# google-research/rigl

Measured on AMD Instinct MI355X. Metric: images/sec/node, ResNet-50 80% ERK RigL step, higher is better.
Workload: dtype bf16

## Files before the change

### include/rigl_hip.h

```cpp
#ifndef RIGL_HIP_H_
#define RIGL_HIP_H_

#include <stddef.h>
#include <stdint.h>

#ifdef __cplusplus
extern "C" {
#endif

#define RIGL_ABI_VERSION 2

typedef void* rigl_stream_t;
typedef uint16_t rigl_bf16;

enum {
  RIGL_OK = 0,
  RIGL_EINVAL = -1,
  RIGL_ELAUNCH = -2,
  RIGL_EWORKSPACE = -3,
  RIGL_EUNSUPPORTED = -4
};

int rigl_version(void);
uint32_t rigl_crc32c(const void* data, size_t n, uint32_t crc);
// ... 104 lines not shown

int rigl_masked_adam(int64_t n, float* w, float* m, float* v,
                     const float* dense_grad, const uint32_t* mask_bits,
                     const float* beta_powers , float lr,
                     float beta1, float beta2, float epsilon,
                     float weight_decay, float grad_scale,
                     rigl_bf16* w_shadow, rigl_stream_t stream);
int rigl_adam_advance(float* beta_powers , float beta1,
                      float beta2, rigl_stream_t stream);

int rigl_pack_weights(const float* w, const uint32_t* mask_bits ,
                      int32_t k, int32_t cout, rigl_bf16* hwio, rigl_bf16* ohwi,
                      rigl_stream_t stream);
typedef struct RiglPackLayer {
  const float* w;
  const uint32_t* mask_bits;
  rigl_bf16* hwio;
  rigl_bf16* ohwi;
  int32_t k, cout;
} RiglPackLayer;
int rigl_pack_weights_batched(const RiglPackLayer* layers, int32_t n_layers,
                              rigl_stream_t stream);

typedef struct RiglConvDesc {
  int32_t n, h, w, cin;
  int32_t ho, wo, cout;
  int32_t kh, kw;
  int32_t stride_h, stride_w;
  int32_t pad_top, pad_left;
} RiglConvDesc;

size_t rigl_conv2d_workspace_bytes(const RiglConvDesc* d, int32_t which );
int rigl_masked_conv2d_fwd(const RiglConvDesc* d, const rigl_bf16* x,
                           const rigl_bf16* w_ohwi, rigl_bf16* y,
                           void* workspace, size_t workspace_bytes,
                           rigl_stream_t stream);
int rigl_masked_conv2d_dgrad(const RiglConvDesc* d, const rigl_bf16* dy,
                             const rigl_bf16* w_hwio, rigl_bf16* dx,
                             void* workspace, size_t workspace_bytes,
                             rigl_stream_t stream);
int32_t rigl_conv2d_stats_parts(const RiglConvDesc* d);
int rigl_masked_conv2d_fwd_stats(const RiglConvDesc* d, const rigl_bf16* x,
                                 const rigl_bf16* w_ohwi, rigl_bf16* y,
                                 float* stats, size_t stats_floats,
                                 void* workspace, size_t workspace_bytes,
                                 rigl_stream_t stream);
int32_t rigl_conv2d_fwd_takes_bn_input(const RiglConvDesc* d);
int rigl_masked_conv2d_fwd_bnrelu(const RiglConvDesc* d, const rigl_bf16* x_pre,
                                  const float* scale_shift, rigl_bf16* a_out,
                                  const rigl_bf16* w_ohwi, rigl_bf16* y,
                                  float* stats , size_t stats_floats,
                                  void* workspace, size_t workspace_bytes,
                                  rigl_stream_t stream);
int rigl_masked_conv2d_dgrad_acc(const RiglConvDesc* d, const rigl_bf16* dy,
                                 const rigl_bf16* w_hwio, const rigl_bf16* addend,
                                 rigl_bf16* dx, void* workspace,
                                 size_t workspace_bytes, rigl_stream_t stream);
int rigl_masked_conv2d_wgrad(const RiglConvDesc* d, const rigl_bf16* x,
                             const rigl_bf16* dy, float* dw, void* workspace,
                             size_t workspace_bytes, rigl_stream_t stream);

int rigl_masked_conv2d_bwd(const RiglConvDesc* d, const rigl_bf16* x,
                           const rigl_bf16* dy, const rigl_bf16* w_hwio,
                           const rigl_bf16* addend , float* dw,
                           rigl_bf16* dx , void* workspace,
                           size_t workspace_bytes, rigl_stream_t stream);

int rigl_masked_conv2d_bwd_grid(const RiglConvDesc* d, const rigl_bf16* x,
                                const rigl_bf16* dy, const rigl_bf16* w_hwio,
                                float* dw, rigl_bf16* dx_grid, void* workspace,
                                size_t workspace_bytes, rigl_stream_t stream);
int rigl_masked_conv2d_bwd_sub(const RiglConvDesc* d, const rigl_bf16* x,
                               const rigl_bf16* dy, const rigl_bf16* w_hwio,
                               const rigl_bf16* addend, int32_t sub_h, int32_t sub_w,
                               float* dw, rigl_bf16* dx, void* workspace,
                               size_t workspace_bytes, rigl_stream_t stream);
int32_t rigl_conv2d_bwd_takes_masked_addend(const RiglConvDesc* d);
int rigl_masked_conv2d_bwd_masked(const RiglConvDesc* d, const rigl_bf16* x,
                                  const rigl_bf16* dy, const rigl_bf16* w_hwio,
                                  const rigl_bf16* addend, const uint8_t* addend_bits,
                                  float* dw, rigl_bf16* dx, void* workspace,
                                  size_t workspace_bytes, rigl_stream_t stream);

typedef struct RiglBnReduceFuse {
  const rigl_bf16* x;
  const uint8_t* relu_bits;
  const float* params;
  int32_t relu;
  float* partial;
  size_t partial_floats;
} RiglBnReduceFuse;
int32_t rigl_conv2d_dgrad_stats_parts(const RiglConvDesc* d);
int rigl_masked_conv2d_bwd_bn(const RiglConvDesc* d, const rigl_bf16* x,
                              const rigl_bf16* dy, const rigl_bf16* w_hwio,
                              const rigl_bf16* addend, float* dw, rigl_bf16* dx,
                              void* workspace, size_t workspace_bytes,
                              const RiglBnReduceFuse* bn ,
                              rigl_stream_t stream);

size_t rigl_depthwise_conv2d_workspace_bytes(const RiglConvDesc* d);
int rigl_depthwise_conv2d_fwd(const RiglConvDesc* d, const rigl_bf16* x,
                              const float* w, rigl_bf16* y, rigl_stream_t stream);
int32_t rigl_depthwise_conv2d_stats_parts(const RiglConvDesc* d);
int rigl_depthwise_conv2d_fwd_stats(const RiglConvDesc* d, const rigl_bf16* x,
                                    const float* w, rigl_bf16* y, float* stats,
                                    size_t stats_floats, rigl_stream_t stream);
int rigl_depthwise_conv2d_dgrad(const RiglConvDesc* d, const rigl_bf16* dy,
                                const float* w, rigl_bf16* dx,
                                rigl_stream_t stream);
int rigl_depthwise_conv2d_wgrad(const RiglConvDesc* d, const rigl_bf16* x,
                                const rigl_bf16* dy, float* dw, void* workspace,
                                size_t workspace_bytes, rigl_stream_t stream);

int rigl_conv2d_fwd_ref(const RiglConvDesc* d, const rigl_bf16* x,
                        const rigl_bf16* w_ohwi, rigl_bf16* y,
                        rigl_stream_t stream);
int rigl_conv2d_dgrad_ref(const RiglConvDesc* d, const rigl_bf16* dy,
                          const rigl_bf16* w_hwio, rigl_bf16* dx,
                          rigl_stream_t stream);
int rigl_conv2d_wgrad_ref(const RiglConvDesc* d, const rigl_bf16* x,
                          const rigl_bf16* dy, float* dw, rigl_stream_t stream);

int rigl_masked_conv2d_fwd_f32(const RiglConvDesc* d, const float* x,
                               const float* w_hwio, const uint32_t* mask_bits ,
                               float* y, rigl_stream_t stream);
int rigl_masked_conv2d_dgrad_f32(const RiglConvDesc* d, const float* dy,
                                 const float* w_hwio, const uint32_t* mask_bits ,
                                 const float* addend ,
                                 float* dx, rigl_stream_t stream);
size_t rigl_conv2d_wgrad_f32_workspace_bytes(const RiglConvDesc* d);
int rigl_masked_conv2d_wgrad_f32(const RiglConvDesc* d, const float* x,
                                 const float* dy, float* dw, void* workspace,
                                 size_t workspace_bytes, rigl_stream_t stream);

size_t rigl_bn_workspace_bytes(int64_t m, int32_t c);
int rigl_bn_fwd(int64_t m, int32_t c, const rigl_bf16* x,
                const rigl_bf16* residual , const float* gamma,
                const float* beta, float* running_mean, float* running_var,
                float momentum, float eps, int32_t relu, rigl_bf16* y,
                float* save_mean, float* save_invstd, float* save_scale,
                float* save_shift, void* workspace, size_t workspace_bytes,
                rigl_stream_t stream);
int rigl_bn_fwd_stats(int64_t m, int32_t c, const rigl_bf16* x,
                      const rigl_bf16* residual ,
                      const float* gamma, const float* beta,
                      float* running_mean, float* running_var, float momentum,
                      float eps, int32_t relu, rigl_bf16* y, float* save_mean,
                      float* save_invstd, float* save_scale, float* save_shift,
                      const float* stats, int32_t stats_parts,
                      uint8_t* relu_bits ,
                      void* workspace, size_t workspace_bytes, rigl_stream_t stream);
int rigl_bn_bwd(int64_t m, int32_t c, const rigl_bf16* x,
                const rigl_bf16* y ,
                const uint8_t* relu_bits , const rigl_bf16* dy,
                const float* gamma, const float* save_mean,
                const float* save_invstd, const float* save_scale,
                const float* save_shift, int32_t relu, rigl_bf16* dx,
                rigl_bf16* dresidual , float* dgamma,
                float* dbeta, void* workspace, size_t workspace_bytes,
                rigl_stream_t stream);
int rigl_bn_bwd_stats(int64_t m, int32_t c, const rigl_bf16* x,
                      const rigl_bf16* y ,
                      const uint8_t* relu_bits , const rigl_bf16* dy,
                      const float* gamma, const float* save_mean,
                      const float* save_invstd, const float* save_scale,
                      const float* save_shift, int32_t relu, rigl_bf16* dx,
                      rigl_bf16* dresidual , float* dgamma,
                      float* dbeta, const float* stats, int32_t stats_parts,
                      void* workspace, size_t workspace_bytes, rigl_stream_t stream);

int rigl_bn_add_bn_fwd(int64_t m, int32_t c, const rigl_bf16* x, const rigl_bf16* x2,
                       const float* scale2, const float* shift2,
                       const float* gamma, const float* beta, float* running_mean,
                       float* running_var, float momentum, float eps, int32_t relu,
                       rigl_bf16* y, float* save_mean, float* save_invstd,
                       float* save_scale, float* save_shift, const float* stats,
                       int32_t stats_parts, uint8_t* relu_bits ,
                       void* workspace, size_t workspace_bytes, rigl_stream_t stream);
size_t rigl_bn_add_bn_bwd_workspace_bytes(int64_t m, int32_t c);
int rigl_bn_add_bn_bwd(int64_t m, int32_t c, const rigl_bf16* x, const rigl_bf16* x2,
                       const uint8_t* relu_bits, const rigl_bf16* dy,
                       const float* gamma, const float* save_mean, const float* save_invstd,
                       const float* gamma2, const float* save_mean2, const float* save_invstd2,
                       rigl_bf16* dx, rigl_bf16* dx2, float* dgamma, float* dbeta,
                       float* dgamma2, float* dbeta2, void* workspace,
                       size_t workspace_bytes, rigl_stream_t stream);

int rigl_stateless_random(float* out, int64_t n, int32_t seed0, int32_t seed1,
                          int32_t dist, float scale, float shift,
                          rigl_stream_t stream);
typedef struct {
  float* out;
  int64_t n;
  int32_t seed0, seed1;
  int32_t dist;
  float scale, shift;
} RiglRandomItem;
int rigl_stateless_random_batched(const RiglRandomItem* items, int32_t n_items,
                                  rigl_stream_t stream);

int rigl_maxpool_fwd(const RiglConvDesc* d, const rigl_bf16* x, rigl_bf16* y,
                     uint8_t* argmax, rigl_stream_t stream);
int rigl_maxpool_bwd(const RiglConvDesc* d, const rigl_bf16* dy,
                     const uint8_t* argmax, rigl_bf16* dx, rigl_stream_t stream);
int rigl_bn_fwd_statistics(int64_t m, int32_t c, const rigl_bf16* x ,
                           const float* gamma, const float* beta,
                           float* running_mean, float* running_var, float momentum,
                           float eps, float* save_mean, float* save_invstd,
                           float* save_scale, float* save_shift,
                           const float* stats, int32_t stats_parts,
                           void* workspace, size_t workspace_bytes, rigl_stream_t stream);
int rigl_bn_relu_maxpool_fwd(const RiglConvDesc* d, const rigl_bf16* x,
                             const float* scale, const float* shift, rigl_bf16* y,
                             uint8_t* argmax, rigl_stream_t stream);
size_t rigl_bn_relu_maxpool_bwd_workspace_bytes(const RiglConvDesc* d);
int rigl_bn_relu_maxpool_bwd(const RiglConvDesc* d, const rigl_bf16* x,
                             const rigl_bf16* dy, const uint8_t* argmax,
                             const float* gamma, const float* save_mean,
                             const float* save_invstd, const float* save_scale,
                             const float* save_shift, rigl_bf16* dx, float* dgamma,
                             float* dbeta, void* workspace, size_t workspace_bytes,
                             rigl_stream_t stream);

int rigl_global_avgpool_fwd(int32_t n, int32_t pixels, int32_t c, const rigl_bf16* x,
                            rigl_bf16* y, rigl_stream_t stream);
int rigl_global_avgpool_bwd(int32_t n, int32_t pixels, int32_t c, const rigl_bf16* dy,
                            rigl_bf16* dx, rigl_stream_t stream);
int rigl_global_avgpool_bwd_relu(int32_t n, int32_t pixels, int32_t c, const rigl_bf16* dy,
                                 const rigl_bf16* x, rigl_bf16* dx, rigl_stream_t stream);
int rigl_softmax_xent(int32_t rows, int32_t classes, const rigl_bf16* logits,
                      const int64_t* labels, float label_smoothing, float grad_scale,
                      float* row_loss, rigl_bf16* dlogits , rigl_stream_t stream);

int32_t rigl_conv2d_fwd_takes_relu_epilogue(const RiglConvDesc* d);
int32_t rigl_conv2d_bwd_takes_relu_epilogue(const RiglConvDesc* d);
int rigl_masked_conv2d_fwd_relu(const RiglConvDesc* d, const rigl_bf16* x,
                                const rigl_bf16* w_ohwi, rigl_bf16* y, void* workspace,
                                size_t workspace_bytes, rigl_stream_t stream);
int rigl_masked_conv2d_bwd_relu(const RiglConvDesc* d, const rigl_bf16* x,
                                const rigl_bf16* dy, const rigl_bf16* w_hwio, float* dw,
                                rigl_bf16* dx, void* workspace, size_t workspace_bytes,
                                rigl_stream_t stream);
int rigl_relu_fwd(int64_t n, const rigl_bf16* x, rigl_bf16* y, rigl_stream_t stream);
// ... 61 lines not shown
```

### rigl_amd/_lib.py

```python
import ctypes as C
import os

_HERE = os.path.dirname(os.path.abspath(__file__))
ABI_VERSION = 2
LIB_PATH = os.environ.get('RIGL_HIP_LIB') or os.path.join(_HERE, 'lib', 'librigl_hip.so')

RIGL_OK = 0
RIGL_EINVAL = -1
RIGL_ELAUNCH = -2
RIGL_EWORKSPACE = -3
RIGL_EUNSUPPORTED = -4
COUNTS_PER_LAYER = 8
MAGPRUNE_COUNTS_PER_LAYER = 4
PROF_KINDS = ('conv_fwd', 'conv_dgrad', 'conv_wgrad', 'prune_regrow',
              'sgd_momentum', 'pack_weights', 'conv_bwd', 'depthwise', 'masked_adam', 'magnitude_prune')

GROW_ZEROS, GROW_GRAD_SCALE, GROW_GRAD_SIGN, GROW_EXPLICIT = 0, 1, 2, 3
MOMRESET_ZEROS, MOMRESET_GRAD = 0, 1


class RiglError(RuntimeError):

  def __init__(self, code, msg):
    super().__init__('librigl_hip: error %d: %s' % (code, msg))
# ... 21 lines not shown
class MagnitudePruneLayer(C.Structure):
  _fields_ = [('n', C.c_int64), ('w', C.c_void_p), ('mask_bits', C.c_void_p), ('threshold', C.c_void_p),
              ('k', C.c_int64)]


class PackLayer(C.Structure):
  _fields_ = [('w', C.c_void_p), ('mask_bits', C.c_void_p),
              ('hwio', C.c_void_p), ('ohwi', C.c_void_p), ('k', C.c_int32),
              ('cout', C.c_int32)]


class ConvDesc(C.Structure):
  _fields_ = [('n', C.c_int32), ('h', C.c_int32), ('w', C.c_int32),
              ('cin', C.c_int32), ('ho', C.c_int32), ('wo', C.c_int32),
              ('cout', C.c_int32), ('kh', C.c_int32), ('kw', C.c_int32),
              ('stride_h', C.c_int32), ('stride_w', C.c_int32),
              ('pad_top', C.c_int32), ('pad_left', C.c_int32)]


class BnReduceFuse(C.Structure):
  _fields_ = [('x', C.c_void_p), ('relu_bits', C.c_void_p), ('params', C.c_void_p), ('relu', C.c_int32),
              ('partial', C.c_void_p), ('partial_floats', C.c_size_t)]


class RandomItem(C.Structure):
  _fields_ = [('out', C.c_void_p), ('n', C.c_int64), ('seed0', C.c_int32), ('seed1', C.c_int32),
              ('dist', C.c_int32), ('scale', C.c_float), ('shift', C.c_float)]


class BnInferItem(C.Structure):
  _fields_ = [('gamma', C.c_void_p), ('beta', C.c_void_p), ('moving_mean', C.c_void_p), ('moving_variance', C.c_void_p),
              ('scale_shift', C.c_void_p), ('c', C.c_int32), ('eps', C.c_float)]


class ProfLaunch(C.Structure):
  _fields_ = [('kind', C.c_int32), ('tag', C.c_int32 * 6), ('ms', C.c_float)]


_P, _I32, _I64, _F, _SZ = C.c_void_p, C.c_int32, C.c_int64, C.c_float, C.c_size_t
SIGNATURES = {
    'rigl_version': (C.c_int, []),
    'rigl_last_error': (C.c_char_p, []),
    'rigl_mask_pack': (C.c_int, [_P, _P, _I64, _P]),
    'rigl_mask_unpack': (C.c_int, [_P, _P, _I64, _P]),
    'rigl_prune_regrow_workspace_bytes': (_SZ, [C.POINTER(_I64), _I32]),
    'rigl_prune_regrow': (C.c_int, [C.POINTER(PruneRegrowLayer), _I32,
                                    C.POINTER(PruneRegrowParams), _P, _P, _SZ,
                                    _P]),
    'rigl_prune_regrow_slots': (C.c_int, [C.POINTER(PruneRegrowLayer), C.POINTER(_P), _I32,
                                          C.POINTER(PruneRegrowParams), _P, _P, _SZ, _P]),
    'rigl_prune_regrow_selections_workspace_bytes': (_SZ, [_I64]),
    'rigl_prune_regrow_selections': (C.c_int, [C.POINTER(PruneRegrowLayer), C.POINTER(PruneRegrowParams), _P, _P, _P, _P, _P,
                                               _P, _SZ, _P]),
    'rigl_prune_regrow_selections_slots': (C.c_int, [C.POINTER(PruneRegrowLayer), _P, C.POINTER(PruneRegrowParams), _P, _P,
                                                     _P, _P, _P, _P, _SZ, _P]),
    'rigl_topk_mask': (C.c_int, [_P, _I64, _I64, _P, _P, _SZ, _P]),
    'rigl_topk_mask_batched': (C.c_int, [C.POINTER(TopkLayer), _I32, _P, _SZ, _P]),
    'rigl_magnitude_prune_batched_workspace_bytes': (_SZ, [_I32]),
    'rigl_magnitude_prune_batched': (C.c_int, [C.POINTER(MagnitudePruneLayer), _I32, C.c_double, _P, _P, _SZ, _P]),
    'rigl_masked_sgd_momentum': (C.c_int, [_I64, _P, _P, _P, _P, _F, _F, _F, _F,
                                           _I32, _P, _P]),
    'rigl_masked_adam': (C.c_int, [_I64, _P, _P, _P, _P, _P, _P, _F, _F, _F, _F, _F, _F, _P, _P]),
    'rigl_adam_advance': (C.c_int, [_P, _F, _F, _P]),
    'rigl_pack_weights': (C.c_int, [_P, _P, _I32, _I32, _P, _P, _P]),
    'rigl_pack_weights_batched': (C.c_int, [C.POINTER(PackLayer), _I32, _P]),
    'rigl_conv2d_workspace_bytes': (_SZ, [C.POINTER(ConvDesc), _I32]),
    'rigl_masked_conv2d_fwd': (C.c_int, [C.POINTER(ConvDesc), _P, _P, _P, _P,
                                         _SZ, _P]),
    'rigl_masked_conv2d_dgrad': (C.c_int, [C.POINTER(ConvDesc), _P, _P, _P, _P,
                                           _SZ, _P]),
    'rigl_conv2d_stats_parts': (_I32, [C.POINTER(ConvDesc)]),
    'rigl_masked_conv2d_fwd_stats': (C.c_int, [C.POINTER(ConvDesc), _P, _P, _P, _P,
                                               _SZ, _P, _SZ, _P]),
    'rigl_conv2d_fwd_takes_bn_input': (_I32, [C.POINTER(ConvDesc)]),
    'rigl_masked_conv2d_fwd_bnrelu': (C.c_int, [C.POINTER(ConvDesc), _P, _P, _P, _P, _P, _P, _SZ, _P, _SZ, _P]),
    'rigl_masked_conv2d_dgrad_acc': (C.c_int, [C.POINTER(ConvDesc), _P, _P, _P,
                                               _P, _P, _SZ, _P]),
    'rigl_conv2d_dgrad_stats_parts': (_I32, [C.POINTER(ConvDesc)]),
    'rigl_masked_conv2d_bwd_bn': (C.c_int, [C.POINTER(ConvDesc), _P, _P, _P, _P, _P, _P, _P, _SZ,
                                            C.POINTER(BnReduceFuse), _P]),
    'rigl_masked_conv2d_bwd': (C.c_int, [C.POINTER(ConvDesc), _P, _P, _P, _P, _P, _P, _P, _SZ, _P]),
    'rigl_masked_conv2d_bwd_masked': (C.c_int, [C.POINTER(ConvDesc), _P, _P, _P, _P, _P, _P, _P, _P, _SZ, _P]),
    'rigl_conv2d_bwd_takes_masked_addend': (_I32, [C.POINTER(ConvDesc)]),
    'rigl_masked_conv2d_bwd_grid': (C.c_int, [C.POINTER(ConvDesc), _P, _P, _P, _P, _P, _P, _SZ, _P]),
    'rigl_masked_conv2d_bwd_sub': (C.c_int, [C.POINTER(ConvDesc), _P, _P, _P, _P, _I32, _I32, _P, _P, _P, _SZ, _P]),
    'rigl_masked_conv2d_wgrad': (C.c_int, [C.POINTER(ConvDesc), _P, _P, _P, _P,
                                           _SZ, _P]),
    'rigl_conv2d_fwd_ref': (C.c_int, [C.POINTER(ConvDesc), _P, _P, _P, _P]),
    'rigl_conv2d_dgrad_ref': (C.c_int, [C.POINTER(ConvDesc), _P, _P, _P, _P]),
    'rigl_conv2d_wgrad_ref': (C.c_int, [C.POINTER(ConvDesc), _P, _P, _P, _P]),
    'rigl_masked_conv2d_fwd_f32': (C.c_int, [C.POINTER(ConvDesc), _P, _P, _P, _P, _P]),
    'rigl_masked_conv2d_dgrad_f32': (C.c_int, [C.POINTER(ConvDesc), _P, _P, _P, _P, _P, _P]),
    'rigl_conv2d_wgrad_f32_workspace_bytes': (_SZ, [C.POINTER(ConvDesc)]),
    'rigl_masked_conv2d_wgrad_f32': (C.c_int, [C.POINTER(ConvDesc), _P, _P, _P, _P, _SZ, _P]),
    'rigl_depthwise_conv2d_workspace_bytes': (_SZ, [C.POINTER(ConvDesc)]),
    'rigl_depthwise_conv2d_fwd': (C.c_int, [C.POINTER(ConvDesc), _P, _P, _P, _P]),
    'rigl_depthwise_conv2d_stats_parts': (_I32, [C.POINTER(ConvDesc)]),
    'rigl_depthwise_conv2d_fwd_stats': (C.c_int, [C.POINTER(ConvDesc), _P, _P, _P, _P, _SZ, _P]),
    'rigl_depthwise_conv2d_dgrad': (C.c_int, [C.POINTER(ConvDesc), _P, _P, _P, _P]),
    'rigl_depthwise_conv2d_wgrad': (C.c_int, [C.POINTER(ConvDesc), _P, _P, _P, _P, _SZ, _P]),
    'rigl_bn_workspace_bytes': (_SZ, [_I64, _I32]),
    'rigl_bn_fwd': (C.c_int, [_I64, _I32, _P, _P, _P, _P, _P, _P, _F, _F, _I32, _P, _P, _P, _P, _P, _P, _SZ, _P]),
    'rigl_bn_fwd_stats': (C.c_int, [_I64, _I32, _P, _P, _P, _P, _P, _P, _F, _F, _I32, _P, _P, _P, _P, _P, _P, _I32, _P, _P, _SZ, _P]),
    'rigl_bn_bwd': (C.c_int, [_I64, _I32, _P, _P, _P, _P, _P, _P, _P, _P, _P, _I32, _P, _P, _P, _P, _P, _SZ, _P]),
    'rigl_bn_bwd_stats': (C.c_int, [_I64, _I32, _P, _P, _P, _P, _P, _P, _P, _P, _P, _I32, _P, _P, _P, _P, _P, _I32, _P, _SZ, _P]),
    'rigl_crc32c': (C.c_uint32, [_P, _SZ, C.c_uint32]),
    'rigl_stateless_random': (C.c_int, [_P, _I64, _I32, _I32, _I32, _F, _F, _P]),
    'rigl_stateless_random_batched': (C.c_int, [C.POINTER(RandomItem), _I32, _P]),
    'rigl_maxpool_fwd': (C.c_int, [C.POINTER(ConvDesc), _P, _P, _P, _P]),
    'rigl_maxpool_bwd': (C.c_int, [C.POINTER(ConvDesc), _P, _P, _P, _P]),
    'rigl_bn_fwd_statistics': (C.c_int, [_I64, _I32, _P, _P, _P, _P, _P, _F, _F, _P, _P, _P, _P, _P, _I32, _P, _SZ, _P]),
    'rigl_bn_add_bn_fwd': (C.c_int, [_I64, _I32, _P, _P, _P, _P, _P, _P, _P, _P, _F, _F, _I32, _P, _P, _P, _P, _P, _P, _I32, _P, _P, _SZ, _P]),
    'rigl_bn_add_bn_bwd_workspace_bytes': (_SZ, [_I64, _I32]),
    'rigl_bn_add_bn_bwd': (C.c_int, [_I64, _I32, _P, _P, _P, _P, _P, _P, _P, _P, _P, _P, _P, _P, _P, _P, _P, _P, _P, _SZ, _P]),
    'rigl_bn_relu_maxpool_fwd': (C.c_int, [C.POINTER(ConvDesc), _P, _P, _P, _P, _P, _P]),
    'rigl_bn_relu_maxpool_bwd_workspace_bytes': (_SZ, [C.POINTER(ConvDesc)]),
    'rigl_bn_relu_maxpool_bwd': (C.c_int, [C.POINTER(ConvDesc), _P, _P, _P, _P, _P, _P, _P, _P, _P, _P, _P, _P, _SZ, _P]),
    'rigl_global_avgpool_fwd': (C.c_int, [_I32, _I32, _I32, _P, _P, _P]),
    'rigl_global_avgpool_bwd': (C.c_int, [_I32, _I32, _I32, _P, _P, _P]),
    'rigl_softmax_xent': (C.c_int, [_I32, _I32, _P, _P, _F, _F, _P, _P, _P]),
    'rigl_global_avgpool_bwd_relu': (C.c_int, [_I32, _I32, _I32, _P, _P, _P, _P]),
    'rigl_conv2d_fwd_takes_relu_epilogue': (C.c_int32, [C.POINTER(ConvDesc)]),
    'rigl_conv2d_bwd_takes_relu_epilogue': (C.c_int32, [C.POINTER(ConvDesc)]),
    'rigl_masked_conv2d_fwd_relu': (C.c_int, [C.POINTER(ConvDesc), _P, _P, _P, _P, _SZ, _P]),
    'rigl_masked_conv2d_bwd_relu': (C.c_int, [C.POINTER(ConvDesc), _P, _P, _P, _P, _P, _P, _SZ, _P]),
    'rigl_relu_fwd': (C.c_int, [_I64, _P, _P, _P]),
    'rigl_relu_bwd': (C.c_int, [_I64, _P, _P, _P, _P]),
    'rigl_bn_infer_params_batched': (C.c_int, [C.POINTER(BnInferItem), _I32, _P]),
    'rigl_bn_apply': (C.c_int, [_I64, _I32, _P, _P, _P, _I32, _P, _P]),
    'rigl_bn_apply_pair': (C.c_int, [_I64, _I32, _P, _P, _P, _P, _I32, _P, _P]),
    'rigl_bn_relu_maxpool_infer': (C.c_int, [C.POINTER(ConvDesc), _P, _P, _P, _P]),
    'rigl_conv2d_fwd_takes_bn_epilogue': (C.c_int32, [C.POINTER(ConvDesc), _I32, _I32]),
    'rigl_masked_conv2d_fwd_bn_infer': (C.c_int, [C.POINTER(ConvDesc), _P, _P, _P, _P, _P, _I32, _P, _P]),
    'rigl_eval_metrics': (C.c_int, [_I32, _I32, _P, _P, _F, _I32, _P, _P, _P, _P]),
    'rigl_prof_enable': (C.c_int, [_I32]),
    'rigl_prof_collect': (C.c_int, [C.POINTER(C.c_double), C.POINTER(_I64)]),
    'rigl_prof_collect_kinds': (C.c_int, [C.POINTER(C.c_double), C.POINTER(_I64), _I32]),
    'rigl_prof_collect_launches': (C.c_int, [C.POINTER(ProfLaunch), _I64, C.POINTER(_I64)]),
    'rigl_probe_mfma_bf16': (C.c_int, [_I32, _I32, _P, _P]),
    'rigl_tune_set': (C.c_int, [C.c_char_p, _I32]),
    'rigl_tune_get': (_I32, [C.c_char_p, _I32]),
    'rigl_tune_generation': (C.c_uint64, []),
    'rigl_tune_generation_addr': (C.c_void_p, []),
    'rigl_tune_unset': (C.c_int, [C.c_char_p]),
}

_lib = None


def load():
  global _lib
  if _lib is not None:
    return _lib
  if not os.path.exists(LIB_PATH):
    raise RiglError(
        RIGL_ELAUNCH, 'HIP extension not built: %s is missing; run '
        '`python -c "import __graft_entry__ as g; g.build()"` or '
        '`make -C rigl_amd/csrc`' % LIB_PATH)
  try:
    import torch
  except ImportError:
    pass
  lib = C.CDLL(LIB_PATH, mode=C.RTLD_GLOBAL)
  for name, (res, args) in SIGNATURES.items():
    fn = getattr(lib, name)
    fn.restype = res
    fn.argtypes = args
  if lib.rigl_version() != ABI_VERSION:
    raise RiglError(RIGL_EINVAL, 'ABI version mismatch')
  _lib = lib
  return lib


def check(rc):
  if rc != RIGL_OK:
    raise RiglError(rc, load().rigl_last_error().decode('utf-8', 'replace'))
```

### rigl_amd/csrc/bn.hip

```cpp
#include "common.hpp"

namespace rigl {
namespace kbn {

constexpr int THREADS = 256;
constexpr int MAX_PARTS = 512;

__device__ __forceinline__ float bf_lo(uint32_t w) { return __uint_as_float(w << 16); }
__device__ __forceinline__ float bf_hi(uint32_t w) { return __uint_as_float(w & 0xFFFF0000u); }
__device__ __forceinline__ uint32_t f2bf(float f) {
  uint32_t u = __float_as_uint(f);
  if ((u & 0x7FFFFFFFu) > 0x7F800000u) return (u >> 16) | 0x40u;
  u += 0x7FFFu + ((u >> 16) & 1u);
  return u >> 16;
}
typedef __attribute__((ext_vector_type(2))) __bf16 bf16x2_t;
typedef __attribute__((ext_vector_type(2))) float f32x2_t;
__device__ __forceinline__ uint32_t pack2(float a, float b) {
  const f32x2_t v = {a, b};
  return __builtin_bit_cast(uint32_t, __builtin_convertvector(v, bf16x2_t));
}
__device__ __forceinline__ void unpack8(const uint4& v, float f[8]) {
  f[0] = bf_lo(v.x); f[1] = bf_hi(v.x); f[2] = bf_lo(v.y); f[3] = bf_hi(v.y);
  f[4] = bf_lo(v.z); f[5] = bf_hi(v.z); f[6] = bf_lo(v.w); f[7] = bf_hi(v.w);
// ... 204 lines not shown
    unpack8(ld16(x + i * 8, G.nt), xv);
    if (HAS_RES) unpack8(ld16(res + i * 8, G.nt), rv);
    float o[8];
#pragma unroll
    for (int j = 0; j < 8; ++j) {
      float v = fmaf(xv[j], psc[j], psh[j]);
      if (HAS_RES) v += rv[j];
      o[j] = RELU ? fmaxf(v, 0.f) : v;
    }
    uint4 out;
    out.x = pack2(o[0], o[1]); out.y = pack2(o[2], o[3]); out.z = pack2(o[4], o[5]); out.w = pack2(o[6], o[7]);
    st16(y + i * 8, out, G.nt);
    if (RELU && mbits) {
      uint32_t mb = 0u;
#pragma unroll
      for (int j = 0; j < 8; ++j) mb |= (o[j] > 0.f ? 1u : 0u) << j;
      mbits[i] = (uint8_t)mb;
    }
  }
}

template <int CL>
__global__ __launch_bounds__(THREADS) void k_bwd_finalize(Geom G, const float* __restrict__ partial,
                                                           const float* __restrict__ gamma, const float* __restrict__ invstd,
                                                           float* __restrict__ dgamma, float* __restrict__ dbeta,
                                                           float* __restrict__ coef ) {
  double s0, s1; int c; bool leader;
  sum_partials<CL>(G, partial, s0, s1, c, leader);
  if (!leader) return;
  dbeta[c] = (float)s0;
  dgamma[c] = (float)s1;
  coef[c] = gamma[c] * invstd[c];
  coef[G.C + c] = (float)(s0 / (double)G.M);
  coef[2 * G.C + c] = (float)(s1 / (double)G.M);
}

template <bool RELU, int MSK, bool HAS_DRES>
__global__ __launch_bounds__(THREADS) void k_bwd_apply(Geom G, const uint16_t* __restrict__ x, const uint16_t* __restrict__ y,
                                                        const uint8_t* __restrict__ mbits,
                                                        const uint16_t* __restrict__ dy, const float* __restrict__ mean,
                                                        const float* __restrict__ invstd, const float* __restrict__ scale,
                                                        const float* __restrict__ shift, const float* __restrict__ coef,
                                                        uint16_t* __restrict__ dx, uint16_t* __restrict__ dres) {
  extern __shared__ __attribute__((aligned(16))) float prm[];
  const bool fixed = G.fixed != 0;
  float pm[8], pis[8], pa[8], pb[8], pc[8], psc[8], psh[8];
  if (fixed) {
    const int c0 = (int)(((int64_t)blockIdx.x * THREADS + threadIdx.x) % G.cg) * 8;
    ld8f(mean + c0, pm); ld8f(invstd + c0, pis);
    ld8f(coef + c0, pa); ld8f(coef + G.C + c0, pb); ld8f(coef + 2 * G.C + c0, pc);
    if (RELU && MSK == 0) { ld8f(scale + c0, psc); ld8f(shift + c0, psh); }
  } else {
    for (int i = threadIdx.x; i < G.C; i += THREADS) {
      prm[i] = mean[i]; prm[G.C + i] = invstd[i];
      prm[2 * G.C + i] = coef[i]; prm[3 * G.C + i] = coef[G.C + i]; prm[4 * G.C + i] = coef[2 * G.C + i];
      if (RELU && MSK == 0) { prm[5 * G.C + i] = scale[i]; prm[6 * G.C + i] = shift[i]; }
    }
    __syncthreads();
  }
  const int64_t total = G.M * G.cg;
  const int64_t stride = (int64_t)gridDim.x * THREADS;
  for (int64_t i = (int64_t)blockIdx.x * THREADS + threadIdx.x; i < total; i += stride) {
    if (!fixed) {
      const int c0 = (int)(i % G.cg) * 8;
#pragma unroll
      for (int j = 0; j < 8; ++j) {
        pm[j] = prm[c0 + j]; pis[j] = prm[G.C + c0 + j]; pa[j] = prm[2 * G.C + c0 + j]; pb[j] = prm[3 * G.C + c0 + j];
        pc[j] = prm[4 * G.C + c0 + j];
        if (RELU && MSK == 0) { psc[j] = prm[5 * G.C + c0 + j]; psh[j] = prm[6 * G.C + c0 + j]; }
      }
    }
    float xv[8], dv[8], yv[8];
    unpack8(ld16(x + i * 8, G.nt), xv);
    unpack8(ld16(dy + i * 8, G.nt), dv);
    uint32_t mb = 0u;
    if (RELU && MSK == 1) unpack8(*reinterpret_cast<const uint4*>(y + i * 8), yv);
    if (RELU && MSK == 2) mb = mbits[i];
    float o[8], z[8];
#pragma unroll
    for (int j = 0; j < 8; ++j) {
      bool on = true;
      if (RELU) on = MSK == 1 ? (yv[j] > 0.f) : (MSK == 2 ? ((mb >> j) & 1u) != 0u : (fmaf(xv[j], psc[j], psh[j]) > 0.f));
      const float dz = on ? dv[j] : 0.f;
      const float xh = (xv[j] - pm[j]) * pis[j];
      o[j] = pa[j] * (dz - pb[j] - xh * pc[j]);
      z[j] = dz;
    }
    uint4 out;
    out.x = pack2(o[0], o[1]); out.y = pack2(o[2], o[3]); out.z = pack2(o[4], o[5]); out.w = pack2(o[6], o[7]);
    st16(dx + i * 8, out, G.nt);
    if (HAS_DRES) {
      out.x = pack2(z[0], z[1]); out.y = pack2(z[2], z[3]); out.z = pack2(z[4], z[5]); out.w = pack2(z[6], z[7]);
      st16(dres + i * 8, out, G.nt);
    }
  }
}

template <bool RELU>
__global__ __launch_bounds__(THREADS) void k_fwd_apply_pair(Geom G, const uint16_t* __restrict__ x, const uint16_t* __restrict__ x2,
                                                             const float* __restrict__ scale, const float* __restrict__ shift,
                                                             const float* __restrict__ scale2, const float* __restrict__ shift2,
                                                             uint16_t* __restrict__ y, uint8_t* __restrict__ mbits) {
  extern __shared__ __attribute__((aligned(16))) float prm[];
  const bool fixed = G.fixed != 0;
  float p0[8], p1[8], p2[8], p3[8];
  if (fixed) {
    const int c0 = (int)(((int64_t)blockIdx.x * THREADS + threadIdx.x) % G.cg) * 8;
    ld8f(scale + c0, p0); ld8f(shift + c0, p1); ld8f(scale2 + c0, p2); ld8f(shift2 + c0, p3);
  } else {
    for (int i = threadIdx.x; i < G.C; i += THREADS) {
      prm[i] = scale[i]; prm[G.C + i] = shift[i]; prm[2 * G.C + i] = scale2[i]; prm[3 * G.C + i] = shift2[i];
    }
    __syncthreads();
  }
  const int64_t total = G.M * G.cg;
  const int64_t stride = (int64_t)gridDim.x * THREADS;
  for (int64_t i = (int64_t)blockIdx.x * THREADS + threadIdx.x; i < total; i += stride) {
    if (!fixed) {
      const int c0 = (int)(i % G.cg) * 8;
#pragma unroll
      for (int j = 0; j < 8; ++j) { p0[j] = prm[c0 + j]; p1[j] = prm[G.C + c0 + j]; p2[j] = prm[2 * G.C + c0 + j]; p3[j] = prm[3 * G.C + c0 + j]; }
    }
    float xv[8], rv[8];
    unpack8(ld16(x + i * 8, G.nt), xv);
    unpack8(ld16(x2 + i * 8, G.nt), rv);
    float o[8];
#pragma unroll
    for (int j = 0; j < 8; j += 2) {
      const uint32_t pk = pack2(fmaf(rv[j], p2[j], p3[j]), fmaf(rv[j + 1], p2[j + 1], p3[j + 1]));
      float v0 = fmaf(xv[j], p0[j], p1[j]);
      float v1 = fmaf(xv[j + 1], p0[j + 1], p1[j + 1]);
      v0 += bf_lo(pk); v1 += bf_hi(pk);
      o[j] = RELU ? fmaxf(v0, 0.f) : v0;
      o[j + 1] = RELU ? fmaxf(v1, 0.f) : v1;
    }
    uint4 out;
    out.x = pack2(o[0], o[1]); out.y = pack2(o[2], o[3]); out.z = pack2(o[4], o[5]); out.w = pack2(o[6], o[7]);
    st16(y + i * 8, out, G.nt);
    if (RELU && mbits) {
      uint32_t mb = 0u;
#pragma unroll
      for (int j = 0; j < 8; ++j) mb |= (o[j] > 0.f ? 1u : 0u) << j;
      mbits[i] = (uint8_t)mb;
    }
  }
}

__global__ __launch_bounds__(THREADS) void k_reduce_pair(Geom G, const uint16_t* __restrict__ x, const uint16_t* __restrict__ x2,
                                                          const uint8_t* __restrict__ mbits, const uint16_t* __restrict__ dy,
                                                          const float* __restrict__ mean, const float* __restrict__ invstd,
                                                          const float* __restrict__ mean2, const float* __restrict__ invstd2,
                                                          float* __restrict__ partial, float* __restrict__ partial2) {
  __shared__ float red[THREADS][25];
  const int tx = threadIdx.x % G.tpr, ty = threadIdx.x / G.tpr;
  const int cgi = blockIdx.y * G.tpr + tx;
  const bool c_ok = cgi < G.cg;
  const int64_t r0 = (int64_t)blockIdx.x * G.rows_per_part;
  int64_t r1 = r0 + G.rows_per_part;
  if (r1 > G.M) r1 = G.M;
  float q0[8], q1[8], q2[8], mu[8], is[8], mu2[8], is2[8];
#pragma unroll
  for (int j = 0; j < 8; ++j) { q0[j] = q1[j] = q2[j] = 0.f; mu[j] = is[j] = mu2[j] = is2[j] = 0.f; }
  if (c_ok) {
#pragma unroll
    for (int j = 0; j < 8; ++j) {
      mu[j] = mean[cgi * 8 + j]; is[j] = invstd[cgi * 8 + j]; mu2[j] = mean2[cgi * 8 + j]; is2[j] = invstd2[cgi * 8 + j];
    }
    const int64_t rb = G.il ? (int64_t)blockIdx.x * G.rpb + ty : r0 + ty, re = G.il ? G.M : r1;
// ... 264 lines not shown
  using namespace rigl;
  using namespace rigl::kbn;
  if (m <= 0 || c <= 0 || (!x && !stats) || !gamma || !beta || !save_mean || !save_invstd || !save_scale || !save_shift)
    return fail(RIGL_EINVAL, "rigl_bn_fwd_statistics: bad arguments");
  if (c % 8) return fail(RIGL_EUNSUPPORTED, "rigl_bn_fwd_statistics: channels %% 8 != 0");
  if (stats && stats_parts <= 0) return fail(RIGL_EINVAL, "rigl_bn_fwd_statistics: stats_parts must be positive");
  Geom g = make_geom(m, c);
  int rc = fwd_statistics(g, c, x, gamma, beta, running_mean, running_var, momentum, eps, save_mean, save_invstd,
                          save_scale, save_shift, stats, stats_parts, workspace, workspace_bytes, as_stream(stream));
  if (rc) return rc;
  RIGL_CHECK_LAUNCH("rigl_bn_fwd_statistics");
  return RIGL_OK;
}

int rigl_bn_add_bn_fwd(int64_t m, int32_t c, const rigl_bf16* x, const rigl_bf16* x2, const float* scale2,
                       const float* shift2, const float* gamma, const float* beta, float* running_mean,
                       float* running_var, float momentum, float eps, int32_t relu, rigl_bf16* y, float* save_mean,
                       float* save_invstd, float* save_scale, float* save_shift, const float* stats,
                       int32_t stats_parts, uint8_t* relu_bits, void* workspace, size_t workspace_bytes,
                       rigl_stream_t stream) {
  using namespace rigl;
  using namespace rigl::kbn;
  if (m <= 0 || c <= 0 || !x || !x2 || !scale2 || !shift2 || !gamma || !beta || !y || !save_mean || !save_invstd ||
      !save_scale || !save_shift)
    return fail(RIGL_EINVAL, "rigl_bn_add_bn_fwd: bad arguments");
  if (c % 8) return fail(RIGL_EUNSUPPORTED, "rigl_bn_add_bn_fwd: channels %% 8 != 0");
  if (4 * (size_t)c * 4 > 65536) return fail(RIGL_EUNSUPPORTED, "rigl_bn_add_bn_fwd: too many channels for the LDS parameter cache");
  if (stats && stats_parts <= 0) return fail(RIGL_EINVAL, "rigl_bn_add_bn_fwd: stats_parts must be positive");
  hipStream_t st = as_stream(stream);
  Geom g = make_geom(m, c);
  int rc = fwd_statistics(g, c, x, gamma, beta, running_mean, running_var, momentum, eps, save_mean, save_invstd,
                          save_scale, save_shift, stats, stats_parts, workspace, workspace_bytes, st);
  if (rc) return rc;
  dim3 agrid(apply_grid(g));
  const size_t lds = g.fixed ? 0 : (size_t)4 * c * 4;
  if (relu) hipLaunchKernelGGL(k_fwd_apply_pair<true>, agrid, dim3(THREADS), lds, st, g, x, x2, save_scale, save_shift, scale2, shift2, y, relu_bits);
  else hipLaunchKernelGGL(k_fwd_apply_pair<false>, agrid, dim3(THREADS), lds, st, g, x, x2, save_scale, save_shift, scale2, shift2, y, nullptr);
  RIGL_CHECK_LAUNCH("rigl_bn_add_bn_fwd");
  return RIGL_OK;
}

size_t rigl_bn_add_bn_bwd_workspace_bytes(int64_t m, int32_t c) { return 2 * rigl_bn_workspace_bytes(m, c); }

int rigl_bn_add_bn_bwd(int64_t m, int32_t c, const rigl_bf16* x, const rigl_bf16* x2, const uint8_t* relu_bits,
                       const rigl_bf16* dy, const float* gamma, const float* save_mean, const float* save_invstd,
                       const float* gamma2, const float* save_mean2, const float* save_invstd2, rigl_bf16* dx,
                       rigl_bf16* dx2, float* dgamma, float* dbeta, float* dgamma2, float* dbeta2, void* workspace,
                       size_t workspace_bytes, rigl_stream_t stream) {
  using namespace rigl;
  using namespace rigl::kbn;
  if (m <= 0 || c <= 0 || !x || !x2 || !relu_bits || !dy || !gamma || !save_mean || !save_invstd || !gamma2 || !save_mean2 ||
      !save_invstd2 || !dx || !dx2 || !dgamma || !dbeta || !dgamma2 || !dbeta2)
    return fail(RIGL_EINVAL, "rigl_bn_add_bn_bwd: bad arguments");
  if (c % 8) return fail(RIGL_EUNSUPPORTED, "rigl_bn_add_bn_bwd: channels %% 8 != 0");
  const size_t lds = (size_t)10 * c * 4;
  if (lds > 160 * 1024 - 1024) return fail(RIGL_EUNSUPPORTED, "rigl_bn_add_bn_bwd: too many channels for the LDS parameter cache");
  const size_t need = rigl_bn_add_bn_bwd_workspace_bytes(m, c);
  if (!workspace || workspace_bytes < need) return fail(RIGL_EWORKSPACE, "rigl_bn_add_bn_bwd: workspace %zu < %zu", workspace_bytes, need);
  static const bool big_lds = hipFuncSetAttribute(reinterpret_cast<const void*>(&k_bwd_apply_pair),
                                                  hipFuncAttributeMaxDynamicSharedMemorySize, 159 * 1024) == hipSuccess;
  if (lds > 65536 && !big_lds) return fail(RIGL_ELAUNCH, "rigl_bn_add_bn_bwd: cannot raise the dynamic LDS limit");
  hipStream_t st = as_stream(stream);
  Geom g = make_geom(m, c);
  const size_t half = rigl_bn_workspace_bytes(m, c);
  const size_t part_bytes = align_up((size_t)g.parts * 2 * c * 4, 256);
  char* w0 = static_cast<char*>(workspace);
  float* partial = reinterpret_cast<float*>(w0);
  float* coef = reinterpret_cast<float*>(w0 + part_bytes);
  float* partial2 = reinterpret_cast<float*>(w0 + half);
  float* coef2 = reinterpret_cast<float*>(w0 + half + part_bytes);
  dim3 rgrid((unsigned)g.parts, (unsigned)((g.cg + g.tpr - 1) / g.tpr));
  hipLaunchKernelGGL(k_reduce_pair, rgrid, dim3(THREADS), 0, st, g, x, x2, relu_bits, dy, save_mean, save_invstd, save_mean2,
                     save_invstd2, partial, partial2);
  const FinSet f0 = {partial, gamma, save_invstd, dgamma, dbeta, coef};
  const FinSet f1 = {partial2, gamma2, save_invstd2, dgamma2, dbeta2, coef2};
  hipLaunchKernelGGL(k_bwd_finalize_pair<16>, dim3((unsigned)((c + 15) / 16), 2), dim3(THREADS), 0, st, g, f0, f1);
  const dim3 pgrid(apply_grid(g));
  hipLaunchKernelGGL(k_bwd_apply_pair, pgrid, dim3(THREADS), g.fixed ? 0 : lds, st, g, x, x2, relu_bits, dy, save_mean, save_invstd,
                     save_mean2, save_invstd2, coef, coef2, dx, dx2);
  RIGL_CHECK_LAUNCH("rigl_bn_add_bn_bwd");
  return RIGL_OK;
}

int rigl_bn_bwd_stats(int64_t m, int32_t c, const rigl_bf16* x, const rigl_bf16* y, const uint8_t* relu_bits,
                      const rigl_bf16* dy, const float* gamma,
                      const float* save_mean, const float* save_invstd, const float* save_scale, const float* save_shift,
                      int32_t relu, rigl_bf16* dx, rigl_bf16* dresidual, float* dgamma, float* dbeta,
                      const float* stats, int32_t stats_parts, void* workspace,
                      size_t workspace_bytes, rigl_stream_t stream) {
  using namespace rigl;
  using namespace rigl::kbn;
  if (m <= 0 || c <= 0 || !x || !dy || !gamma || !save_mean || !save_invstd || !dx || !dgamma || !dbeta)
    return fail(RIGL_EINVAL, "rigl_bn_bwd: bad arguments");
  if (c % 8) return fail(RIGL_EUNSUPPORTED, "rigl_bn_bwd: channels %% 8 != 0");
  if (relu && !y && !relu_bits && (!save_scale || !save_shift))
    return fail(RIGL_EINVAL, "rigl_bn_bwd: relu needs y, relu_bits or scale/shift");
  if (7 * (size_t)c * 4 > 65536) return fail(RIGL_EUNSUPPORTED, "rigl_bn_bwd: too many channels for the LDS parameter cache");
  if (stats && stats_parts <= 0) return fail(RIGL_EINVAL, "rigl_bn_bwd_stats: stats_parts must be positive");
  const size_t need = rigl_bn_workspace_bytes(m, c);
  if (!workspace || workspace_bytes < need) return fail(RIGL_EWORKSPACE, "rigl_bn_bwd: workspace %zu < %zu", workspace_bytes, need);
  hipStream_t st = as_stream(stream);
  Geom g = make_geom(m, c);
  float* partial = static_cast<float*>(workspace);
  float* coef = reinterpret_cast<float*>(static_cast<char*>(workspace) + align_up((size_t)g.parts * 2 * c * 4, 256));
  dim3 rgrid((unsigned)g.parts, (unsigned)((g.cg + g.tpr - 1) / g.tpr));
  const int msk = relu_bits ? 2 : (y ? 1 : 0);
  const float* red = partial;
  if (stats) {
    red = stats;
    g.parts = stats_parts;
  } else {
#define RIGL_BWD_REDUCE(R, K) hipLaunchKernelGGL((k_reduce<1, R, K>), rgrid, dim3(THREADS), 0, st, g, x, y, relu_bits, dy, save_mean, save_invstd, save_scale, save_shift, partial)
    if (!relu) RIGL_BWD_REDUCE(false, 0);
    else if (msk == 2) RIGL_BWD_REDUCE(true, 2);
    else if (msk == 1) RIGL_BWD_REDUCE(true, 1);
    else RIGL_BWD_REDUCE(true, 0);
#undef RIGL_BWD_REDUCE
  }
  if (g.parts > MAX_PARTS)
    hipLaunchKernelGGL(k_bwd_finalize<4>, dim3((unsigned)((c + 3) / 4)), dim3(THREADS), 0, st, g, red, gamma,
                       save_invstd, dgamma, dbeta, coef);
  else
    hipLaunchKernelGGL(k_bwd_finalize<16>, dim3((unsigned)((c + 15) / 16)), dim3(THREADS), 0, st, g, red, gamma,
                       save_invstd, dgamma, dbeta, coef);
  dim3 agrid(apply_grid(g));
  const size_t lds = g.fixed ? 0 : (size_t)7 * c * 4;
#define RIGL_BWD_APPLY(R, K, D) hipLaunchKernelGGL((k_bwd_apply<R, K, D>), agrid, dim3(THREADS), lds, st, g, x, y, relu_bits, dy, save_mean, save_invstd, save_scale, save_shift, coef, dx, dresidual)
  const bool dres = dresidual != nullptr;
  if (!relu) { if (dres) RIGL_BWD_APPLY(false, 0, true); else RIGL_BWD_APPLY(false, 0, false); }
  else if (msk == 2) { if (dres) RIGL_BWD_APPLY(true, 2, true); else RIGL_BWD_APPLY(true, 2, false); }
  else if (msk == 1) { if (dres) RIGL_BWD_APPLY(true, 1, true); else RIGL_BWD_APPLY(true, 1, false); }
  else { if (dres) RIGL_BWD_APPLY(true, 0, true); else RIGL_BWD_APPLY(true, 0, false); }
#undef RIGL_BWD_APPLY
  RIGL_CHECK_LAUNCH("rigl_bn_bwd");
  return RIGL_OK;
}

int rigl_bn_bwd(int64_t m, int32_t c, const rigl_bf16* x, const rigl_bf16* y, const uint8_t* relu_bits,
                const rigl_bf16* dy, const float* gamma,
                const float* save_mean, const float* save_invstd, const float* save_scale, const float* save_shift,
                int32_t relu, rigl_bf16* dx, rigl_bf16* dresidual, float* dgamma, float* dbeta, void* workspace,
                size_t workspace_bytes, rigl_stream_t stream) {
  return rigl_bn_bwd_stats(m, c, x, y, relu_bits, dy, gamma, save_mean, save_invstd, save_scale, save_shift, relu, dx,
                           dresidual, dgamma, dbeta, nullptr, 0, workspace, workspace_bytes, stream);
}

int rigl_bn_infer_params_batched(const RiglBnInferItem* items, int32_t n_items, rigl_stream_t stream) {
  using namespace rigl;
  using namespace rigl::kbn;
  if (n_items < 0 || (n_items > 0 && !items)) return fail(RIGL_EINVAL, "rigl_bn_infer_params_batched: bad arguments");
  for (int i = 0; i < n_items; ++i) {
    const RiglBnInferItem& t = items[i];
    if (t.c < 0 || (t.c > 0 && (!t.gamma || !t.beta || !t.moving_mean || !t.moving_variance || !t.scale_shift)))
      return fail(RIGL_EINVAL, "rigl_bn_infer_params_batched: item %d: bad channels / NULL tensor", i);
  }
  hipStream_t st = as_stream(stream);
  for (int b = 0; b < n_items; b += INFER_BATCH) {
    InferBatch B;
    B.count = 0;
    int32_t blk = 0;
    for (int i = b; i < n_items && i < b + INFER_BATCH; ++i) {
      if (items[i].c == 0) continue;
      B.it[B.count] = items[i];
      B.blk_begin[B.count] = blk;
      blk += (items[i].c + THREADS - 1) / THREADS;
      ++B.count;
    }
    B.blk_begin[B.count] = blk;
    if (B.count) hipLaunchKernelGGL(k_infer_params, dim3((unsigned)blk), dim3(THREADS), 0, st, B);
  }
  RIGL_CHECK_LAUNCH("rigl_bn_infer_params_batched");
  return RIGL_OK;
}

int rigl_bn_apply(int64_t m, int32_t c, const rigl_bf16* x, const rigl_bf16* residual, const float* scale_shift, int32_t relu,
                  rigl_bf16* y, rigl_stream_t stream) {
  using namespace rigl;
  using namespace rigl::kbn;
  if (m <= 0 || c <= 0 || !x || !scale_shift || !y) return fail(RIGL_EINVAL, "rigl_bn_apply: bad arguments");
  if (c % 8) return fail(RIGL_EUNSUPPORTED, "rigl_bn_apply: channels %% 8 != 0");
  if (2 * (size_t)c * 4 > 65536) return fail(RIGL_EUNSUPPORTED, "rigl_bn_apply: too many channels for the LDS parameter cache");
  hipStream_t st = as_stream(stream);
  Geom g = make_geom(m, c);
  dim3 agrid(apply_grid(g));
  const size_t lds = g.fixed ? 0 : (size_t)2 * c * 4;
  const float* sc = scale_shift;
  const float* sh = scale_shift + c;
  if (relu && residual) hipLaunchKernelGGL((k_fwd_apply<true, true>), agrid, dim3(THREADS), lds, st, g, x, residual, sc, sh, y, nullptr);
  else if (relu) hipLaunchKernelGGL((k_fwd_apply<true, false>), agrid, dim3(THREADS), lds, st, g, x, residual, sc, sh, y, nullptr);
  else if (residual) hipLaunchKernelGGL((k_fwd_apply<false, true>), agrid, dim3(THREADS), lds, st, g, x, residual, sc, sh, y, nullptr);
  else hipLaunchKernelGGL((k_fwd_apply<false, false>), agrid, dim3(THREADS), lds, st, g, x, residual, sc, sh, y, nullptr);
  RIGL_CHECK_LAUNCH("rigl_bn_apply");
  return RIGL_OK;
}

int rigl_bn_apply_pair(int64_t m, int32_t c, const rigl_bf16* x, const rigl_bf16* x2, const float* scale_shift,
                       const float* scale_shift2, int32_t relu, rigl_bf16* y, rigl_stream_t stream) {
  using namespace rigl;
  using namespace rigl::kbn;
  if (m <= 0 || c <= 0 || !x || !x2 || !scale_shift || !scale_shift2 || !y) return fail(RIGL_EINVAL, "rigl_bn_apply_pair: bad arguments");
  if (c % 8) return fail(RIGL_EUNSUPPORTED, "rigl_bn_apply_pair: channels %% 8 != 0");
  if (4 * (size_t)c * 4 > 65536) return fail(RIGL_EUNSUPPORTED, "rigl_bn_apply_pair: too many channels for the LDS parameter cache");
  hipStream_t st = as_stream(stream);
  Geom g = make_geom(m, c);
  dim3 agrid(apply_grid(g));
  const size_t lds = g.fixed ? 0 : (size_t)4 * c * 4;
  if (relu) hipLaunchKernelGGL(k_fwd_apply_pair<true>, agrid, dim3(THREADS), lds, st, g, x, x2, scale_shift, scale_shift + c, scale_shift2, scale_shift2 + c, y, nullptr);
  else hipLaunchKernelGGL(k_fwd_apply_pair<false>, agrid, dim3(THREADS), lds, st, g, x, x2, scale_shift, scale_shift + c, scale_shift2, scale_shift2 + c, y, nullptr);
  RIGL_CHECK_LAUNCH("rigl_bn_apply_pair");
  return RIGL_OK;
}

}
```

### rigl_amd/csrc/bwd1x1.hpp

```cpp
#pragma once

struct Bwd1x1Args {
  const uint16_t* X;
  const uint16_t* DY;
  const uint16_t* W;
  const uint16_t* ADD;
  uint16_t* DX;
  float* SLAB;
  int M, splits, interleave;
  uint32_t x_bytes, dy_bytes;
};

template <int ROWB>
__device__ __forceinline__ int dual_swz(int row) {
  if (ROWB == 512) return ((row & 1) << 1) | (((row >> 1) & 1) << 2) | (((row ^ (row >> 2)) & 1) << 3);
  return (((row >> 1) & 1) << 1) | ((((row >> 1) ^ (row >> 2)) & 1) << 2);
}

typedef __attribute__((ext_vector_type(4))) float f32x4;

template <int CI, int CO, bool DO_W, int NST>
struct Bwd1x1Smem { static constexpr int BYTES = NST * 32 * ((DO_W ? CI : 0) + CO) * 2 + (CI <= 64 ? 2 : 1) * 32 * (CI * 2 + 16); };
template <int CI, int CO, bool DO_W, int NST>
__global__ __launch_bounds__(THREADS) void k_bwd1x1(Bwd1x1Args P) {
  constexpr int PX = 32;
  constexpr int YROWB = CO * 2, XROWB = CI * 2;
  constexpr int Y_BYTES = PX * YROWB, X_BYTES = DO_W ? PX * XROWB : 0, STAGE = Y_BYTES + X_BYTES;
  constexpr int YI = YROWB / 32, XI = XROWB / 32;
  constexpr int YPW = YI / 4 > 0 ? YI / 4 : 1, XPW = XI / 4 > 0 ? XI / 4 : 1;
  static_assert(YI % 4 == 0 && XI % 4 == 0, "tiles are whole rounds of four waves");
  constexpr int L = YPW + (DO_W ? XPW : 0);
  constexpr int CF = CI / 16, CFW = CF / 2;
  constexpr int KSD = CO / 32;
  constexpr int NFI = CI / 32, NFO = CO / 32;
  constexpr bool WIDE_O = NFO >= NFI;
  constexpr int WF = NFI * NFO / 4 > 0 ? NFI * NFO / 4 : 1;
  static_assert(CFW * KSD * 4 <= 96, "W fragments stay in registers");
  constexpr bool DXDB = CI <= 64;
  constexpr int NDX = DXDB ? 2 : 1;
  constexpr int DXROWB = XROWB + 16, DX_BYTES = PX * DXROWB;
  static_assert(NST * STAGE + NDX * DX_BYTES == Bwd1x1Smem<CI, CO, DO_W, NST>::BYTES, "host and device agree on the LDS size");
  extern __shared__ __attribute__((aligned(1024))) unsigned char smem[];
  unsigned char* const dxs = smem + NST * STAGE;

  const int tid = threadIdx.x, lane = tid & 63;
  const int wave = __builtin_amdgcn_readfirstlane(tid >> 6);
  const int split = blockIdx.x;
  const int KT_all = (P.M + PX - 1) / PX;
  const int kt_begin = P.interleave ? split : (int)((int64_t)KT_all * split / P.splits);
  const int kt_step = P.interleave ? P.splits : 1;
  const int KT = P.interleave ? (split < KT_all ? (KT_all - split + P.splits - 1) / P.splits : 0)
                              : (int)((int64_t)KT_all * (split + 1) / P.splits) - kt_begin;
  const __amdgpu_buffer_rsrc_t rsrcY = make_rsrc(P.DY, P.dy_bytes), rsrcX = make_rsrc(P.X, P.x_bytes);
  const u32x4 rsrcY4 = make_rsrc4(P.DY, P.dy_bytes), rsrcX4 = make_rsrc4(P.X, P.x_bytes);
  (void)rsrcY4; (void)rsrcX4; (void)rsrcY; (void)rsrcX;

  int y_row[YPW], y_col[YPW], x_row[XPW], x_col[XPW];
#pragma unroll
  for (int q = 0; q < YPW; ++q) {
    const int i = q * 4 + wave, row = i * (1024 / YROWB) + lane / (YROWB / 16), slot = lane % (YROWB / 16);
    y_row[q] = row; y_col[q] = (slot ^ dual_swz<YROWB>(row)) * 8;
  }
#pragma unroll
  for (int q = 0; q < XPW; ++q) {
    const int i = q * 4 + wave, row = i * (1024 / XROWB) + lane / (XROWB / 16), slot = lane % (XROWB / 16);
    x_row[q] = row; x_col[q] = (slot ^ dual_swz<XROWB>(row)) * 8;
  }
#if !defined(RIGL_B1_NO_NT) && !defined(RIGL_DMA_BUILTIN)
#define B1_DMA16(r_, lds_, off_) lds_dma16_nt(r_##4, lds_, off_)
#else
#define B1_DMA16(r_, lds_, off_) RIGL_DMA16(r_, lds_, off_)
#endif
#define B1_ISSUE(kt_, stage_)                                                                            \
  {                                                                                                      \
    const int p0_ = (kt_begin + (kt_) * kt_step) * PX;                                                             \
    _Pragma("unroll") for (int q = 0; q < YPW; ++q) {                                                    \
      const int p_ = p0_ + y_row[q];                                                                     \
      const int off_ = p_ < P.M ? (int)((uint32_t)(p_ * CO + y_col[q]) * 2u) : (int)OOB;                 \
      B1_DMA16(rsrcY, smem + (stage_) * STAGE + (q * 4 + wave) * 1024, off_); \
    }                                                                                                    \
    if (DO_W) {                                                                                          \
      _Pragma("unroll") for (int q = 0; q < XPW; ++q) {                                                  \
        const int p_ = p0_ + x_row[q];                                                                   \
        const int off_ = p_ < P.M ? (int)((uint32_t)(p_ * CI + x_col[q]) * 2u) : (int)OOB;               \
        B1_DMA16(rsrcX, smem + (stage_) * STAGE + Y_BYTES + (q * 4 + wave) * 1024, off_); \
      }                                                                                                  \
    }                                                                                                    \
  }

  const int pf = wave & 1, chalf = wave >> 1;
  bf16x8 wfr[CFW][KSD];
#pragma unroll
  for (int c = 0; c < CFW; ++c)
#pragma unroll
    for (int ks = 0; ks < KSD; ++ks) {
      const int ci = (chalf * CFW + c) * 16 + (lane & 15), co = ks * 32 + (lane >> 4) * 8;
      wfr[c][ks] = *reinterpret_cast<const bf16x8*>(P.W + (int64_t)ci * CO + co);
    }
  const int d_row = 16 * pf + (lane & 15);
  const int d_base = d_row * YROWB, d_swz = dual_swz<YROWB>(d_row), d_hi = lane >> 4;

  const int g = lane >> 4, j16 = lane & 15;
  const int t_row = 8 * (g >> 1) + (j16 >> 2);
  const int t_low = 2 * (g & 1) + ((j16 >> 1) & 1), t_half = (j16 & 1) * 8;
  f32x16 acc2[DO_W ? WF : 1];
  if (DO_W) {
#pragma unroll
    for (int f = 0; f < WF; ++f)
#pragma unroll
      for (int e = 0; e < 16; ++e) acc2[f][e] = 0.f;
  }
  const int w_fix = WIDE_O ? wave % NFI : wave % NFO;
  const int w_var0 = WIDE_O ? (wave / NFI) * WF : (wave / NFO) * WF;
#define B1_TR_OFF(ROWB_, chunk_, plus4_) \
  ((t_row + (plus4_)) * (ROWB_) + ((((chunk_) + t_low) ^ dual_swz<ROWB_>(t_row + (plus4_))) << 4) + t_half)

  constexpr int DXP = PX * (CI / 8) / THREADS;
  static_assert(PX * (CI / 8) % THREADS == 0, "whole pieces per thread");
  constexpr int W_N = L * (NST - 2), W_A = W_N + DXP * (NST - 1);
  uint4 addv[DXP];
#define B1_FLUSH(ktp_, second_barrier_)                                                                    \
  {                                                                                                        \
    const int p0_ = (kt_begin + (ktp_) * kt_step) * PX;                                                              \
    const unsigned char* src_ = dxs + ((ktp_) & (NDX - 1)) * DX_BYTES;                                     \
    uint4 v_[DXP];                                                                                         \
    _Pragma("unroll") for (int q = 0; q < DXP; ++q) {                                                      \
      const int idx = q * THREADS + tid, row = idx / (CI / 8), ch = idx % (CI / 8);                        \
      v_[q] = *reinterpret_cast<const uint4*>(src_ + row * DXROWB + ch * 16);                              \
    }                                                                                                      \
    if (second_barrier_) __syncthreads();                                                                  \
    _Pragma("unroll") for (int q = 0; q < DXP; ++q) {                                                      \
      const int idx = q * THREADS + tid, row = idx / (CI / 8), ch = idx % (CI / 8);                        \
      if (p0_ + row < P.M) {                                                                               \
        uint4 v = v_[q];                                                                                   \
        if (P.ADD) {                                                                                       \
          const uint4 a = addv[q];                                                                         \
          v.x = add_bf16x2(v.x, a.x); v.y = add_bf16x2(v.y, a.y); v.z = add_bf16x2(v.z, a.z); v.w = add_bf16x2(v.w, a.w); \
        }                                                                                                  \
        *reinterpret_cast<uint4*>(P.DX + (int64_t)(p0_ + row) * CI + ch * 8) = v;                          \
      }                                                                                                    \
    }                                                                                                      \
  }
  for (int t = 0; t < NST - 1; ++t)
    if (t < KT) B1_ISSUE(t, t);
  for (int kt = 0; kt < KT; ++kt) {
    if (kt + NST - 1 <= KT) {
      if (P.ADD && kt >= NST - 1) wait_vmcnt<W_A>();
      else wait_vmcnt<W_N>();
    } else {
      wait_vmcnt<0>();
    }
    asm volatile("s_waitcnt lgkmcnt(0)" ::: "memory");
    __builtin_amdgcn_s_barrier();
    asm volatile("" ::: "memory");
    if (kt + NST - 1 < KT) B1_ISSUE(kt + NST - 1, (kt + NST - 1) % NST);
    asm volatile("" ::: "memory");
    __builtin_amdgcn_sched_barrier(0);
    if (kt > 0) B1_FLUSH(kt - 1, !DXDB);
    asm volatile("" ::: "memory");
    __builtin_amdgcn_sched_barrier(0);
    const unsigned char* Ys = smem + (kt % NST) * STAGE;
    const unsigned char* Xs = Ys + Y_BYTES;
    if (P.ADD) {
      const int p0 = (kt_begin + kt * kt_step) * PX;
#pragma unroll
      for (int q = 0; q < DXP; ++q) {
        const int idx = q * THREADS + tid, row = idx / (CI / 8), ch = idx % (CI / 8);
        addv[q] = p0 + row < P.M ? *reinterpret_cast<const uint4*>(P.ADD + (int64_t)(p0 + row) * CI + ch * 8) : make_uint4(0u, 0u, 0u, 0u);
      }
    }
    asm volatile("" ::: "memory");
    __builtin_amdgcn_sched_barrier(0);
    f32x4 acc1[CFW];
#pragma unroll
    for (int c = 0; c < CFW; ++c) acc1[c] = (f32x4){0.f, 0.f, 0.f, 0.f};
#pragma unroll
    for (int ks = 0; ks < KSD; ++ks) {
      const bf16x8 yf = *reinterpret_cast<const bf16x8*>(Ys + d_base + (((4 * ks + d_hi) ^ d_swz) << 4));
#pragma unroll
      for (int c = 0; c < CFW; ++c) acc1[c] = __builtin_amdgcn_mfma_f32_16x16x32_bf16(wfr[c][ks], yf, acc1[c], 0, 0, 0);
    }
    if (DO_W) {
#pragma unroll
      for (int k2 = 0; k2 < 2; ++k2) {
        bf16x8 fa[WIDE_O ? 1 : WF], fb[WIDE_O ? WF : 1];
        if (WIDE_O) {
          fa[0] = lds_read_tr_pair(Xs + k2 * 16 * XROWB + B1_TR_OFF(XROWB, w_fix * 4, 0), Xs + k2 * 16 * XROWB + B1_TR_OFF(XROWB, w_fix * 4, 4));
#pragma unroll
          for (int f = 0; f < WF; ++f)
            fb[f] = lds_read_tr_pair(Ys + k2 * 16 * YROWB + B1_TR_OFF(YROWB, (w_var0 + f) * 4, 0),
                                     Ys + k2 * 16 * YROWB + B1_TR_OFF(YROWB, (w_var0 + f) * 4, 4));
#pragma unroll
          for (int f = 0; f < WF; ++f) acc2[f] = __builtin_amdgcn_mfma_f32_32x32x16_bf16(fa[0], fb[f], acc2[f], 0, 0, 0);
        } else {
          fb[0] = lds_read_tr_pair(Ys + k2 * 16 * YROWB + B1_TR_OFF(YROWB, w_fix * 4, 0), Ys + k2 * 16 * YROWB + B1_TR_OFF(YROWB, w_fix * 4, 4));
#pragma unroll
          for (int f = 0; f < WF; ++f)
            fa[f] = lds_read_tr_pair(Xs + k2 * 16 * XROWB + B1_TR_OFF(XROWB, (w_var0 + f) * 4, 0),
                                     Xs + k2 * 16 * XROWB + B1_TR_OFF(XROWB, (w_var0 + f) * 4, 4));
#pragma unroll
          for (int f = 0; f < WF; ++f) acc2[f] = __builtin_amdgcn_mfma_f32_32x32x16_bf16(fa[f], fb[0], acc2[f], 0, 0, 0);
        }
      }
    }
    {
      const int prow = 16 * pf + (lane & 15);
      unsigned char* const dst = dxs + (kt & (NDX - 1)) * DX_BYTES;
#pragma unroll
      for (int c = 0; c < CFW; ++c) {
        const f32x2 lo = {acc1[c][0], acc1[c][1]}, hi2 = {acc1[c][2], acc1[c][3]};
        uint2 pk;
        pk.x = __builtin_bit_cast(uint32_t, __builtin_convertvector(lo, bf16x2));
        pk.y = __builtin_bit_cast(uint32_t, __builtin_convertvector(hi2, bf16x2));
        *reinterpret_cast<uint2*>(dst + prow * DXROWB + ((chalf * CFW + c) * 16 + (lane >> 4) * 4) * 2) = pk;
      }
    }
  }
  if (KT > 0) {
    __syncthreads();
    B1_FLUSH(KT - 1, false);
  }
#undef B1_FLUSH
#undef B1_ISSUE
#undef B1_TR_OFF
  if (DO_W) {
    float* const out = P.SLAB + (int64_t)split * CI * CO;
#pragma unroll
    for (int f = 0; f < WF; ++f) {
      const int fi = WIDE_O ? w_fix : w_var0 + f, fo = WIDE_O ? w_var0 + f : w_fix;
#pragma unroll
      for (int e = 0; e < 16; ++e) {
        const int ci = fi * 32 + (e & 3) + 8 * (e >> 2) + 4 * (lane >> 5), co = fo * 32 + (lane & 31);
        out[(int64_t)ci * CO + co] = acc2[f][e];
      }
    }
  }
}

static inline int bwd1x1_kind(const RiglConvDesc* d) {
  if (d->kh != 1 || d->kw != 1 || d->stride_h != 1 || d->stride_w != 1 || d->pad_top || d->pad_left) return 0;
  if (d->ho != d->h || d->wo != d->w) return 0;
  if ((int64_t)d->n * d->h * d->w < 65536) return 0;
  if (RIGL_TUNE("bwd1x1", 1) == 0) return 0;
  if (d->cin == 64 && d->cout == 256) return 1;
  if (d->cin == 64 && d->cout == 64) return 3;
  return 0;
}
static inline int bwd1x1_splits() { return 2 * num_cus(); }
static inline size_t bwd1x1_workspace(const RiglConvDesc* d) {
  return bwd1x1_kind(d) ? (size_t)2 * num_cus() * d->cin * d->cout * 4 : 0;
}
template <int CI, int CO, bool DO_W, int NST>
static bool bwd1x1_ready_i() {
  constexpr int SMEM = Bwd1x1Smem<CI, CO, DO_W, NST>::BYTES;
  static_assert(SMEM <= 160 * 1024 / 2, "the rings of the two workgroups resident on a CU fit its LDS");
  static const bool ready = hipFuncSetAttribute(reinterpret_cast<const void*>(&k_bwd1x1<CI, CO, DO_W, NST>),
                                                hipFuncAttributeMaxDynamicSharedMemorySize, SMEM) == hipSuccess;
  return ready;
}
static bool bwd1x1_ready(const RiglConvDesc* d) {
  switch (bwd1x1_kind(d)) {
    case 1: return bwd1x1_ready_i<64, 256, true, 3>();
    case 3: return bwd1x1_ready_i<64, 64, true, 3>();
    default: return false;
  }
}
template <int CI, int CO, bool DO_W, int NST>
static bool launch_bwd1x1_i(const Bwd1x1Args& a, hipStream_t st) {
  constexpr int SMEM = Bwd1x1Smem<CI, CO, DO_W, NST>::BYTES;
  if (!bwd1x1_ready_i<CI, CO, DO_W, NST>()) return false;
  RIGL_K_LAUNCH((k_bwd1x1<CI, CO, DO_W, NST>), dim3((unsigned)a.splits), dim3(THREADS), SMEM, st, a);
  return true;
}
template <int CI, int CO>
static bool launch_bwd1x1_t(const Bwd1x1Args& a, bool w, hipStream_t st) {
  return w ? launch_bwd1x1_i<CI, CO, true, 3>(a, st) : launch_bwd1x1_i<CI, CO, false, 3>(a, st);
}
static bool launch_bwd1x1(const RiglConvDesc* d, const rigl_bf16* x, const rigl_bf16* dy, const rigl_bf16* w_hwio,
                          const rigl_bf16* addend, rigl_bf16* dx, float* slab, hipStream_t st) {
  Bwd1x1Args a = {};
  a.X = x; a.DY = dy; a.W = w_hwio; a.ADD = addend; a.DX = dx; a.SLAB = slab;
  a.M = d->n * d->h * d->w; a.splits = bwd1x1_splits(); a.interleave = RIGL_TUNE("bwd1x1_il", 1);
  a.x_bytes = (uint32_t)((size_t)a.M * d->cin * 2); a.dy_bytes = (uint32_t)((size_t)a.M * d->cout * 2);
  const bool w = slab != nullptr;
  switch (bwd1x1_kind(d)) {
    case 1: return launch_bwd1x1_t<64, 256>(a, w, st);
    case 3: return launch_bwd1x1_t<64, 64>(a, w, st);
    default: return false;
  }
}
```

### rigl_amd/csrc/common.hpp

```cpp
#pragma once
#include <hip/hip_runtime.h>
#include <hip/hip_ext.h>
#include <stdarg.h>
#include <atomic>
#include <stdint.h>
#include <stdio.h>

#include "../../include/rigl_hip.h"

namespace rigl {

void set_error(const char* fmt, ...);
int fail(int code, const char* fmt, ...);

int tune_get(const char* key, int dflt);
struct TuneSite { std::atomic<uint64_t> gen{0}; std::atomic<int> value{0}; };
uint64_t tune_generation();
int tune_cached(TuneSite& site, const char* key, int dflt);
#define RIGL_TUNE(key, dflt) ([]() -> int { static ::rigl::TuneSite site__; return ::rigl::tune_cached(site__, key, dflt); }())

inline hipStream_t as_stream(rigl_stream_t s) { return reinterpret_cast<hipStream_t>(s); }

#define RIGL_CHECK_LAUNCH(what)                                              \
  do {                                                                       \
    hipError_t e__ = hipGetLastError();                                      \
    if (e__ != hipSuccess)                                                   \
      return ::rigl::fail(RIGL_ELAUNCH, "%s: %s", what, hipGetErrorString(e__)); \
  } while (0)

#define RIGL_HIP(call)                                                       \
  do {                                                                       \
    hipError_t e__ = (call);                                                 \
    if (e__ != hipSuccess)                                                   \
      return ::rigl::fail(RIGL_ELAUNCH, "%s: %s", #call, hipGetErrorString(e__)); \
  } while (0)

enum ProfKind { PROF_CONV_FWD = 0, PROF_CONV_DGRAD = 1, PROF_CONV_WGRAD = 2,
                PROF_PRUNE_REGROW = 3, PROF_SGD = 4, PROF_PACK = 5, PROF_CONV_BWD = 6, PROF_DEPTHWISE = 7,
                PROF_ADAM = 8, PROF_MAGPRUNE = 9 };
bool prof_enabled();
void prof_begin(int kind, hipStream_t s);
void prof_end(int kind, hipStream_t s);

hipEvent_t prof_get_event();
void prof_add_pair(int kind, hipEvent_t a, hipEvent_t b);
int& prof_current_kind();
void prof_set_tag(const RiglConvDesc* d);
struct ProfFamily {
  int prev;
  explicit ProfFamily(int k) : prev(prof_current_kind()) { prof_current_kind() = k; }
  ~ProfFamily() { prof_current_kind() = prev; }
};

struct ProfScope {
  int kind; hipStream_t s; bool on;
  ProfScope(int k, hipStream_t st) : kind(k), s(st), on(prof_enabled()) { if (on) prof_begin(kind, s); }
  ~ProfScope() { if (on) prof_end(kind, s); }
};

template <typename F, typename... Args>
inline void prof_launch(F kernel, dim3 grid, dim3 blk, unsigned lds, hipStream_t st, Args... args) {
  hipEvent_t a = prof_get_event(), b = prof_get_event();
  if (!a || !b) { hipLaunchKernelGGL(kernel, grid, blk, lds, st, args...); return; }
  hipExtLaunchKernelGGL(kernel, grid, blk, lds, st, a, b, 0, args...);
  prof_add_pair(prof_current_kind(), a, b);
}
#define RIGL_K_LAUNCH(kernel, grid, blk, lds, st, ...)                                      \
  do {                                                                                      \
    if (::rigl::prof_enabled()) ::rigl::prof_launch(kernel, grid, blk, lds, st, __VA_ARGS__); \
    else hipLaunchKernelGGL(kernel, grid, blk, lds, st, __VA_ARGS__);                       \
  } while (0)

inline int64_t ceil_div64(int64_t a, int64_t b) { return (a + b - 1) / b; }
inline size_t align_up(size_t x, size_t a) { return (x + a - 1) / a * a; }

__device__ __forceinline__ uint32_t relu_bf16x2(uint32_t v) {
  return v & ~(((v & 0x80008000u) >> 15) * 0xFFFFu);
}
__device__ __forceinline__ uint32_t gate_bf16x2(uint32_t v, uint32_t x) {
  const uint32_t lo = (x & 0xFFFFu) - 1u < 0x7FFFu ? 0x0000FFFFu : 0u;
  const uint32_t hi = (x >> 16) - 1u < 0x7FFFu ? 0xFFFF0000u : 0u;
  return v & (lo | hi);
}
__device__ __forceinline__ uint4 relu_bf16x8(uint4 v) {
  return make_uint4(relu_bf16x2(v.x), relu_bf16x2(v.y), relu_bf16x2(v.z), relu_bf16x2(v.w));
}
__device__ __forceinline__ uint4 gate_bf16x8(uint4 v, uint4 x) {
  return make_uint4(gate_bf16x2(v.x, x.x), gate_bf16x2(v.y, x.y), gate_bf16x2(v.z, x.z), gate_bf16x2(v.w, x.w));
}

}
```

### rigl_amd/csrc/conv.hip

```cpp
#include <stdlib.h>

#include "common.hpp"

#if defined(RIGL_ABLATE) && RIGL_ABLATE == 1
#define RIGL_MFMA_OR_ABLATE(i, j) acc[i][j][0] += (float)af[i][0] + (float)bfr[j][0];
#else
#define RIGL_MFMA_OR_ABLATE(i, j) acc[i][j] = __builtin_amdgcn_mfma_f32_32x32x16_bf16(bfr[j], af[i], acc[i][j], 0, 0, 0);
#endif

namespace rigl {
namespace k1 {

typedef __attribute__((ext_vector_type(8))) __bf16 bf16x8;
typedef __attribute__((ext_vector_type(2))) __bf16 bf16x2;
typedef __attribute__((ext_vector_type(2))) float f32x2;
typedef __attribute__((ext_vector_type(16))) float f32x16;

constexpr int THREADS = 256;

__device__ __forceinline__ uint16_t f2bf(float f) {
  uint32_t u = __float_as_uint(f);
  if ((u & 0x7FFFFFFFu) > 0x7F800000u) return (uint16_t)((u >> 16) | 0x40u);
  u += 0x7FFFu + ((u >> 16) & 1u);
  return (uint16_t)(u >> 16);
// ... 1665 lines not shown
    tg = tiny_geom(d);
    const size_t xp_bytes = (size_t)d->n * tg.hp * tg.wp * 4 * 2;
    uint16_t* xp = reinterpret_cast<uint16_t*>(ws);
    ws += align_up(xp_bytes, 256);
    PadArgs pa = {x, xp, d->n, d->h, d->w, d->cin, tg.hp, tg.wp, d->pad_top, d->pad_left};
    RIGL_K_LAUNCH(k_pad_input4, dim3(2048), dim3(THREADS), 0, st, pa);
    a.X = xp; a.Cin = tg.cred; a.x_pix_stride = 4; a.KH = d->kh; a.KW = 1; a.H = tg.hp; a.W = tg.wp;
    a.Ho = d->ho; a.Wo = d->wo; a.sh = d->stride_h; a.sw = d->stride_w; a.ph = a.pw = 0;
    a.x_bytes = (uint32_t)xp_bytes;
    a.fold = tg.cred; a.Cin = d->kh * tg.cred; a.KH = 1;
    n_out = (int64_t)d->kh * tg.cred * d->cout;
    tiny_tmp = reinterpret_cast<float*>(ws);
    ws += align_up((size_t)n_out * 4, 256);
  } else if (small_cin(d)) {
    const int K = d->kh * d->kw * d->cin, Kp = kpad(d);
    uint16_t* col = reinterpret_cast<uint16_t*>(ws);
    ws += align_up((size_t)a.M * Kp * 2, 256);
    Im2colArgs ia = {x, col, a.M, d->cin, d->kh, d->kw, d->h, d->w, d->ho, d->wo, d->stride_h, d->stride_w, d->pad_top, d->pad_left, K, Kp};
    RIGL_K_LAUNCH(k_im2col, dim3(2048), dim3(THREADS), 0, st, ia);
    a.X = col; a.Cin = Kp; a.x_pix_stride = Kp; a.KH = a.KW = 1; a.H = 1; a.W = a.M; a.Ho = 1; a.Wo = a.M;
    a.sh = a.sw = 1; a.ph = a.pw = 0;
    a.x_bytes = (uint32_t)((size_t)a.M * Kp * 2);
    n_out = (int64_t)K * d->cout;
  } else {
    a.X = x; a.Cin = d->cin; a.x_pix_stride = d->cin; a.KH = d->kh; a.KW = d->kw; a.H = d->h; a.W = d->w;
    a.Ho = d->ho; a.Wo = d->wo; a.sh = d->stride_h; a.sw = d->stride_w; a.ph = d->pad_top; a.pw = d->pad_left;
    a.x_bytes = (uint32_t)((size_t)d->n * d->h * d->w * d->cin * 2);
    n_out = (int64_t)d->kh * d->kw * d->cin * d->cout;
  }
  WgradPlan p = plan_wgrad(a.M, a.Cin, a.Cout, a.KH * a.KW);
  a.tiles_ci = p.tiles_ci; a.tiles_co = p.tiles_co; a.splits = p.splits; a.slab_elems = p.slab;
  const bool two_pass = p.splits > 1 || small_cin(d) || tiny_cin(d);
  a.OUT = two_pass ? reinterpret_cast<float*>(ws) : dw;
  dim3 grid((unsigned)((int64_t)p.tiles_ci * p.tiles_co * a.KH * a.KW * p.splits)), blk(THREADS);
  if (wgrad_stages(p.tm, p.tn) == 3) RIGL_K_LAUNCH((k_wgrad_tr<2, 2, 3>), grid, blk, 0, st, a);
  else if (p.tm == 2) RIGL_K_LAUNCH((k_wgrad_tr<2, 1, 4>), grid, blk, 0, st, a);
  else if (p.tn == 2) RIGL_K_LAUNCH((k_wgrad_tr<1, 2, 4>), grid, blk, 0, st, a);
  else RIGL_K_LAUNCH((k_wgrad_tr<1, 1, 4>), grid, blk, 0, st, a);
  if (two_pass) {
    ReduceArgs ra = {reinterpret_cast<const float*>(ws), tiny_tmp ? tiny_tmp : dw, n_out, p.slab, p.splits};
    launch_wgrad_reduce(ra, st);
  }
  if (tiny_tmp)
    RIGL_K_LAUNCH(k_stem_unpack, dim3(64), blk, 0, st, tiny_tmp, dw, d->kh, d->kw, d->cin, tg.cred, d->cout, 0);
  RIGL_CHECK_LAUNCH("rigl_masked_conv2d_wgrad");
  return RIGL_OK;
}

static int bwd_impl(const RiglConvDesc* d, const rigl_bf16* x, const rigl_bf16* dy, const rigl_bf16* w_hwio,
                    const rigl_bf16* addend, float* dw, rigl_bf16* dx, void* workspace, size_t workspace_bytes,
                    const RiglBnReduceFuse* bn, rigl_stream_t stream, AddendSub sub = {1, 1},
                    const RiglConvDesc* dg = nullptr, const uint8_t* addend_bits = nullptr, int epi = rigl::k1::EPI_NONE);

int rigl_masked_conv2d_bwd_bn(const RiglConvDesc* d, const rigl_bf16* x, const rigl_bf16* dy, const rigl_bf16* w_hwio,
                              const rigl_bf16* addend, float* dw, rigl_bf16* dx, void* workspace, size_t workspace_bytes,
                              const RiglBnReduceFuse* bn, rigl_stream_t stream) {
  if (bn && !dx) return rigl::fail(RIGL_EINVAL, "rigl_masked_conv2d_bwd_bn: the reductions ride on dX, which was not requested");
  return bwd_impl(d, x, dy, w_hwio, addend, dw, dx, workspace, workspace_bytes, bn, stream);
}

static int bwd_impl(const RiglConvDesc* d, const rigl_bf16* x, const rigl_bf16* dy, const rigl_bf16* w_hwio,
                    const rigl_bf16* addend, float* dw, rigl_bf16* dx, void* workspace, size_t workspace_bytes,
                    const RiglBnReduceFuse* bn, rigl_stream_t stream, AddendSub sub, const RiglConvDesc* dg,
                    const uint8_t* addend_bits, int epi) {
  using namespace rigl;
  using namespace rigl::k1;
  static const bool fuse = [] { const char* e = getenv("RIGL_BWD_FUSED"); return e ? atoi(e) != 0 : true; }();
  const RiglConvDesc* dd = dg ? dg : d;
  int rc = check_desc(d, "rigl_masked_conv2d_bwd");
  if (rc) return rc;
  hipStream_t st = as_stream(stream);
  prof_set_tag(d);
  const bool subadd = addend_is_sub(addend, sub);
  if (subadd && bn) return fail(RIGL_EUNSUPPORTED, "rigl_masked_conv2d_bwd: a subsampled addend and the batch-norm reductions do not combine");
  if (subadd && !dx) return fail(RIGL_EINVAL, "rigl_masked_conv2d_bwd: an addend without dX");
  const bool both = dx && x && dy && w_hwio && dw;
  const bool whole = both && !subadd && !dg;
  const size_t need = rigl_conv2d_workspace_bytes(d, 2);
  bool dgrad_pp = false;
  if (dx && (d->cin % 8) == 0 && (d->cout % 8) == 0 && !bn && !subadd && !dg) {
    const IgemmArgs ap = dgrad_args(d, dy, w_hwio, addend, dx);
    dgrad_pp = plan_pp<1>(ap).variant != 0;
  }
  if (whole && !bn && bwd1x1_kind(d) && bwd1x1_ready(d)) {
    if (need && (!workspace || workspace_bytes < need))
      return fail(RIGL_EWORKSPACE, "rigl_masked_conv2d_bwd: workspace %zu < %zu", workspace_bytes, need);
    ProfFamily prof(PROF_CONV_BWD);
    if (launch_bwd1x1(d, x, dy, w_hwio, addend, dx, static_cast<float*>(workspace), st)) {
      const int64_t n_out = (int64_t)d->cin * d->cout;
      ReduceArgs ra = {static_cast<const float*>(workspace), dw, n_out, n_out, bwd1x1_splits()};
      launch_wgrad_reduce(ra, st);
      RIGL_CHECK_LAUNCH("rigl_masked_conv2d_bwd");
      return RIGL_OK;
    }
  }
  {
    BsPlan bp;
    if (both && !dg && !bn && bs_use(d, &bp)) {
      if (need && (!workspace || workspace_bytes < need))
        return fail(RIGL_EWORKSPACE, "rigl_masked_conv2d_bwd: workspace %zu < %zu", workspace_bytes, need);
      ProfFamily prof(PROF_CONV_BWD);
      launch_bs(d, bp, x, dy, w_hwio, addend, dx, static_cast<float*>(workspace), st, sub.sh, sub.sw, addend_bits);
      const int64_t n_out = (int64_t)d->cin * d->cout;
      ReduceArgs ra = {static_cast<const float*>(workspace), dw, n_out, n_out, bp.G};
      launch_wgrad_reduce(ra, st);
      RIGL_CHECK_LAUNCH("rigl_masked_conv2d_bwd");
      return RIGL_OK;
    }
  }
  if (addend_bits) return fail(RIGL_EUNSUPPORTED, "rigl_masked_conv2d_bwd_masked: this layer's kernels take no masked addend (ask rigl_conv2d_bwd_takes_masked_addend)");
  {
    RsPlan rp;
    if (whole && !bn && rs_use<1>(d, &rp)) {
      ProfFamily prof(PROF_CONV_BWD);
      rc = rigl_masked_conv2d_wgrad(d, x, dy, dw, workspace, workspace_bytes, stream);
      if (rc) return rc;
      prof_current_kind() = PROF_CONV_BWD;
      launch_rs<1>(d, rp, dy, w_hwio, addend, dx, nullptr, st);
      RIGL_CHECK_LAUNCH("rigl_masked_conv2d_bwd");
      return RIGL_OK;
    }
  }
  if (whole && !bn && c3x3_use(d)) {
    if (need && (!workspace || workspace_bytes < need))
      return fail(RIGL_EWORKSPACE, "rigl_masked_conv2d_bwd: workspace %zu < %zu", workspace_bytes, need);
    ProfFamily prof(PROF_CONV_BWD);
    float* slabs = static_cast<float*>(workspace);
    launch_c3x3_wgrad(d, x, dy, slabs, st);
    ReduceArgs ra = {slabs, dw, (int64_t)9 * 64 * 64, (int64_t)9 * 64 * 64, c3x3_wgrad_geom(d).grid};
    launch_wgrad_reduce(ra, st);
    launch_c3x3<true>(d, dy, w_hwio, addend, dx, nullptr, st);
    RIGL_CHECK_LAUNCH("rigl_masked_conv2d_bwd");
    return RIGL_OK;
  }
  if (RIGL_TUNE("pp_bwd", -1) != 0 && both && !subadd && !bn && !tiny_cin(d) && !small_cin(d) && pp_wgrad_legal(d)) {
    IgemmArgs ad = dgrad_args(dd, dy, w_hwio, addend, dx);
    const int dvar = RIGL_TUNE("pp_dgrad", -1) >= 0 ? PP_NONE : pp_bwd_dgrad_variant(ad);
    if (dvar != PP_NONE && pp_legal<1>(ad, dvar)) {
      int bm, bn2;
      pp_dims(dvar, bm, bn2);
      const bool strided = pp_strided(ad);
      const int tiles_m = strided ? pp_fill_classes(ad, bm) : (ad.M + bm - 1) / bm;
      const unsigned nd = (unsigned)(tiles_m * (ad.N / bn2));
      const int kt_d = (int)((int64_t)dd->kh * dd->kw * (dd->cout / 64) * bm * bn2 / (256 * 256) / (dd->stride_h * dd->stride_w));
      const PPBwdPlan pw = plan_wgrad_pp(d, nd, kt_d);
      if (need && (!workspace || workspace_bytes < need))
        return fail(RIGL_EWORKSPACE, "rigl_masked_conv2d_bwd: workspace %zu < %zu", workspace_bytes, need);
      ProfFamily prof(PROF_CONV_BWD);
      const WgradArgs aw = pp_wgrad_args(d, x, dy, pw, dw, workspace);
      ad.fd_rw = make_fastdiv(ad.RW); ad.fd_rh = make_fastdiv(ad.RH);
      ad.tiles_n = ad.N / bn2;
      if (epi == EPI_RELU ? pp_bwd_launch<EPI_RELU>(dvar, strided, ad, aw, pw, st) : pp_bwd_launch(dvar, strided, ad, aw, pw, st)) {
        if (pw.splits > 1) {
          ReduceArgs ra = {static_cast<const float*>(workspace), dw, pw.slab, pw.slab, pw.splits};
          launch_wgrad_reduce(ra, st);
        }
        RIGL_CHECK_LAUNCH("rigl_masked_conv2d_bwd");
        return RIGL_OK;
      }
    }
  }
  if (fuse && !dgrad_pp && both && !tiny_cin(d) && !small_cin(d) && (d->cin % 8) == 0 && (d->cout % 8) == 0) {
    IgemmArgs ad = dgrad_args(dd, dy, w_hwio, addend, dx);
    if (subadd) set_addend_sub(ad, dd, sub);
    rc = attach_bn(ad, d, bn);
    if (rc) return rc;
    const IgemmPlan pd = plan_igemm<1>(ad);
    WgradArgs aw = {};
    aw.interleave = RIGL_TUNE("wgrad_il", 1);
    aw.DY = dy; aw.M = d->n * d->ho * d->wo; aw.Cout = d->cout;
    aw.dy_bytes = (uint32_t)((size_t)aw.M * d->cout * 2);
    aw.X = x; aw.Cin = d->cin; aw.x_pix_stride = d->cin; aw.KH = d->kh; aw.KW = d->kw; aw.H = d->h; aw.W = d->w;
    aw.Ho = d->ho; aw.Wo = d->wo; aw.sh = d->stride_h; aw.sw = d->stride_w; aw.ph = d->pad_top; aw.pw = d->pad_left;
    aw.x_bytes = (uint32_t)((size_t)d->n * d->h * d->w * d->cin * 2);
    const WgradPlan p = plan_wgrad(aw.M, aw.Cin, aw.Cout, aw.KH * aw.KW, true);
    if (pd.dma) {
      if (need && (!workspace || workspace_bytes < need))
        return fail(RIGL_EWORKSPACE, "rigl_masked_conv2d_bwd: workspace %zu < %zu", workspace_bytes, need);
      ProfFamily prof(PROF_CONV_BWD);
      aw.tiles_ci = p.tiles_ci; aw.tiles_co = p.tiles_co; aw.splits = p.splits; aw.slab_elems = p.slab;
      const bool two_pass = p.splits > 1;
      aw.OUT = two_pass ? static_cast<float*>(workspace) : dw;
      const unsigned nd = pd.grid, nw = (unsigned)((int64_t)p.tiles_ci * p.tiles_co * aw.KH * aw.KW * p.splits);
      const dim3 grid(nd + nw), blk(THREADS);
#define RIGL_FUSED(KB, TND, CLSD)                                                                                      \
      {                                                                                                                \
        if (p.tm == 2 && p.tn == 2) RIGL_K_LAUNCH((KB<TND, CLSD, 2, 2, 3>), grid, blk, 0, st, ad, aw, nd, nw);          \
        else if (p.tm == 2) RIGL_K_LAUNCH((KB<TND, CLSD, 2, 1, 4>), grid, blk, 0, st, ad, aw, nd, nw);                   \
        else if (p.tn == 2) RIGL_K_LAUNCH((KB<TND, CLSD, 1, 2, 4>), grid, blk, 0, st, ad, aw, nd, nw);                   \
        else RIGL_K_LAUNCH((KB<TND, CLSD, 1, 1, 4>), grid, blk, 0, st, ad, aw, nd, nw);                                  \
      }
      if (epi == EPI_RELU) {
        if (pd.wide_n) { if (pd.cls) RIGL_FUSED(k_bwd_fused_relu, 2, true) else RIGL_FUSED(k_bwd_fused_relu, 2, false) }
        else { if (pd.cls) RIGL_FUSED(k_bwd_fused_relu, 1, true) else RIGL_FUSED(k_bwd_fused_relu, 1, false) }
      } else {
        if (pd.wide_n) { if (pd.cls) RIGL_FUSED(k_bwd_fused, 2, true) else RIGL_FUSED(k_bwd_fused, 2, false) }
        else { if (pd.cls) RIGL_FUSED(k_bwd_fused, 1, true) else RIGL_FUSED(k_bwd_fused, 1, false) }
      }
#undef RIGL_FUSED
      if (two_pass) {
        const int64_t n_out = (int64_t)d->kh * d->kw * d->cin * d->cout;
        ReduceArgs ra = {static_cast<const float*>(workspace), dw, n_out, p.slab, p.splits};
        launch_wgrad_reduce(ra, st);
      }
      RIGL_CHECK_LAUNCH("rigl_masked_conv2d_bwd");
      return RIGL_OK;
    }
  }
  rc = rigl_masked_conv2d_wgrad(d, x, dy, dw, workspace, workspace_bytes, stream);
  if (rc || !dx) return rc;
  return dgrad_impl(dd, dy, w_hwio, addend, dx, bn, stream, sub, epi);
}

int32_t rigl_conv2d_bwd_takes_relu_epilogue(const RiglConvDesc* d) {
  using namespace rigl;
  using namespace rigl::k1;
  if (!d || check_desc(d, "rigl_conv2d_bwd_takes_relu_epilogue")) return 0;
  return relu_dgrad_fusable(d) ? 1 : 0;
}

int rigl_masked_conv2d_bwd_relu(const RiglConvDesc* d, const rigl_bf16* x, const rigl_bf16* dy, const rigl_bf16* w_hwio,
                                float* dw, rigl_bf16* dx, void* workspace, size_t workspace_bytes, rigl_stream_t stream) {
  using namespace rigl;
  using namespace rigl::k1;
  int rc = check_desc(d, "rigl_masked_conv2d_bwd_relu");
  if (rc) return rc;
  if (!x || !dy || !w_hwio || !dw || !dx) return fail(RIGL_EINVAL, "rigl_masked_conv2d_bwd_relu: NULL tensor");
  if ((d->cin % 8) || (d->cout % 8)) return fail(RIGL_EUNSUPPORTED, "rigl_masked_conv2d_bwd_relu: cin/cout %% 8 != 0");
  if (relu_dgrad_fusable(d))
    return bwd_impl(d, x, dy, w_hwio, x, dw, dx, workspace, workspace_bytes, nullptr, stream, AddendSub{1, 1}, nullptr, nullptr, EPI_RELU);
  rc = bwd_impl(d, x, dy, w_hwio, nullptr, dw, dx, workspace, workspace_bytes, nullptr, stream);
  if (rc) return rc;
  return relu_bwd_launch((int64_t)d->n * d->h * d->w * d->cin, dx, x, dx, as_stream(stream));
}

int rigl_masked_conv2d_bwd(const RiglConvDesc* d, const rigl_bf16* x, const rigl_bf16* dy, const rigl_bf16* w_hwio,
                           const rigl_bf16* addend, float* dw, rigl_bf16* dx, void* workspace, size_t workspace_bytes,
                           rigl_stream_t stream) {
  return bwd_impl(d, x, dy, w_hwio, addend, dw, dx, workspace, workspace_bytes, nullptr, stream);
}

int32_t rigl_conv2d_bwd_takes_masked_addend(const RiglConvDesc* d) {
  using namespace rigl;
  using namespace rigl::k1;
  if (!d || check_desc(d, "rigl_conv2d_bwd_takes_masked_addend")) return 0;
  return bs_use(d) ? 1 : 0;
}
int rigl_masked_conv2d_bwd_masked(const RiglConvDesc* d, const rigl_bf16* x, const rigl_bf16* dy, const rigl_bf16* w_hwio,
                                  const rigl_bf16* addend, const uint8_t* addend_bits, float* dw, rigl_bf16* dx,
                                  void* workspace, size_t workspace_bytes, rigl_stream_t stream) {
  if (!addend || !addend_bits || !dx) return rigl::fail(RIGL_EINVAL, "rigl_masked_conv2d_bwd_masked: addend, addend_bits and dx are required");
  return bwd_impl(d, x, dy, w_hwio, addend, dw, dx, workspace, workspace_bytes, nullptr, stream, AddendSub{1, 1}, nullptr, addend_bits);
}

int rigl_masked_conv2d_bwd_grid(const RiglConvDesc* d, const rigl_bf16* x, const rigl_bf16* dy, const rigl_bf16* w_hwio,
                                float* dw, rigl_bf16* dx_grid, void* workspace, size_t workspace_bytes, rigl_stream_t stream) {
  using namespace rigl;
  using namespace rigl::k1;
  int rc = check_desc(d, "rigl_masked_conv2d_bwd_grid");
  if (rc) return rc;
  if (d->kh != 1 || d->kw != 1 || d->pad_top || d->pad_left || d->ho != (d->h + d->stride_h - 1) / d->stride_h ||
      d->wo != (d->w + d->stride_w - 1) / d->stride_w)
    return fail(RIGL_EUNSUPPORTED, "rigl_masked_conv2d_bwd_grid: a 1x1 conv without padding whose output grid is every stride-th pixel");
  if (!x || !dy || !w_hwio || !dw || !dx_grid) return fail(RIGL_EINVAL, "rigl_masked_conv2d_bwd_grid: NULL tensor");
  if ((d->cin % 8) || (d->cout % 8)) return fail(RIGL_EUNSUPPORTED, "rigl_masked_conv2d_bwd_grid: cin/cout %% 8 != 0");
  RiglConvDesc g = *d;
  g.h = d->ho; g.w = d->wo; g.stride_h = g.stride_w = 1;
  return bwd_impl(d, x, dy, w_hwio, nullptr, dw, dx_grid, workspace, workspace_bytes, nullptr, stream, AddendSub{1, 1}, &g);
}

int rigl_masked_conv2d_bwd_sub(const RiglConvDesc* d, const rigl_bf16* x, const rigl_bf16* dy, const rigl_bf16* w_hwio,
                               const rigl_bf16* addend, int32_t sub_h, int32_t sub_w, float* dw, rigl_bf16* dx,
                               void* workspace, size_t workspace_bytes, rigl_stream_t stream) {
  if (sub_h < 1 || sub_w < 1) return rigl::fail(RIGL_EINVAL, "rigl_masked_conv2d_bwd_sub: subsampling factors must be >= 1");
  return bwd_impl(d, x, dy, w_hwio, addend, dw, dx, workspace, workspace_bytes, nullptr, stream, AddendSub{sub_h, sub_w});
}


int rigl_probe_mfma_bf16(int32_t blocks, int32_t iters, float* sink, rigl_stream_t stream) {
  using namespace rigl;
  using namespace rigl::k1;
  if (blocks <= 0 || iters <= 0 || !sink) return fail(RIGL_EINVAL, "rigl_probe_mfma_bf16: bad argument");
  hipLaunchKernelGGL(k_mfma_probe, dim3((unsigned)blocks), dim3(THREADS), 0, as_stream(stream), sink, (int)iters, 0.5f);
  RIGL_CHECK_LAUNCH("rigl_probe_mfma_bf16");
  return RIGL_OK;
}

}
```

### rigl_amd/csrc/rowstream.hpp

```cpp
#pragma once

struct RsArgs {
  const uint16_t* A;
  const uint16_t* B;
  uint16_t* C;
  const uint16_t* ADD;
  float* STATS;
  int M, N;
  int F, nfrag;
  int slices, gprime;
  uint32_t a_bytes, b_bytes, c_bytes;
  unsigned long long* TRACE;
  const float* BNP;
  uint16_t* A2;
  const float* EPS;
};
#ifdef RIGL_RS_TRACE
#define RS_STAMP(i_) { if (tid == 0 && P.TRACE && (i_) < 64) P.TRACE[blockIdx.x * 64 + (i_)] = __builtin_amdgcn_s_memtime(); }
#else
#define RS_STAMP(i_) { }
#endif

constexpr int RS_THREADS = 512;

__device__ __forceinline__ uint32_t rs_add_bf16x2(uint32_t a, uint32_t b) {
  const f32x2 s = {__uint_as_float(a << 16) + __uint_as_float(b << 16),
                   __uint_as_float(a & 0xFFFF0000u) + __uint_as_float(b & 0xFFFF0000u)};
  return __builtin_bit_cast(uint32_t, __builtin_convertvector(s, bf16x2));
}

typedef __attribute__((ext_vector_type(4))) float rs_f32x4;
__device__ __forceinline__ u32x4 rs_bnrelu(bf16x8 v, const float* ps, int K, bool rowok) {
  const rs_f32x4 s0 = *reinterpret_cast<const rs_f32x4*>(ps), s1 = *reinterpret_cast<const rs_f32x4*>(ps + 4);
  const rs_f32x4 h0 = *reinterpret_cast<const rs_f32x4*>(ps + K), h1 = *reinterpret_cast<const rs_f32x4*>(ps + K + 4);
  u32x4 w = __builtin_bit_cast(u32x4, v);
#pragma unroll
  for (int d = 0; d < 4; ++d) {
    const float sa = d < 2 ? s0[2 * d] : s1[2 * d - 4], sb = d < 2 ? s0[2 * d + 1] : s1[2 * d - 3];
    const float ha = d < 2 ? h0[2 * d] : h1[2 * d - 4], hb = d < 2 ? h0[2 * d + 1] : h1[2 * d - 3];
    const f32x2 y = {fmaxf(fmaf(__uint_as_float(w[d] << 16), sa, ha), 0.f), fmaxf(fmaf(__uint_as_float(w[d] & 0xFFFF0000u), sb, hb), 0.f)};
    w[d] = rowok ? __builtin_bit_cast(uint32_t, __builtin_convertvector(y, bf16x2)) : 0u;
  }
  return w;
}

template <int KC, int TN>
struct RsGeom {
  static constexpr int K = 64 * KC, NS = 32 * TN, RB = K * 2, CPR = K / 8;
  static constexpr int WBYTES = NS * RB;
  static constexpr int SROW = NS * 2 + 8, STG_WAVE = 32 * SROW;
  static constexpr int SMEM = WBYTES + 8 * STG_WAVE;
  static constexpr int SMEM_BNL = SMEM + 2 * K * 4;
  static_assert(8 * STG_WAVE >= 8 * 64 * 16 * 4, "the statistics hand-off re-uses the staging tiles");
};

constexpr int RS_EPI_EVAL = 8, RS_EPI_BN = 1, RS_EPI_RES = 2, RS_EPI_RELU = 4;
template <int KC, int TN, int MODE, bool BNL = false, int EPI = 0>
__global__ __launch_bounds__(RS_THREADS) void k_rowstream(RsArgs P) {
  static_assert(!BNL || MODE == 0, "the on-load transform belongs to the forward");
  static_assert(EPI == 0 || (MODE == 0 && (EPI & RS_EPI_EVAL)), "the eval epilogue belongs to the forward");
  constexpr bool EVAL = EPI != 0, EBN = (EPI & RS_EPI_BN) != 0, ERES = EBN && (EPI & RS_EPI_RES), ERELU = EBN && (EPI & RS_EPI_RELU);
  constexpr bool DGRAD = MODE != 0, ADDEND = MODE == 2 || ERES, STATS = !DGRAD && !EVAL, A2OUT = BNL && !EVAL;
  using G = RsGeom<KC, TN>;
  constexpr int NS = G::NS, RB = G::RB, CPR = G::CPR, SROW = G::SROW;
  constexpr int CHR = 4 * TN, RPI = 64 / CHR, ITERS = 32 / RPI;
  constexpr int U = KC >= 4 ? 1 : 4 / KC;
  extern __shared__ __attribute__((aligned(1024))) unsigned char smem_rs[];
  const int tid = threadIdx.x, lane = tid & 63;
  const int wave = __builtin_amdgcn_readfirstlane(tid >> 6);
  const int hi = lane >> 5, r31 = lane & 31;
  RS_STAMP(0);
  const int xcd = (int)(blockIdx.x & 7u), idx = (int)(blockIdx.x >> 3);
  const int slice = idx % P.slices, gp = xcd + 8 * (idx / P.slices);
  const int slots = 8 * P.gprime, ws = gp * 8 + wave;
  const __amdgpu_buffer_rsrc_t rsrcA = make_rsrc(P.A, P.a_bytes), rsrcB = make_rsrc(P.B, P.b_bytes);
  const __amdgpu_buffer_rsrc_t rsrcD = make_rsrc(ADDEND ? P.ADD : P.A, ADDEND ? P.c_bytes : 0u);
  const __amdgpu_buffer_rsrc_t rsrcC = make_rsrc(P.C, P.c_bytes);

  float* const prm = reinterpret_cast<float*>(smem_rs + G::SMEM);
  const __amdgpu_buffer_rsrc_t rsrcA2 = make_rsrc(A2OUT ? P.A2 : P.C, A2OUT ? P.a_bytes : 0u);
  if (BNL) {
    for (int i = tid; i < 2 * G::K; i += RS_THREADS) prm[i] = P.BNP[i];
    asm volatile("s_waitcnt lgkmcnt(0)" ::: "memory");
    __builtin_amdgcn_sched_barrier(0);
  }
#define RS_SWZ(row_) (CPR == 8 ? (((row_) >> 1) & 7) : ((row_) & 15))
  {
    constexpr int PIECES = G::WBYTES / 1024, PPW = PIECES / 8;
    static_assert(PIECES % 8 == 0, "whole rounds of eight waves");
#pragma unroll
    for (int j = 0; j < PPW; ++j) {
      const int piece = j * 8 + wave, p = piece * 64 + lane, row = p / CPR, ch = p % CPR;
      const int src = ((slice * NS + row) * CPR + (ch ^ RS_SWZ(row))) * 16;
      __builtin_amdgcn_raw_ptr_buffer_load_lds(rsrcB, (__attribute__((address_space(3))) void*)(smem_rs + piece * 1024), 16, src, 0, 0, 0);
    }
  }
  __builtin_amdgcn_sched_barrier(0);
  const uint32_t a_lane = r31 < P.F ? (uint32_t)(r31 * RB + hi * 16) : OOB;
  auto row_off = [&](int ii) -> uint32_t {
    return a_lane + (uint32_t)__builtin_amdgcn_readfirstlane((ws + ii * slots) * P.F * RB);
  };
  bf16x8 a[4][4];
#define RS_LOAD_CHUNK(slot_, ii_, c_)                                                                    \
  {                                                                                                      \
    const uint32_t o_ = row_off(ii_) + (uint32_t)((c_) * 128);                                           \
    _Pragma("unroll") for (int k4 = 0; k4 < 4; ++k4)                                                     \
      a[slot_][k4] = __builtin_bit_cast(bf16x8, buf_load16(rsrcA, o_ + (uint32_t)(k4 * 32)));            \
  }
#pragma unroll
  for (int s = 0; s < 4; ++s) RS_LOAD_CHUNK(s, s / KC, s % KC);
  __builtin_amdgcn_sched_barrier(0);
  asm volatile("s_waitcnt vmcnt(16)" ::: "memory");
  __builtin_amdgcn_s_barrier();
  asm volatile("" ::: "memory");
  RS_STAMP(1);

  const int swz = RS_SWZ(r31);
  const unsigned char* const bs = smem_rs + r31 * RB;
  unsigned char* const stg = smem_rs + G::WBYTES + wave * G::STG_WAVE;
  float sS[8], sQ[8];
#pragma unroll
  for (int e = 0; e < 8; ++e) sS[e] = sQ[e] = 0.f;
  const int ni = ws < P.nfrag ? (P.nfrag - ws + slots - 1) / slots : 0;
  const int srow = lane / CHR, sch = lane % CHR;
  if constexpr (EBN) {
    const float* const ps = P.EPS + slice * NS + sch * 8;
#pragma unroll
    for (int e = 0; e < 8; ++e) { sS[e] = ps[e]; sQ[e] = ps[P.N + e]; }
  }
  uint32_t c_lane[ITERS];
#pragma unroll
  for (int it = 0; it < ITERS; ++it)
    c_lane[it] = it * RPI + srow < P.F ? (uint32_t)(((it * RPI + srow) * P.N + slice * NS + sch * 8) * 2) : OOB;

  for (int i0 = 0; i0 < ni; i0 += U) {
#pragma unroll
    for (int u = 0; u < U; ++u) {
      const int ii = i0 + u;
      const int fr = ws + ii * slots;
      const int row0 = fr * P.F;
      RS_STAMP(2 + 3 * ii);
      uint32_t coff[ITERS];
      const uint32_t c_base = (uint32_t)__builtin_amdgcn_readfirstlane(row0 * P.N * 2);
#pragma unroll
      for (int it = 0; it < ITERS; ++it) coff[it] = c_lane[it] + c_base;
      uint4 addv[ITERS];
      if (ADDEND) {
#pragma unroll
        for (int it = 0; it < ITERS; ++it) addv[it] = buf_load16(rsrcD, coff[it]);
      }
      f32x16 acc[TN];
#pragma unroll
      for (int j = 0; j < TN; ++j)
#pragma unroll
        for (int e = 0; e < 16; ++e) acc[j][e] = 0.f;
      {
        constexpr int S = KC * 4;
        bf16x8 bq[2][TN];
#define RS_READ(s_, buf_)                                                                                \
        _Pragma("unroll") for (int j = 0; j < TN; ++j)                                                   \
          bq[buf_][j] = *reinterpret_cast<const bf16x8*>(bs + j * 32 * RB + ((((2 * (s_) + hi)) ^ swz) << 4));
        RS_READ(0, 0);
        RS_READ(1, 1);
        const bool rowok = BNL && r31 < P.F && row0 + r31 < P.M;
#define RS_BNL(st_)                                                                                      \
        {                                                                                                \
          const int c_ = (st_) / 4, g_ = (st_) % 4, slot_ = (u * KC + c_) & 3;                           \
          const u32x4 w_ = rs_bnrelu(a[slot_][g_], prm + c_ * 64 + g_ * 16 + hi * 8, G::K, rowok);       \
          a[slot_][g_] = __builtin_bit_cast(bf16x8, w_);                                                 \
          if (A2OUT && (c_ % P.slices) == slice)                                                         \
            __builtin_amdgcn_raw_buffer_store_b128(w_, rsrcA2, (int)(row_off(ii) + (uint32_t)(c_ * 128 + g_ * 32)), 0, 0); \
        }
        if (BNL) RS_BNL(0);
        __builtin_amdgcn_sched_barrier(0);
#pragma unroll
        for (int st = 0; st < S; ++st) {
          const int c = st / 4, g4 = st % 4;
          const int t = u * KC + c;
          const int slot = t & 3;
#pragma unroll
          for (int j = 0; j < TN; ++j)
#if defined(RIGL_RS_ABLATE) && (RIGL_RS_ABLATE & 8)
            acc[j][0] += (float)bq[st & 1][j][0] + (float)a[slot][g4][0];
#else
            acc[j] = __builtin_amdgcn_mfma_f32_32x32x16_bf16(bq[st & 1][j], a[slot][g4], acc[j], 0, 0, 0);
#endif
#if !(defined(RIGL_RS_ABLATE) && (RIGL_RS_ABLATE & 64))
          if (st + 2 < S) RS_READ(st + 2, st & 1);
#endif
          if (BNL && st + 1 < S) RS_BNL(st + 1);
          if (g4 == 3) {
            const int t4 = t + 4;
#if !(defined(RIGL_RS_ABLATE) && (RIGL_RS_ABLATE & 1))
            RS_LOAD_CHUNK(slot, i0 + t4 / KC, t4 % KC);
#endif
          }
          __builtin_amdgcn_sched_barrier(0);
        }
#undef RS_READ
#undef RS_BNL
      }
      RS_STAMP(3 + 3 * ii);
#pragma unroll
      for (int j = 0; j < TN; ++j)
#pragma unroll
        for (int q = 0; q < 4; ++q) {
          const f32x2 lo = {acc[j][4 * q], acc[j][4 * q + 1]}, hi2 = {acc[j][4 * q + 2], acc[j][4 * q + 3]};
          uint2 pk;
          pk.x = __builtin_bit_cast(uint32_t, __builtin_convertvector(lo, bf16x2));
          pk.y = __builtin_bit_cast(uint32_t, __builtin_convertvector(hi2, bf16x2));
#if defined(RIGL_RS_ABLATE) && (RIGL_RS_ABLATE & 32)
          if (pk.x == 0x12345678u)
#endif
          *reinterpret_cast<uint2*>(stg + r31 * SROW + (j * 32 + 8 * q + 4 * hi) * 2) = pk;
        }
#pragma unroll
      for (int g0 = 0; g0 < ITERS; g0 += 4) {
        uint4 v[4];
#pragma unroll
        for (int i4 = 0; i4 < 4; ++i4) {
          const unsigned char* const p = stg + ((g0 + i4) * RPI + srow) * SROW + sch * 16;
          const uint2 lo8 = *reinterpret_cast<const uint2*>(p), hi8 = *reinterpret_cast<const uint2*>(p + 8);
          v[i4] = make_uint4(lo8.x, lo8.y, hi8.x, hi8.y);
        }
        if constexpr (EBN) {
#pragma unroll
          for (int i4 = 0; i4 < 4; ++i4) {
            u32x4 w4 = {v[i4].x, v[i4].y, v[i4].z, v[i4].w};
            const u32x4 r4 = ERES ? u32x4{addv[g0 + i4].x, addv[g0 + i4].y, addv[g0 + i4].z, addv[g0 + i4].w} : u32x4{0u, 0u, 0u, 0u};
#pragma unroll
            for (int d = 0; d < 4; ++d) {
              float y0 = fmaf(__uint_as_float(w4[d] << 16), sS[2 * d], sQ[2 * d]);
              float y1 = fmaf(__uint_as_float(w4[d] & 0xFFFF0000u), sS[2 * d + 1], sQ[2 * d + 1]);
              if (ERES) { y0 += __uint_as_float(r4[d] << 16); y1 += __uint_as_float(r4[d] & 0xFFFF0000u); }
              if (ERELU) { y0 = fmaxf(y0, 0.f); y1 = fmaxf(y1, 0.f); }
              const f32x2 yy = {y0, y1};
              w4[d] = __builtin_bit_cast(uint32_t, __builtin_convertvector(yy, bf16x2));
            }
            v[i4] = make_uint4(w4[0], w4[1], w4[2], w4[3]);
          }
        } else if (ADDEND) {
#pragma unroll
          for (int i4 = 0; i4 < 4; ++i4) {
            const uint4 q4 = addv[g0 + i4];
            v[i4].x = rs_add_bf16x2(v[i4].x, q4.x); v[i4].y = rs_add_bf16x2(v[i4].y, q4.y);
            v[i4].z = rs_add_bf16x2(v[i4].z, q4.z); v[i4].w = rs_add_bf16x2(v[i4].w, q4.w);
          }
        }
#pragma unroll
        for (int i4 = 0; i4 < 4; ++i4) {
          const u32x4 o = {v[i4].x, v[i4].y, v[i4].z, v[i4].w};
#if defined(RIGL_RS_ABLATE) && (RIGL_RS_ABLATE & 2)
          if (o.x == 0x12345678u)
#endif
          __builtin_amdgcn_raw_buffer_store_b128(o, rsrcC, (int)coff[g0 + i4], 0, 0);
        }
#if defined(RIGL_RS_ABLATE) && (RIGL_RS_ABLATE & 4)
        if (false) {
#else
        if (STATS) {
#endif
#pragma unroll
          for (int i4 = 0; i4 < 4; ++i4)
#pragma unroll
            for (int d = 0; d < 4; ++d) {
              const uint32_t w2 = dword_of(v[i4], d);
              const float y0 = __uint_as_float(w2 << 16), y1 = __uint_as_float(w2 & 0xFFFF0000u);
              sS[2 * d] += y0; sQ[2 * d] += y0 * y0;
              sS[2 * d + 1] += y1; sQ[2 * d + 1] += y1 * y1;
            }
        }
        __builtin_amdgcn_sched_barrier(0);
      }
      __builtin_amdgcn_sched_barrier(0);
      asm volatile("" ::: "memory");
      RS_STAMP(4 + 3 * ii);
    }
  }
  RS_STAMP(62);
#undef RS_LOAD_CHUNK
#undef RS_SWZ
  if (STATS && P.STATS) {
    __syncthreads();
    float* const area = reinterpret_cast<float*>(smem_rs + G::WBYTES);
#pragma unroll
    for (int e = 0; e < 8; ++e) {
      area[(wave * 64 + lane) * 16 + e] = sS[e];
      area[(wave * 64 + lane) * 16 + 8 + e] = sQ[e];
    }
    __syncthreads();
    if (tid < 2 * NS) {
      const int k = tid / NS, n = tid % NS, ch = n / 8, e = n % 8;
      float v[8 * RPI];
#pragma unroll
      for (int w8 = 0; w8 < 8; ++w8)
#pragma unroll
        for (int q = 0; q < RPI; ++q) v[w8 * RPI + q] = area[(w8 * 64 + q * CHR + ch) * 16 + k * 8 + e];
      float s = 0.f;
#pragma unroll
      for (int i = 0; i < 8 * RPI; ++i) s += v[i];
      P.STATS[((int64_t)gp * 2 + k) * P.N + slice * NS + n] = s;
    }
  }
  RS_STAMP(63);
}

struct RsPlan { int kc, tn, slices, gprime, F, nfrag; };
template <int MODE>
static bool rs_plan(const RiglConvDesc* d, RsPlan& p) {
  if (d->kh != 1 || d->kw != 1 || d->stride_h != 1 || d->stride_w != 1 || d->pad_top || d->pad_left) return false;
  if (d->ho != d->h || d->wo != d->w) return false;
  const int k = MODE == 0 ? d->cin : d->cout, n = MODE == 0 ? d->cout : d->cin;
  if (k != 64 && k != 128 && k != 256 && k != 512) return false;
  p.kc = k / 64;
  p.tn = (k <= 256 && n % 128 == 0) ? 4 : 2;
  const int ns = 32 * p.tn;
  if (n % ns) return false;
  p.slices = n / ns;
  if (p.slices > 32 || (p.slices & (p.slices - 1))) return false;
  const int64_t M = (int64_t)d->n * d->h * d->w;
  if (M < 4096 || M * (k > n ? k : n) * 2 >= (1ll << 30)) return false;
  int groups = num_cus() / (8 * p.slices);
  if (groups < 1) groups = 1;
  p.gprime = 8 * groups;
  const int slots = 8 * p.gprime;
  const int passes = (int)((M + 32ll * slots - 1) / (32ll * slots));
  p.F = (int)((M + (int64_t)slots * passes - 1) / ((int64_t)slots * passes));
  if (p.F > 32) p.F = 32;
  if (p.F < 8) p.F = 8;
  p.nfrag = (int)((M + p.F - 1) / p.F);
  return true;
}
template <int KC, int TN, int MODE>
static bool rs_ready_i() {
  static const bool ready = hipFuncSetAttribute(reinterpret_cast<const void*>(&k_rowstream<KC, TN, MODE>),
                                                hipFuncAttributeMaxDynamicSharedMemorySize, RsGeom<KC, TN>::SMEM) == hipSuccess;
  return ready;
}
template <int KC, int TN>
static bool rs_ready_bnl() {
  static const bool ready = hipFuncSetAttribute(reinterpret_cast<const void*>(&k_rowstream<KC, TN, 0, true>),
                                                hipFuncAttributeMaxDynamicSharedMemorySize, RsGeom<KC, TN>::SMEM_BNL) == hipSuccess;
  return ready;
}
#define RS_DISPATCH(p_, DG_, WHAT_)                                                                      \
  switch ((p_).kc * 8 + (p_).tn) {                                                                       \
    case 1 * 8 + 2: { WHAT_(1, 2, DG_); } break;                                                         \
    case 1 * 8 + 4: { WHAT_(1, 4, DG_); } break;                                                         \
    case 2 * 8 + 2: { WHAT_(2, 2, DG_); } break;                                                         \
    case 2 * 8 + 4: { WHAT_(2, 4, DG_); } break;                                                         \
    case 4 * 8 + 2: { WHAT_(4, 2, DG_); } break;                                                         \
    case 4 * 8 + 4: { WHAT_(4, 4, DG_); } break;                                                         \
    case 8 * 8 + 2: { WHAT_(8, 2, DG_); } break;                                                         \
    default: break;                                                                                      \
  }
template <int MODE>
static bool rs_default(const RiglConvDesc* d, const RsPlan& p) {
  const int k = MODE == 0 ? d->cin : d->cout, n = MODE == 0 ? d->cout : d->cin;
  const int64_t M = (int64_t)d->n * d->h * d->w;
  if (MODE == 0) return k <= 256 && p.slices <= 8 && M >= 25088;
  return k == 64 && n == 256;
}
template <int MODE>
static bool rs_use(const RiglConvDesc* d, RsPlan* out = nullptr) {
  RsPlan p;
  if (!rs_plan<MODE>(d, p)) return false;
  const int knob = RIGL_TUNE("rowstream", 1);
  if (knob == 0 || (knob == 1 && !rs_default<MODE>(d, p))) return false;
  bool ready = false;
#define RS_READY(KC_, TN_, DG_) ready = rs_ready_i<KC_, TN_, DG_>();
  if (MODE == 0) { RS_DISPATCH(p, 0, RS_READY) } else { RS_DISPATCH(p, 1, RS_READY) if (ready) { RS_DISPATCH(p, 2, RS_READY) } }
#undef RS_READY
  if (ready && out) *out = p;
  return ready;
}
template <int MODE>
static void launch_rs(const RiglConvDesc* d, const RsPlan& p, const rigl_bf16* a_act, const rigl_bf16* b_w, const rigl_bf16* addend,
                      rigl_bf16* c_out, float* stats, hipStream_t st) {
  RsArgs a = {};
#ifdef RIGL_RS_TRACE
  { const char* e = getenv("RIGL_RS_TRACE_PTR"); a.TRACE = e ? reinterpret_cast<unsigned long long*>(strtoull(e, nullptr, 0)) : nullptr; }
#endif
  const int k = MODE == 0 ? d->cin : d->cout, n = MODE == 0 ? d->cout : d->cin;
  a.A = a_act; a.B = b_w; a.C = c_out; a.ADD = addend; a.STATS = stats;
  a.M = d->n * d->h * d->w; a.N = n; a.F = p.F; a.nfrag = p.nfrag; a.slices = p.slices; a.gprime = p.gprime;
  a.a_bytes = (uint32_t)((size_t)a.M * k * 2); a.b_bytes = (uint32_t)((size_t)n * k * 2); a.c_bytes = (uint32_t)((size_t)a.M * n * 2);
  const dim3 grid((unsigned)(p.slices * p.gprime)), blk(RS_THREADS);
#define RS_LAUNCH(KC_, TN_, DG_) RIGL_K_LAUNCH((k_rowstream<KC_, TN_, DG_>), grid, blk, (unsigned)(RsGeom<KC_, TN_>::SMEM), st, a);
  if (MODE == 0) { RS_DISPATCH(p, 0, RS_LAUNCH) } else if (addend) { RS_DISPATCH(p, 2, RS_LAUNCH) } else { RS_DISPATCH(p, 1, RS_LAUNCH) }
#undef RS_LAUNCH
}

static bool rs_bnl_use(const RiglConvDesc* d, RsPlan* out = nullptr) {
  RsPlan p;
  if (!RIGL_TUNE("bn_on_load", 1) || !rs_use<0>(d, &p)) return false;
  if (p.kc == 1 && p.tn == 4) return false;
  bool ready = false;
#define RS_READY(KC_, TN_, DG_) ready = rs_ready_bnl<KC_, TN_>();
  RS_DISPATCH(p, 0, RS_READY)
#undef RS_READY
  if (ready && out) *out = p;
  return ready;
}
static void launch_rs_bnl(const RiglConvDesc* d, const RsPlan& p, const rigl_bf16* x_pre, const float* scale_shift, rigl_bf16* a_out,
                          const rigl_bf16* w_ohwi, rigl_bf16* y, float* stats, hipStream_t st) {
  RsArgs a = {};
  a.A = x_pre; a.B = w_ohwi; a.C = y; a.STATS = stats; a.BNP = scale_shift; a.A2 = a_out;
  a.M = d->n * d->h * d->w; a.N = d->cout; a.F = p.F; a.nfrag = p.nfrag; a.slices = p.slices; a.gprime = p.gprime;
  a.a_bytes = (uint32_t)((size_t)a.M * d->cin * 2); a.b_bytes = (uint32_t)((size_t)d->cout * d->cin * 2);
  a.c_bytes = (uint32_t)((size_t)a.M * d->cout * 2);
  const dim3 grid((unsigned)(p.slices * p.gprime)), blk(RS_THREADS);
#define RS_LAUNCH(KC_, TN_, DG_) RIGL_K_LAUNCH((k_rowstream<KC_, TN_, 0, true>), grid, blk, (unsigned)(RsGeom<KC_, TN_>::SMEM_BNL), st, a);
  RS_DISPATCH(p, 0, RS_LAUNCH)
#undef RS_LAUNCH
}

template <int KC, int TN, bool BNL, int EPI>
static bool rs_ready_eval() {
  static const bool ready = hipFuncSetAttribute(reinterpret_cast<const void*>(&k_rowstream<KC, TN, 0, BNL, EPI>),
                                                hipFuncAttributeMaxDynamicSharedMemorySize,
                                                BNL ? RsGeom<KC, TN>::SMEM_BNL : RsGeom<KC, TN>::SMEM) == hipSuccess;
  return ready;
}
#define RS_EVAL_PLAIN_true(WHAT_, KC_, TN_) WHAT_(KC_, TN_, true, RS_EPI_EVAL);
#define RS_EVAL_PLAIN_false(WHAT_, KC_, TN_)
#define RS_EVAL_RES_1(WHAT_, KC_, TN_, BNL_)                                                             \
    case RS_EPI_EVAL | RS_EPI_BN | RS_EPI_RES: { WHAT_(KC_, TN_, BNL_, RS_EPI_EVAL | RS_EPI_BN | RS_EPI_RES); } break;   \
    case RS_EPI_EVAL | RS_EPI_BN | RS_EPI_RES | RS_EPI_RELU:                                             \
      { WHAT_(KC_, TN_, BNL_, RS_EPI_EVAL | RS_EPI_BN | RS_EPI_RES | RS_EPI_RELU); } break;
#define RS_EVAL_RES_0(WHAT_, KC_, TN_, BNL_)
#define RS_EVAL_SWITCH(BNL_, epi_, WHAT_, KC_, TN_, RES_)                                                \
  switch (epi_) {                                                                                        \
    case RS_EPI_EVAL: { RS_EVAL_PLAIN_##BNL_(WHAT_, KC_, TN_) } break;                                  \
    case RS_EPI_EVAL | RS_EPI_BN: { WHAT_(KC_, TN_, BNL_, RS_EPI_EVAL | RS_EPI_BN); } break;             \
    case RS_EPI_EVAL | RS_EPI_BN | RS_EPI_RELU: { WHAT_(KC_, TN_, BNL_, RS_EPI_EVAL | RS_EPI_BN | RS_EPI_RELU); } break; \
    RS_EVAL_RES_##RES_(WHAT_, KC_, TN_, BNL_)                                                            \
    default: break;                                                                                      \
  }
#define RS_EVAL_DISPATCH(p_, bnl_, epi_, WHAT_)                                                          \
  switch ((p_).kc * 8 + (p_).tn) {                                                                       \
    case 1 * 8 + 2: { if (bnl_) { RS_EVAL_SWITCH(true, epi_, WHAT_, 1, 2, 1) } else { RS_EVAL_SWITCH(false, epi_, WHAT_, 1, 2, 1) } } break; \
    case 1 * 8 + 4: { if (!(bnl_)) { RS_EVAL_SWITCH(false, epi_, WHAT_, 1, 4, 1) } } break;              \
    case 2 * 8 + 2: { if (bnl_) { RS_EVAL_SWITCH(true, epi_, WHAT_, 2, 2, 1) } else { RS_EVAL_SWITCH(false, epi_, WHAT_, 2, 2, 1) } } break; \
    case 2 * 8 + 4: { if (bnl_) { RS_EVAL_SWITCH(true, epi_, WHAT_, 2, 4, 0) } else { RS_EVAL_SWITCH(false, epi_, WHAT_, 2, 4, 1) } } break; \
    case 4 * 8 + 2: { if (bnl_) { RS_EVAL_SWITCH(true, epi_, WHAT_, 4, 2, 1) } else { RS_EVAL_SWITCH(false, epi_, WHAT_, 4, 2, 1) } } break; \
    case 4 * 8 + 4: { if (bnl_) { RS_EVAL_SWITCH(true, epi_, WHAT_, 4, 4, 0) } else { RS_EVAL_SWITCH(false, epi_, WHAT_, 4, 4, 1) } } break; \
    case 8 * 8 + 2: { if (bnl_) { RS_EVAL_SWITCH(true, epi_, WHAT_, 8, 2, 1) } else { RS_EVAL_SWITCH(false, epi_, WHAT_, 8, 2, 1) } } break; \
    default: break;                                                                                      \
  }
static int rs_eval_epi(bool bn, bool residual, bool relu) {
  return RS_EPI_EVAL | (bn ? RS_EPI_BN | (residual ? RS_EPI_RES : 0) | (relu ? RS_EPI_RELU : 0) : 0);
}
static bool rs_eval_use(const RiglConvDesc* d, bool bnl, int epi, RsPlan* out = nullptr) {
  RsPlan p;
  if (!RIGL_TUNE("eval_fuse", 1)) return false;
  if (bnl ? !rs_bnl_use(d, &p) : !rs_use<0>(d, &p)) return false;
  if (!bnl && !(epi & RS_EPI_BN)) return false;
  if (bnl && (epi & RS_EPI_RES) && p.tn == 4) return false;
  bool ready = false;
#define RS_READY(KC_, TN_, BNL_, EPI_) ready = rs_ready_eval<KC_, TN_, BNL_, EPI_>();
  RS_EVAL_DISPATCH(p, bnl, epi, RS_READY)
#undef RS_READY
  if (ready && out) *out = p;
  return ready;
}
static void launch_rs_eval(const RiglConvDesc* d, const RsPlan& p, int epi, const rigl_bf16* x, const float* bnl_scale_shift,
                           const rigl_bf16* w_ohwi, const float* scale_shift, const rigl_bf16* residual, rigl_bf16* y, hipStream_t st) {
  RsArgs a = {};
  const bool bnl = bnl_scale_shift != nullptr;
  a.A = x; a.B = w_ohwi; a.C = y; a.ADD = residual; a.BNP = bnl_scale_shift; a.EPS = scale_shift;
  a.M = d->n * d->h * d->w; a.N = d->cout; a.F = p.F; a.nfrag = p.nfrag; a.slices = p.slices; a.gprime = p.gprime;
  a.a_bytes = (uint32_t)((size_t)a.M * d->cin * 2); a.b_bytes = (uint32_t)((size_t)d->cout * d->cin * 2);
// ... 9 lines not shown
```

### rigl_amd/ops.py

```python
import ctypes as C
import os

import torch

from rigl_amd import _lib
from rigl_amd._lib import (ConvDesc, PackLayer, PruneRegrowLayer,
                           PruneRegrowParams, RiglError, check)

_workspaces = {}


_raw_stream = getattr(torch._C, '_cuda_getCurrentRawStream', None)
_cur_device = getattr(torch._C, '_cuda_getDevice', None)


def _stream():
  if _raw_stream is not None and _cur_device is not None:
    return C.c_void_p(_raw_stream(_cur_device()))
  return C.c_void_p(torch.cuda.current_stream().cuda_stream)


def _ptr(t):
  return C.c_void_p(t.data_ptr()) if t is not None else C.c_void_p(0)

# ... 432 lines not shown
        raise ValueError('%s must be [2, %d] (or a [4, %d] saved block)' % (nm, c, c))
  if x.numel() != d.n * d.h * d.w * d.cin:
    raise ValueError('x must be [n, h, w, Cin] of the descriptor')
  _req(residual, torch.bfloat16, 'residual', allow_none=True)
  if residual is not None and residual.numel() != d.n * d.ho * d.wo * d.cout:
    raise ValueError('residual must have the shape of the output')
  if y is None:
    y = torch.empty((d.n, d.ho, d.wo, d.cout), dtype=torch.bfloat16, device=x.device)
  _req(y, torch.bfloat16, 'y')
  if conv_fwd_takes_bn_epilogue(d, in_ss is not None, residual is not None):
    _count_macs('fwd_macs', d)
    check(_lib.load().rigl_masked_conv2d_fwd_bn_infer(
        C.byref(d), _ptr(x), _ptr(in_ss[-2] if in_ss is not None else None), _ptr(w_ohwi),
        _ptr(ss[-2] if ss is not None else None), _ptr(residual), int(bool(relu)), _ptr(y), _stream()))
    return y
  if in_ss is not None:
    x = bn_apply(x, in_ss, relu=True)
    if ss is not None and conv_fwd_takes_bn_epilogue(d, False, residual is not None):
      return _conv_fwd_infer(d, x, None, w_ohwi, ss, residual, relu, y)
  if ss is None:
    return conv_fwd(d, x, w_ohwi, y)
  return bn_apply(conv_fwd(d, x, w_ohwi), ss, relu=relu, residual=residual, y=y)


def conv_dgrad(d, dy, w_hwio, dx=None, force_ref=False, addend=None):
  _count_macs('dgrad_macs', d)
  _req(dy, torch.bfloat16, 'dy')
  _req(w_hwio, torch.bfloat16, 'w_hwio')
  if dx is None:
    dx = torch.empty((d.n, d.h, d.w, d.cin), dtype=torch.bfloat16,
                     device=dy.device)
  _req(dx, torch.bfloat16, 'dx')
  if addend is not None:
    _req(addend, torch.bfloat16, 'addend')
    if addend.numel() != dx.numel():
      raise ValueError('addend must have the shape of dx')
  lib = _lib.load()
  if force_ref or not mfma_dgrad_supported(d):
    check(lib.rigl_conv2d_dgrad_ref(C.byref(d), _ptr(dy), _ptr(w_hwio),
                                    _ptr(dx), _stream()))
    if addend is not None:
      dx += addend.view_as(dx)
    return dx
  check(lib.rigl_masked_conv2d_dgrad_acc(C.byref(d), _ptr(dy), _ptr(w_hwio),
                                         _ptr(addend), _ptr(dx), None, 0,
                                         _stream()))
  return dx


def conv_wgrad(d, x, dy, dw=None, force_ref=False):
  _count_macs('wgrad_macs', d)
  _req(x, torch.bfloat16, 'x')
  _req(dy, torch.bfloat16, 'dy')
  if dw is None:
    dw = torch.empty(d.kh * d.kw * d.cin * d.cout, dtype=torch.float32,
                     device=x.device)
  _req(dw, torch.float32, 'dw')
  lib = _lib.load()
  if force_ref or not mfma_supported(d):
    check(lib.rigl_conv2d_wgrad_ref(C.byref(d), _ptr(x), _ptr(dy), _ptr(dw),
                                    _stream()))
    return dw
  need = lib.rigl_conv2d_workspace_bytes(C.byref(d), 2)
  ws = workspace(need, x.device) if need else None
  check(lib.rigl_masked_conv2d_wgrad(C.byref(d), _ptr(x), _ptr(dy), _ptr(dw),
                                     _ptr(ws),
                                     ws.numel() if ws is not None else 0,
                                     _stream()))
  return dw


def dgrad_stats_parts(d):
  v = _plan_cached(d, 'dgrad_parts', lambda: int(_lib.load().rigl_conv2d_dgrad_stats_parts(C.byref(d))))
  return v


LAZY_ADDEND_BITS = {}


def conv_bwd_takes_masked_addend(d):
  return bool(_plan_cached(d, 'masked_addend', lambda: int(_lib.load().rigl_conv2d_bwd_takes_masked_addend(C.byref(d)))))


def conv_bwd(d, x, dy, w_hwio, dw, need_dx=True, addend=None, on_dw_ready=None, bn_fuse=None, addend_sub=None,
             addend_bits=None, dx=None):
  if addend_sub is not None and tuple(addend_sub) == (1, 1):
    addend_sub = None
  if addend_bits is not None:
    if addend is None or not need_dx or bn_fuse is not None or addend_sub is not None or not conv_bwd_takes_masked_addend(d):
      raise ValueError('addend_bits needs an addend, dX and a layer whose backward takes a masked addend')
    _req(x, torch.bfloat16, 'x'); _req(dy, torch.bfloat16, 'dy'); _req(dw, torch.float32, 'dw')
    _req(addend, torch.bfloat16, 'addend'); _req(addend_bits, torch.uint8, 'addend_bits'); _req(w_hwio, torch.bfloat16, 'w_hwio')
    if addend.numel() != d.n * d.h * d.w * d.cin or addend_bits.numel() * 8 != addend.numel():
      raise ValueError('addend must have the shape of dx and addend_bits one bit per element of it')
    lib = _lib.load()
    _count_macs('wgrad_macs', d)
    _count_macs('dgrad_macs', d)
    need = _plan_cached(d, 'ws_wgrad', lambda: lib.rigl_conv2d_workspace_bytes(C.byref(d), 2))
    ws = workspace(need, x.device, 'wg') if need else None
    dx = _out(dx, (d.n, d.h, d.w, d.cin), torch.bfloat16, dy.device, 'dx')
    check(lib.rigl_masked_conv2d_bwd_masked(C.byref(d), _ptr(x), _ptr(dy), _ptr(w_hwio), _ptr(addend), _ptr(addend_bits), _ptr(dw),
                                            _ptr(dx), _ptr(ws), ws.numel() if ws is not None else 0, _stream()))
    if on_dw_ready is not None:
      on_dw_ready()
    return dx
  if addend_sub is not None:
    if addend is None or not need_dx or bn_fuse is not None:
      raise ValueError('addend_sub needs an addend and dX, and does not combine with bn_fuse')
    if not (mfma_supported(d) and mfma_dgrad_supported(d)):
      raise ValueError('addend_sub needs cin % 8 == cout % 8 == 0')
  if bn_fuse is not None:
    bn_fuse.pop('partials', None)
    if not (need_dx and mfma_supported(d) and mfma_dgrad_supported(d) and dgrad_stats_parts(d) > 0):
      bn_fuse = None
  if not (mfma_supported(d) and (not need_dx or mfma_dgrad_supported(d))):
    conv_wgrad(d, x, dy, dw)
    if on_dw_ready is not None:
      on_dw_ready()
    return conv_dgrad(d, dy, w_hwio, dx=dx, addend=addend) if need_dx else None
  _req(x, torch.bfloat16, 'x')
  _req(dy, torch.bfloat16, 'dy')
  _req(dw, torch.float32, 'dw')
  _req(addend, torch.bfloat16, 'addend', allow_none=True)
  lib = _lib.load()
  _count_macs('wgrad_macs', d)
  if need_dx:
    _count_macs('dgrad_macs', d)
  need = _plan_cached(d, 'ws_wgrad', lambda: lib.rigl_conv2d_workspace_bytes(C.byref(d), 2))
  ws = workspace(need, x.device, 'wg') if need else None
  if not need_dx:
    dx = None
  else:
    _req(w_hwio, torch.bfloat16, 'w_hwio')
    dx = _out(dx, (d.n, d.h, d.w, d.cin), torch.bfloat16, dy.device, 'dx')
    if addend is not None and addend_sub is None and addend.numel() != dx.numel():
      raise ValueError('addend must have the shape of dx')
  if addend_sub is not None:
    sh, sw = addend_sub
    if addend.numel() != d.n * (-(-d.h // sh)) * (-(-d.w // sw)) * d.cin:
      raise ValueError('addend must be [n, ceil(h / sh), ceil(w / sw), cin]')
    check(lib.rigl_masked_conv2d_bwd_sub(
        C.byref(d), _ptr(x), _ptr(dy), _ptr(w_hwio), _ptr(addend), int(sh), int(sw), _ptr(dw), _ptr(dx), _ptr(ws),
        ws.numel() if ws is not None else 0, _stream()))
    if on_dw_ready is not None:
      on_dw_ready()
    return dx
  bn = None
  if bn_fuse is not None:
    bx, saved = bn_fuse['x'], bn_fuse['saved']
    _req(bx, torch.bfloat16, 'bn x')
    _req(saved, torch.float32, 'bn saved')
    bits = bn_fuse.get('relu_bits')
    _req(bits, torch.uint8, 'bn relu_bits', allow_none=True)
    if bx.numel() != dx.numel() or saved.numel() != 4 * d.cin:
      raise ValueError('bn_fuse: x must have the shape of dx and saved must be [4, Cin]')
    part = torch.empty((dgrad_stats_parts(d), 2, d.cin), dtype=torch.float32, device=dy.device)
    bn = _lib.BnReduceFuse(bx.data_ptr(), bits.data_ptr() if bits is not None else None, saved.data_ptr(),
                           int(bool(bn_fuse['relu'])), part.data_ptr(), part.numel())
    bn_fuse['partials'] = part
  check(lib.rigl_masked_conv2d_bwd_bn(
      C.byref(d), _ptr(x), _ptr(dy), _ptr(w_hwio), _ptr(addend), _ptr(dw), _ptr(dx), _ptr(ws),
      ws.numel() if ws is not None else 0, C.byref(bn) if bn is not None else None, _stream()))
  if on_dw_ready is not None:
    on_dw_ready()
  return dx


def conv_bwd_grid(d, x, dy, w_hwio, dw, on_dw_ready=None, dx=None):
  _req(x, torch.bfloat16, 'x')
  _req(dy, torch.bfloat16, 'dy')
  _req(w_hwio, torch.bfloat16, 'w_hwio')
  _req(dw, torch.float32, 'dw')
  lib = _lib.load()
# ... 125 lines not shown
    parts = _plan_cached(d, 'dw_parts', lambda: int(lib.rigl_depthwise_conv2d_stats_parts(C.byref(d))))
    if parts > 0:
      part = _stats_out(part, parts, d.cout, x.device)
      check(lib.rigl_depthwise_conv2d_fwd_stats(C.byref(d), _ptr(x), _ptr(w), _ptr(y), _ptr(part), part.numel(), _stream()))
      return y, part
  check(lib.rigl_depthwise_conv2d_fwd(C.byref(d), _ptr(x), _ptr(w), _ptr(y), _stream()))
  return (y, None) if stats else y


def depthwise_dgrad(d, dy, w, dx=None):
  _count_depthwise(d)
  _req(dy, torch.bfloat16, 'dy')
  _req(w, torch.float32, 'w')
  dx = _out(dx, (d.n, d.h, d.w, d.cin), torch.bfloat16, dy.device, 'dx')
  check(_lib.load().rigl_depthwise_conv2d_dgrad(C.byref(d), _ptr(dy), _ptr(w), _ptr(dx), _stream()))
  return dx


def depthwise_wgrad(d, x, dy, dw):
  _count_depthwise(d)
  _req(x, torch.bfloat16, 'x')
  _req(dy, torch.bfloat16, 'dy')
  _req(dw, torch.float32, 'dw')
  lib = _lib.load()
  ws = workspace(lib.rigl_depthwise_conv2d_workspace_bytes(C.byref(d)), x.device)
  check(lib.rigl_depthwise_conv2d_wgrad(C.byref(d), _ptr(x), _ptr(dy), _ptr(dw), _ptr(ws), ws.numel(), _stream()))
  return dw


def bn_fwd(x, gamma, beta, running_mean, running_var, momentum, eps, relu,
           residual=None, partials=None, want_relu_bits=False):
  _req(x, torch.bfloat16, 'x')
  _req(residual, torch.bfloat16, 'residual', allow_none=True)
  for t, nm in ((gamma, 'gamma'), (beta, 'beta')):
    _req(t, torch.float32, nm)
  c = x.shape[-1]
  m = x.numel() // c
  lib = _lib.load()
  y = torch.empty_like(x)
  saved = torch.empty((4, c), dtype=torch.float32, device=x.device)
  bits = torch.empty(x.numel() // 8, dtype=torch.uint8, device=x.device) \
      if (want_relu_bits and relu) else None
  if partials is not None:
    _req(partials, torch.float32, 'partials')
    if partials.dim() != 3 or partials.shape[1] != 2 or partials.shape[2] != c:
      raise ValueError('partials must be [parts, 2, C]')
    ws = None
  else:
    ws = workspace(lib.rigl_bn_workspace_bytes(m, c), x.device)
  check(lib.rigl_bn_fwd_stats(
      m, c, _ptr(x), _ptr(residual), _ptr(gamma), _ptr(beta),
      _ptr(running_mean), _ptr(running_var), float(momentum), float(eps),
      int(bool(relu)), _ptr(y), _ptr(saved[0]), _ptr(saved[1]), _ptr(saved[2]),
      _ptr(saved[3]), _ptr(partials),
      partials.shape[0] if partials is not None else 0, _ptr(bits), _ptr(ws),
      ws.numel() if ws is not None else 0, _stream()))
  return (y, saved, bits) if want_relu_bits else (y, saved)


def bn_bwd(x, y, dy, gamma, saved, relu, dgamma, dbeta, want_dres=False,
           relu_bits=None, partials=None):
  _req(relu_bits, torch.uint8, 'relu_bits', allow_none=True)
  _req(x, torch.bfloat16, 'x')
  _req(dy, torch.bfloat16, 'dy')
  _req(y, torch.bfloat16, 'y', allow_none=True)
  c = x.shape[-1]
  m = x.numel() // c
  lib = _lib.load()
  dx = torch.empty_like(x)
  dres = torch.empty_like(x) if want_dres else None
  ws = workspace(lib.rigl_bn_workspace_bytes(m, c), x.device)
  _req(partials, torch.float32, 'partials', allow_none=True)
  if partials is not None and (partials.dim() != 3 or partials.shape[1] != 2 or partials.shape[2] != c):
    raise ValueError('partials must be [parts, 2, %d]' % c)
  check(lib.rigl_bn_bwd_stats(m, c, _ptr(x), _ptr(y), _ptr(relu_bits), _ptr(dy), _ptr(gamma),
                              _ptr(saved[0]), _ptr(saved[1]), _ptr(saved[2]),
                              _ptr(saved[3]), int(bool(relu)), _ptr(dx), _ptr(dres),
                              _ptr(dgamma), _ptr(dbeta), _ptr(partials),
                              partials.shape[0] if partials is not None else 0, _ptr(ws), ws.numel(),
                              _stream()))
  return dx, dres


def stateless_random(n, seed0, seed1, dist, scale=1.0, shift=0.0, device=None,
                     out=None):
  def i32(v):
    v = int(v) & 0xFFFFFFFF
    return v - (1 << 32) if v >= 1 << 31 else v
  if dist not in ('uniform', 'normal'):
    raise ValueError('dist must be "uniform" or "normal"')
  if out is None:
    out = torch.empty(int(n), dtype=torch.float32, device=device)
  _req(out, torch.float32, 'out')
  check(_lib.load().rigl_stateless_random(_ptr(out), out.numel(), i32(seed0), i32(seed1),
                                          1 if dist == 'normal' else 0,
                                          float(scale), float(shift), _stream()))
  return out


def stateless_random_batched(items, device):
  def i32(v):
    v = int(v) & 0xFFFFFFFF
    return v - (1 << 32) if v >= 1 << 31 else v
  if not items:
    return []
  offs, total = [], 0
  for it in items:
    offs.append(total)
    total += (int(it[0]) + 63) // 64 * 64
  buf = torch.empty(max(total, 1), dtype=torch.float32, device=device)
  arr = (_lib.RandomItem * len(items))()
  outs = []
  for i, (n, s0, s1, dist, scale, shift) in enumerate(items):
    if dist not in ('uniform', 'normal'):
      raise ValueError('dist must be "uniform" or "normal"')
    t = buf[offs[i]:offs[i] + int(n)]
    outs.append(t)
    arr[i].out = t.data_ptr() if int(n) else None
    arr[i].n = int(n)
    arr[i].seed0, arr[i].seed1 = i32(s0), i32(s1)
    arr[i].dist = 1 if dist == 'normal' else 0
    arr[i].scale, arr[i].shift = float(scale), float(shift)
  check(_lib.load().rigl_stateless_random_batched(arr, len(items), _stream()))
  return outs


def maxpool_fwd(d, x):
  _req(x, torch.bfloat16, 'x')
  y = torch.empty((d.n, d.ho, d.wo, d.cout), dtype=torch.bfloat16, device=x.device)
  arg = torch.empty((d.n, d.ho, d.wo, d.cout), dtype=torch.uint8, device=x.device)
  check(_lib.load().rigl_maxpool_fwd(C.byref(d), _ptr(x), _ptr(y), _ptr(arg), _stream()))
  return y, arg


def maxpool_bwd(d, dy, arg):
  _req(dy, torch.bfloat16, 'dy')
  _req(arg, torch.uint8, 'argmax')
  dx = torch.empty((d.n, d.h, d.w, d.cin), dtype=torch.bfloat16, device=dy.device)
  check(_lib.load().rigl_maxpool_bwd(C.byref(d), _ptr(dy), _ptr(arg), _ptr(dx), _stream()))
  return dx


def bn_statistics(x, gamma, beta, running_mean, running_var, momentum, eps, partials=None):
  _req(x, torch.bfloat16, 'x')
  c = x.shape[-1]
  m = x.numel() // c
  lib = _lib.load()
  saved = torch.empty((4, c), dtype=torch.float32, device=x.device)
  if partials is not None:
    _req(partials, torch.float32, 'partials')
    ws = None
  else:
    ws = workspace(lib.rigl_bn_workspace_bytes(m, c), x.device)
  check(lib.rigl_bn_fwd_statistics(
      m, c, _ptr(x), _ptr(gamma), _ptr(beta), _ptr(running_mean), _ptr(running_var), float(momentum), float(eps),
      _ptr(saved[0]), _ptr(saved[1]), _ptr(saved[2]), _ptr(saved[3]), _ptr(partials),
      partials.shape[0] if partials is not None else 0, _ptr(ws), ws.numel() if ws is not None else 0, _stream()))
  return saved


def bn_add_bn_fwd(x, x2, saved2, gamma, beta, running_mean, running_var, momentum, eps, relu, partials=None):
  _req(x, torch.bfloat16, 'x')
  _req(x2, torch.bfloat16, 'x2')
  if x2.shape != x.shape:
    raise ValueError('x2 must have the shape of x')
  c = x.shape[-1]
# ... 231 lines not shown
```

### rigl_amd/pruning_layers.py

```python
import math
import os

import numpy as np
import torch

from rigl_amd import ops
from rigl_amd import variables as V


def _same_pad(size, k, stride):
  out = -(-size // stride)
  total = max((out - 1) * stride + k - size, 0)
  return out, total // 2


def _valid_out(size, k, stride):
  return (size - k) // stride + 1


_BN_FUSE_BWD = os.environ.get('RIGL_BN_FUSE_BWD', '0') == '1'
_CONV_PAIR = os.environ.get('RIGL_CONV_PAIR', '1') != '0'
_BN_FUSE_MAX_BYTES = float(os.environ.get('RIGL_BN_FUSE_MAX_MB', '1e9')) * 1e6


def _bn_source(x):
  h = getattr(x, 'bn_ctx', None) if _BN_FUSE_BWD else None
  if h is not None:
    h.attached += 1
  return h


def _bn_fuse_request(holder, need_dx):
  if holder is None or not need_dx or holder.attached != 1 or holder.x is None:
    return None
  if holder.x.numel() * 2 > _BN_FUSE_MAX_BYTES:
    return None
  return dict(x=holder.x, saved=holder.saved, relu=holder.relu, relu_bits=holder.bits)


def _bn_fuse_publish(holder, req, dx):
  if req is not None and req.get('partials') is not None and dx is not None:
    holder.partials, holder.dx_ptr = req['partials'], dx.data_ptr()


def _mask_bits(lv):
  return lv.mask.bits if lv.mask is not None else None


class _MaskedConvFn(torch.autograd.Function):

  @staticmethod
  def forward(ctx, x, lv, desc, need_dx, want_stats=False, bn_holder=None, pending=None):
    ctx.lv, ctx.desc, ctx.need_dx = lv, desc, need_dx
    ctx.bn_holder = bn_holder
    ctx.save_for_backward(x)
    if pending is not None:
      out = ops.conv_fwd_bnrelu(desc, pending.x, pending.saved, lv.ohwi, x, stats=want_stats)
      if not want_stats:
        return out
      y, part = out
      ctx.mark_non_differentiable(part)
      ctx.set_materialize_grads(False)
      return y, part
    if x.dtype == torch.float32:
      y = ops.conv_fwd_f32(desc, x, lv.weights.data.view(-1), _mask_bits(lv))
      if not want_stats:
        return y
      part = torch.empty(0, device=x.device)
      ctx.mark_non_differentiable(part)
      ctx.set_materialize_grads(False)
      return y, part
    if not want_stats:
      return ops.conv_fwd(desc, x, lv.ohwi)
    y, part = ops.conv_fwd(desc, x, lv.ohwi, stats=True)
    if part is None:
      part = torch.empty(0, device=x.device)
    ctx.mark_non_differentiable(part)
    ctx.set_materialize_grads(False)
    return y, part

  @staticmethod
  def backward(ctx, dy, _dpart=None):
    (x,) = ctx.saved_tensors
    lv, d = ctx.lv, ctx.desc
    if dy is None:
      dy = torch.zeros((d.n, d.ho, d.wo, d.cout), dtype=x.dtype, device=x.device)
    dy = dy.contiguous()
    sync = getattr(lv.weights.graph, 'grad_sync', None)
    ready = (lambda: sync.notify_layer_grad_ready(lv.weights)) if sync is not None else None
    if x.dtype == torch.float32:
      dx = ops.conv_bwd_f32(d, x, dy, lv.weights.data.view(-1), _mask_bits(lv), lv.weights.grad.view(-1),
                            need_dx=ctx.need_dx, on_dw_ready=ready)
      return dx, None, None, None, None, None, None
    req = _bn_fuse_request(ctx.bn_holder, ctx.need_dx)
    dx = ops.conv_bwd(d, x, dy, lv.hwio, lv.weights.grad.view(-1), need_dx=ctx.need_dx, on_dw_ready=ready, bn_fuse=req)
    _bn_fuse_publish(ctx.bn_holder, req, dx)
    return dx, None, None, None, None, None, None


class _MaskedConvReluFn(torch.autograd.Function):

  @staticmethod
  def forward(ctx, x, lv, desc, need_dx, gate_input):
    ctx.lv, ctx.desc, ctx.need_dx, ctx.gate_input = lv, desc, need_dx, gate_input
    ctx.save_for_backward(x)
    return ops.conv_fwd_relu(desc, x, lv.ohwi)

  @staticmethod
  def backward(ctx, dy):
    (x,) = ctx.saved_tensors
    lv, d = ctx.lv, ctx.desc
    dy = dy.contiguous()
    sync = getattr(lv.weights.graph, 'grad_sync', None)
    ready = (lambda: sync.notify_layer_grad_ready(lv.weights)) if sync is not None else None
    if ctx.need_dx and ctx.gate_input:
      dx = ops.conv_bwd_relu(d, x, dy, lv.hwio, lv.weights.grad.view(-1), on_dw_ready=ready)
    else:
      dx = ops.conv_bwd(d, x, dy, lv.hwio, lv.weights.grad.view(-1), need_dx=ctx.need_dx, on_dw_ready=ready)
    return dx, None, None, None, None


class _MaskedConvForkFn(torch.autograd.Function):

  @staticmethod
  def forward(ctx, x, lv, desc, want_stats=False, bn_holder=None):
    ctx.lv, ctx.desc = lv, desc
    ctx.bn_holder = bn_holder
    ctx.save_for_backward(x)
    if x.dtype == torch.float32:
      y = ops.conv_fwd_f32(desc, x, lv.weights.data.view(-1), _mask_bits(lv))
      if not want_stats:
        return y, x.view_as(x)
      part = torch.empty(0, device=x.device)
      ctx.mark_non_differentiable(part)
      ctx.set_materialize_grads(False)
      return y, x.view_as(x), part
    if not want_stats:
      return ops.conv_fwd(desc, x, lv.ohwi), x.view_as(x)
    y, part = ops.conv_fwd(desc, x, lv.ohwi, stats=True)
    if part is None:
      part = torch.empty(0, device=x.device)
    ctx.mark_non_differentiable(part)
    ctx.set_materialize_grads(False)
    return y, x.view_as(x), part

  @staticmethod
  def backward(ctx, dy, dalias, _dpart=None):
    (x,) = ctx.saved_tensors
    lv, d = ctx.lv, ctx.desc
    if dy is None:
      dy = torch.zeros((d.n, d.ho, d.wo, d.cout), dtype=x.dtype, device=x.device)
    dy = dy.contiguous()
    if dalias is not None:
      dalias = dalias.contiguous()
    sync = getattr(lv.weights.graph, 'grad_sync', None)
    ready = (lambda: sync.notify_layer_grad_ready(lv.weights)) if sync is not None else None
    if x.dtype == torch.float32:
      dx = ops.conv_bwd_f32(d, x, dy, lv.weights.data.view(-1), _mask_bits(lv), lv.weights.grad.view(-1),
                            need_dx=True, addend=dalias, on_dw_ready=ready)
      return dx, None, None, None, None
    lazy = ops.LAZY_ADDEND_BITS.pop(dalias.data_ptr(), None) if dalias is not None else None
    if lazy is not None:
      dx = ops.conv_bwd(d, x, dy, lv.hwio, lv.weights.grad.view(-1), need_dx=True, addend=dalias, addend_bits=lazy[0],
                        on_dw_ready=ready)
      return dx, None, None, None, None
    req = _bn_fuse_request(ctx.bn_holder, True)
    dx = ops.conv_bwd(d, x, dy, lv.hwio, lv.weights.grad.view(-1), need_dx=True, addend=dalias, on_dw_ready=ready, bn_fuse=req)
    _bn_fuse_publish(ctx.bn_holder, req, dx)
    return dx, None, None, None, None


class _MaskedConvPairFn(torch.autograd.Function):

  @staticmethod
  def forward(ctx, x, lv_s, d_s, lv_m, d_m, want_stats):
    ctx.lv_s, ctx.d_s, ctx.lv_m, ctx.d_m = lv_s, d_s, lv_m, d_m
# ... 44 lines not shown
  if not bn_stats:
    return _MaskedConvPairFn.apply(x.contiguous(), conv_sub.vars, d_s, conv_main.vars, d_m, False)
  ys, ym, ps, pm = _MaskedConvPairFn.apply(x.contiguous(), conv_sub.vars, d_s, conv_main.vars, d_m, True)
  if ps.numel():
    ys.bn_partials = ps
  if pm.numel():
    ym.bn_partials = pm
  return ys, ym


class _Layer:

  def __init__(self, graph, scope, shape, sparsity_technique, weight_decay,
               kernel_initializer):
    if sparsity_technique not in ('threshold', 'baseline'):
      raise ValueError(
          'Unsupported sparsity technique {}'.format(sparsity_technique))
    self.graph = graph
    self.scope = scope
    self.masked = sparsity_technique == 'threshold'
    init = kernel_initializer(shape) if kernel_initializer is not None else \
        variance_scaling_initializer()(shape)
    self.vars = graph.add_masked_layer(scope, shape, self.masked, weight_decay,
                                       init)
    self.bias = None

  @property
  def weights(self):
    return self.vars.weights

  @property
  def mask(self):
    return self.vars.mask


class MaskedConv2d(_Layer):

  def __init__(self, graph, scope, cin, units, kernel_size, strides=(1, 1),
               padding='SAME', sparsity_technique='baseline', weight_decay=0.0,
               kernel_initializer=None, need_input_grad=True):
    kh, kw = kernel_size
    super().__init__(graph, scope, (kh, kw, cin, units), sparsity_technique,
                     weight_decay, kernel_initializer)
    if padding not in ('SAME', 'VALID'):
      raise ValueError('padding must be SAME or VALID')
    self.cin, self.units, self.kh, self.kw = cin, units, kh, kw
    self.strides = tuple(strides)
    self.padding = padding
    self.need_input_grad = need_input_grad
    self._descs = {}

  def desc_for(self, n, h, w):
    key = (n, h, w)
    d = self._descs.get(key)
    if d is None:
      sh, sw = self.strides
      if self.padding == 'SAME':
        ho, pt = _same_pad(h, self.kh, sh)
        wo, pl = _same_pad(w, self.kw, sw)
      else:
        ho, pt = _valid_out(h, self.kh, sh), 0
        wo, pl = _valid_out(w, self.kw, sw), 0
      d = ops.conv_desc(n, h, w, self.cin, self.units, self.kh, self.kw,
                        (sh, sw), pt, pl, ho, wo)
      self._descs[key] = d
    return d

  def __call__(self, x, bn_stats=False):
    if x.dim() != 4:
      raise ValueError('Rank not supported {}'.format(x.dim()))
    if x.shape[-1] != self.cin:
      raise ValueError('expected %d input channels, got %d' %
                       (self.cin, x.shape[-1]))
    self.graph.refresh_shadows()
    n, h, w, _ = x.shape
    d = self.desc_for(n, h, w)
    need_dx = self.need_input_grad and x.requires_grad
    holder = _bn_source(x) if need_dx else None
    pending = getattr(x, 'bn_pending', None)
    if pending is not None and (pending.x is None or not x.is_contiguous()):
      raise RuntimeError('a deferred batch-norm output must reach its consumer conv as it was returned')
    if not x.requires_grad:
      x = x.detach().requires_grad_(True)
    if not bn_stats:
      return _MaskedConvFn.apply(x.contiguous(), self.vars, d, need_dx, False, holder, pending)
    y, part = _MaskedConvFn.apply(x.contiguous(), self.vars, d, need_dx, True, holder, pending)
    if part.numel():
      y.bn_partials = part
    return y

  def conv_relu(self, x, gate_input=True):
    if x.dim() != 4 or x.shape[-1] != self.cin:
      raise ValueError('expected [N,H,W,%d], got %s' % (self.cin, tuple(x.shape)))
    if x.dtype != torch.bfloat16:
      raise NotImplementedError('conv_relu: bf16 activations only')
    self.graph.refresh_shadows()
    n, h, w, _ = x.shape
    d = self.desc_for(n, h, w)
    need_dx = self.need_input_grad and x.requires_grad
    if not x.requires_grad:
      x = x.detach().requires_grad_(True)
    return _MaskedConvReluFn.apply(x.contiguous(), self.vars, d, need_dx, bool(gate_input))

  def takes_bn_input(self, x):
    if not (x.is_cuda and x.dtype == torch.bfloat16 and x.dim() == 4 and x.shape[-1] == self.cin):
      return False
    n, h, w, _ = x.shape
    return ops.conv_fwd_takes_bn_input(self.desc_for(n, h, w))

  def takes_masked_addend(self, x):
    if not (self.need_input_grad and x.requires_grad and x.dtype == torch.bfloat16 and x.dim() == 4) or _BN_FUSE_BWD:
      return False
    n, h, w, _ = x.shape
    return ops.conv_bwd_takes_masked_addend(self.desc_for(n, h, w))

  def fork(self, x, bn_stats=False):
    if x.dim() != 4 or x.shape[-1] != self.cin:
      raise ValueError('expected [N,H,W,%d], got %s' % (self.cin, tuple(x.shape)))
    if not (self.need_input_grad and x.requires_grad):
      return self(x, bn_stats), x
    self.graph.refresh_shadows()
    n, h, w, _ = x.shape
    holder = _bn_source(x)
    if not bn_stats:
      return _MaskedConvForkFn.apply(x.contiguous(), self.vars, self.desc_for(n, h, w), False, holder)
    y, alias, part = _MaskedConvForkFn.apply(x.contiguous(), self.vars, self.desc_for(n, h, w), True, holder)
    if part.numel():
      y.bn_partials = part
    return y, alias


class MaskedDense(_Layer):

  def __init__(self, graph, scope, n_in, units, use_bias=True,
               sparsity_technique='baseline', weight_decay=0.0,
               kernel_initializer=None, activation=None):
    super().__init__(graph, scope, (n_in, units), sparsity_technique,
                     weight_decay, kernel_initializer)
    self.n_in, self.units = n_in, units
    self.activation = activation
    self._descs = {}
    if use_bias:
      self.bias = graph.add_variable(scope + '/biases', (units,), V.KIND_OTHER, 0.0)

  def __call__(self, x):
    if x.shape[-1] != self.n_in:
      raise ValueError('expected %d inputs, got %d' % (self.n_in, x.shape[-1]))
    self.graph.refresh_shadows()
    lead = x.shape[:-1]
    x2 = x.reshape(-1, 1, 1, self.n_in)
    b = x2.shape[0]
    d = self._descs.get(b)
    if d is None:
      d = ops.conv_desc(b, 1, 1, self.n_in, self.units, 1, 1, 1, 0, 0, 1, 1)
      self._descs[b] = d
    need_dx = x2.requires_grad
    if not x2.requires_grad:
      x2 = x2.detach().requires_grad_(True)
    y = _MaskedConvFn.apply(x2.contiguous(), self.vars, d, need_dx)
    y = y.reshape(*lead, self.units)
    if self.bias is not None:
      y = y + bias_tensor(self.bias).to(y.dtype)
    if self.activation is not None:
      y = self.activation(y)
    return y


def bias_tensor(var):
  leaf = getattr(var, '_leaf', None)
  if leaf is None or leaf.data_ptr() != var.data.data_ptr():
    leaf = var.data.detach().requires_grad_(True)
# ... 105 lines not shown
```

### rigl_amd/workloads/nn.py

```python
import os

import torch
import torch.nn.functional as F

from rigl_amd import variables as V
from rigl_amd.pruning_layers import bias_tensor

BATCH_NORM_DECAY = 0.9
BATCH_NORM_EPSILON = 1e-5
_DW_STATS = os.environ.get('RIGL_DW_STATS', '1') != '0'


def activation_dtype(precision=None):
  if precision is None:
    from rigl_amd import ops
    precision = 'float32' if ops.tune_get('k1_fp32', 0) == 1 else 'bfloat16'
  if precision not in ('bfloat16', 'float32'):
    raise ValueError('precision must be bfloat16 or float32, got %r' % (precision,))
  return torch.float32 if precision == 'float32' else torch.bfloat16


def nchw_view(x):
  return x.permute(0, 3, 1, 2)


def nhwc_view(x):
  return x.permute(0, 2, 3, 1)


class _BnBwdHolder:
  __slots__ = ('x', 'saved', 'bits', 'relu', 'attached', 'partials', 'dx_ptr')

  def __init__(self, relu):
    self.x = self.saved = self.bits = self.partials = self.dx_ptr = None
    self.relu = relu
    self.attached = 0


_LAZY_RES_GRAD = os.environ.get('RIGL_LAZY_RES_GRAD', '1') != '0'
_BN_ON_LOAD = os.environ.get('RIGL_BN_ON_LOAD', '0') == '1'


class _FusedBNFn(torch.autograd.Function):

  @staticmethod
  def forward(ctx, x, residual, bn, relu, partials=None, holder=None, lazy_res_grad=False, defer=False):
    from rigl_amd import ops
    x = x.contiguous()
    res = residual.contiguous() if residual is not None else None
    ctx.bn, ctx.relu, ctx.has_res = bn, relu, res is not None
    ctx.holder = holder
    ctx.lazy_res_grad = bool(lazy_res_grad) and relu and res is not None
    if defer:
      saved = ops.bn_statistics(x, bn.gamma.data, bn.beta.data, bn.moving_mean, bn.moving_variance, 1.0 - bn.decay, bn.eps,
                                partials=partials)
      ctx.save_for_backward(x, saved)
      holder.x, holder.saved, holder.bits = x, saved, None
      return torch.empty_like(x)
    if relu and res is not None:
      y, saved, bits = ops.bn_fwd(x, bn.gamma.data, bn.beta.data, bn.moving_mean,
                                  bn.moving_variance, 1.0 - bn.decay, bn.eps, relu, res,
                                  partials=partials, want_relu_bits=True)
      ctx.save_for_backward(x, saved, bits)
    else:
      bits = None
      y, saved = ops.bn_fwd(x, bn.gamma.data, bn.beta.data, bn.moving_mean,
                            bn.moving_variance, 1.0 - bn.decay, bn.eps, relu, res,
                            partials=partials)
      ctx.save_for_backward(x, saved)
    if holder is not None:
      holder.x, holder.saved, holder.bits = x, saved, bits
    return y

  @staticmethod
  def backward(ctx, dy):
    from rigl_amd import ops
    bn = ctx.bn
    if ctx.relu and ctx.has_res:
      x, saved, bits = ctx.saved_tensors
    else:
      (x, saved), bits = ctx.saved_tensors, None
    dy = dy.contiguous()
    h, part = ctx.holder, None
    if h is not None:
      if h.partials is not None and h.dx_ptr == dy.data_ptr():
        part = h.partials
      h.partials = h.x = h.saved = h.bits = None
    if ctx.lazy_res_grad and bits is not None and ctx.needs_input_grad[1]:
      dx, _ = ops.bn_bwd(x, None, dy, bn.gamma.data, saved, ctx.relu, bn.gamma.grad, bn.beta.grad, want_dres=False,
                         relu_bits=bits, partials=part)
      ops.LAZY_ADDEND_BITS[dy.data_ptr()] = (bits, dy)
      return dx, dy, None, None, None, None, None, None
    dx, dres = ops.bn_bwd(x, None, dy, bn.gamma.data, saved, ctx.relu,
                          bn.gamma.grad, bn.beta.grad,
                          want_dres=ctx.has_res and ctx.needs_input_grad[1],
                          relu_bits=bits, partials=part)
    return dx, dres, None, None, None, None, None, None


class _BnAddBnFn(torch.autograd.Function):

  @staticmethod
  def forward(ctx, x, x2, bn, bn2, partials, partials2):
    from rigl_amd import ops
    x, x2 = x.contiguous(), x2.contiguous()
    saved2 = ops.bn_statistics(x2, bn2.gamma.data, bn2.beta.data, bn2.moving_mean, bn2.moving_variance,
                               1.0 - bn2.decay, bn2.eps, partials=partials2)
    y, saved, bits = ops.bn_add_bn_fwd(x, x2, saved2, bn.gamma.data, bn.beta.data, bn.moving_mean, bn.moving_variance,
                                       1.0 - bn.decay, bn.eps, True, partials=partials)
    ctx.bn, ctx.bn2 = bn, bn2
    ctx.save_for_backward(x, x2, saved, saved2, bits)
    return y

  @staticmethod
  def backward(ctx, dy):
    from rigl_amd import ops
    x, x2, saved, saved2, bits = ctx.saved_tensors
    bn, bn2 = ctx.bn, ctx.bn2
    dx, dx2 = ops.bn_add_bn_bwd(x, x2, bits, dy.contiguous(), bn.gamma.data, saved, bn2.gamma.data, saved2,
                                bn.gamma.grad, bn.beta.grad, bn2.gamma.grad, bn2.beta.grad)
    return dx, dx2, None, None, None, None


_BN_PAIR_FUSED = os.environ.get('RIGL_BN_PAIR', '1') != '0'


def bn_add_bn_relu(bn, x, bn2, x2, is_training=True):
  c = x.shape[-1]
  if (_BN_PAIR_FUSED and bn.fused and bn2.fused and is_training and x.is_cuda and x.dtype == torch.bfloat16
      and x2.dtype == torch.bfloat16 and x2.shape == x.shape and c % 8 == 0 and c <= 3968):
    px, px2 = getattr(x, 'bn_partials', None), getattr(x2, 'bn_partials', None)
    if not x.requires_grad:
      x = x.detach().requires_grad_(True)
    if not x2.requires_grad:
      x2 = x2.detach().requires_grad_(True)
    return _BnAddBnFn.apply(x, x2, bn, bn2, px, px2)
  return bn(x, is_training, relu=True, residual=bn2(x2, is_training, relu=False))


class BatchNorm:

  def __init__(self, graph, scope, channels, init_zero=False,
               decay=BATCH_NORM_DECAY, eps=BATCH_NORM_EPSILON, fused=True):
    self.gamma = graph.add_variable(scope + '/gamma', (channels,), V.KIND_OTHER,
                                    0.0, init=None)
    if not init_zero:
      self.gamma.data.fill_(1.0)
    self.beta = graph.add_variable(scope + '/beta', (channels,), V.KIND_OTHER)
    self.moving_mean = torch.zeros(channels, device=graph.device)
    self.moving_variance = torch.ones(channels, device=graph.device)
    self.decay, self.eps = decay, eps
    self.channels = channels
    self.fused = fused
    self.scope = scope
    graph.modules[scope] = self

  def __call__(self, x, is_training=True, relu=False, residual=None, lazy_res_grad=False, consumer=None):
    if (self.fused and is_training and x.is_cuda and self.channels % 8 == 0
        and x.dtype == torch.bfloat16):
      partials = getattr(x, 'bn_partials', None)
      if not x.requires_grad:
        x = x.detach().requires_grad_(True)
      holder = _BnBwdHolder(relu)
      defer = bool(_BN_ON_LOAD and consumer is not None and relu and residual is None and consumer.takes_bn_input(x))
      y = _FusedBNFn.apply(x, residual, self, relu, partials, holder, lazy_res_grad and _LAZY_RES_GRAD, defer)
      y.bn_ctx = holder
      if defer:
        y.bn_pending = holder
      return y
    y = F.batch_norm(nchw_view(x), self.moving_mean, self.moving_variance,
                     bias_tensor(self.gamma), bias_tensor(self.beta),
                     is_training, 1.0 - self.decay, self.eps)
    y = nhwc_view(y)
    if residual is not None:
      y = y + residual
    if relu:
      y = F.relu(y)
    return y


def eval_fused():
  from rigl_amd import ops
  return ops.tune_get('eval_fuse', 1) != 0


def infer_params(graph):
  from rigl_amd import ops
  bns = [m for m in graph.modules.values() if isinstance(m, BatchNorm)]
  return dict(zip(bns, ops.bn_infer_params(bns)))


def conv_infer(conv, x, desc=None, **epilogue):
  from rigl_amd import ops
  n, h, w, _ = x.shape
  d = desc if desc is not None else conv.desc_for(n, h, w)
  return ops.conv_fwd(d, x.contiguous(), conv.vars.ohwi, **epilogue)


def conv_bn_infer(conv, x, bn_in, **epilogue):
  from rigl_amd import ops
  n, h, w, _ = x.shape
  return ops.conv_fwd_bnrelu(conv.desc_for(n, h, w), x.contiguous(), bn_in, conv.vars.ohwi, None, **epilogue)


def dense_infer(layer, x):
  from rigl_amd import ops
  lead = x.shape[:-1]
  x2 = x.reshape(-1, 1, 1, layer.n_in).contiguous()
  b = x2.shape[0]
  d = layer._descs.get(b)
  if d is None:
    d = ops.conv_desc(b, 1, 1, layer.n_in, layer.units, 1, 1, 1, 0, 0, 1, 1)
    layer._descs[b] = d
  y = ops.conv_fwd(d, x2, layer.vars.ohwi).reshape(*lead, layer.units)
  if layer.bias is not None:
    y = y + layer.bias.data.to(y.dtype)
  if layer.activation is not None:
    y = layer.activation(y)
  return y


def bn_relu_max_pool_infer(x, scale_shift):
  from rigl_amd import ops
  if eval_fused():
    return ops.bn_relu_maxpool_infer(_pool_desc(x), x.contiguous(), scale_shift)
  return max_pool_3x3_s2_same(ops.bn_apply(x.contiguous(), scale_shift, relu=True))


class _DepthwiseFn(torch.autograd.Function):

  @staticmethod
  def forward(ctx, x, layer, desc, want_stats=False):
    from rigl_amd import ops
    x = x.contiguous()
    ctx.layer, ctx.desc = layer, desc
    ctx.save_for_backward(x)
    if not want_stats:
      return ops.depthwise_fwd(desc, x, layer.weights.data.view(-1))
    y, part = ops.depthwise_fwd(desc, x, layer.weights.data.view(-1), stats=True)
    if part is None:
      part = torch.empty(0, device=x.device)
    ctx.mark_non_differentiable(part)
    ctx.set_materialize_grads(False)
    return y, part

  @staticmethod
  def backward(ctx, dy, _dpart=None):
    from rigl_amd import ops
# ... 197 lines not shown
```

Baseline: 12510.

## Fuse batch-norm backward apply into the 1x1 conv backward load path

Splits BN backward into a reduce-only pass that emits per-channel coefficients, then applies the BN dx formula inside the 1x1 (64->256) conv backward kernel as dy tiles land in LDS. This avoids writing and re-reading the BN dx tensor for the bottleneck expand convs that feed a residual BN+ReLU. In exchange the conv kernel streams the BN input and relu bits as extra LDS stages, which raises LDS use and register pressure, and the autograd path gains holder handshakes between the BN and conv nodes.

```diff
diff --git a/include/rigl_hip.h b/include/rigl_hip.h
--- a/include/rigl_hip.h
+++ b/include/rigl_hip.h
@@ -210,6 +210,15 @@
                                   float* dw, rigl_bf16* dx, void* workspace,
                                   size_t workspace_bytes, rigl_stream_t stream);
 
+int32_t rigl_conv2d_bwd_takes_bn_apply(const RiglConvDesc* d);
+int rigl_masked_conv2d_bwd_bnapply(const RiglConvDesc* d, const rigl_bf16* x,
+                                   const rigl_bf16* dout, const rigl_bf16* w_hwio,
+                                   const rigl_bf16* addend , float* dw,
+                                   rigl_bf16* dx, void* workspace, size_t workspace_bytes,
+                                   const rigl_bf16* y, const uint8_t* relu_bits,
+                                   const float* mean, const float* invstd,
+                                   const float* coef, rigl_stream_t stream);
+
 typedef struct RiglBnReduceFuse {
   const rigl_bf16* x;
   const uint8_t* relu_bits;
@@ -287,6 +296,12 @@
                 rigl_bf16* dresidual , float* dgamma,
                 float* dbeta, void* workspace, size_t workspace_bytes,
                 rigl_stream_t stream);
+int rigl_bn_bwd_reduce(int64_t m, int32_t c, const rigl_bf16* x,
+                       const uint8_t* relu_bits ,
+                       const rigl_bf16* dy, const float* gamma, const float* save_mean,
+                       const float* save_invstd, int32_t relu, float* dgamma,
+                       float* dbeta, float* coef, void* workspace,
+                       size_t workspace_bytes, rigl_stream_t stream);
 int rigl_bn_bwd_stats(int64_t m, int32_t c, const rigl_bf16* x,
                       const rigl_bf16* y ,
                       const uint8_t* relu_bits , const rigl_bf16* dy,
diff --git a/rigl_amd/_lib.py b/rigl_amd/_lib.py
--- a/rigl_amd/_lib.py
+++ b/rigl_amd/_lib.py
@@ -127,6 +127,8 @@
     'rigl_masked_conv2d_bwd': (C.c_int, [C.POINTER(ConvDesc), _P, _P, _P, _P, _P, _P, _P, _SZ, _P]),
     'rigl_masked_conv2d_bwd_masked': (C.c_int, [C.POINTER(ConvDesc), _P, _P, _P, _P, _P, _P, _P, _P, _SZ, _P]),
     'rigl_conv2d_bwd_takes_masked_addend': (_I32, [C.POINTER(ConvDesc)]),
+    'rigl_conv2d_bwd_takes_bn_apply': (_I32, [C.POINTER(ConvDesc)]),
+    'rigl_masked_conv2d_bwd_bnapply': (C.c_int, [C.POINTER(ConvDesc), _P, _P, _P, _P, _P, _P, _P, _SZ, _P, _P, _P, _P, _P, _P]),
     'rigl_masked_conv2d_bwd_grid': (C.c_int, [C.POINTER(ConvDesc), _P, _P, _P, _P, _P, _P, _SZ, _P]),
     'rigl_masked_conv2d_bwd_sub': (C.c_int, [C.POINTER(ConvDesc), _P, _P, _P, _P, _I32, _I32, _P, _P, _P, _SZ, _P]),
     'rigl_masked_conv2d_wgrad': (C.c_int, [C.POINTER(ConvDesc), _P, _P, _P, _P,
@@ -149,6 +151,7 @@
     'rigl_bn_fwd_stats': (C.c_int, [_I64, _I32, _P, _P, _P, _P, _P, _P, _F, _F, _I32, _P, _P, _P, _P, _P, _P, _I32, _P, _P, _SZ, _P]),
     'rigl_bn_bwd': (C.c_int, [_I64, _I32, _P, _P, _P, _P, _P, _P, _P, _P, _P, _I32, _P, _P, _P, _P, _P, _SZ, _P]),
     'rigl_bn_bwd_stats': (C.c_int, [_I64, _I32, _P, _P, _P, _P, _P, _P, _P, _P, _P, _I32, _P, _P, _P, _P, _P, _I32, _P, _SZ, _P]),
+    'rigl_bn_bwd_reduce': (C.c_int, [_I64, _I32, _P, _P, _P, _P, _P, _P, _I32, _P, _P, _P, _P, _SZ, _P]),
     'rigl_crc32c': (C.c_uint32, [_P, _SZ, C.c_uint32]),
     'rigl_stateless_random': (C.c_int, [_P, _I64, _I32, _I32, _I32, _F, _F, _P]),
     'rigl_stateless_random_batched': (C.c_int, [C.POINTER(RandomItem), _I32, _P]),
diff --git a/rigl_amd/csrc/bn.hip b/rigl_amd/csrc/bn.hip
--- a/rigl_amd/csrc/bn.hip
+++ b/rigl_amd/csrc/bn.hip
@@ -310,8 +310,7 @@
       bool on = true;
       if (RELU) on = MSK == 1 ? (yv[j] > 0.f) : (MSK == 2 ? ((mb >> j) & 1u) != 0u : (fmaf(xv[j], psc[j], psh[j]) > 0.f));
       const float dz = on ? dv[j] : 0.f;
-      const float xh = (xv[j] - pm[j]) * pis[j];
-      o[j] = pa[j] * (dz - pb[j] - xh * pc[j]);
+      o[j] = bn_bwd_dx(dz, xv[j], pm[j], pis[j], pa[j], pb[j], pc[j]);
       z[j] = dz;
     }
     uint4 out;
@@ -742,15 +741,15 @@
   return RIGL_OK;
 }
 
-int rigl_bn_bwd_stats(int64_t m, int32_t c, const rigl_bf16* x, const rigl_bf16* y, const uint8_t* relu_bits,
-                      const rigl_bf16* dy, const float* gamma,
-                      const float* save_mean, const float* save_invstd, const float* save_scale, const float* save_shift,
-                      int32_t relu, rigl_bf16* dx, rigl_bf16* dresidual, float* dgamma, float* dbeta,
-                      const float* stats, int32_t stats_parts, void* workspace,
-                      size_t workspace_bytes, rigl_stream_t stream) {
+static int bn_bwd_impl(int64_t m, int32_t c, const rigl_bf16* x, const rigl_bf16* y, const uint8_t* relu_bits,
+                       const rigl_bf16* dy, const float* gamma,
+                       const float* save_mean, const float* save_invstd, const float* save_scale, const float* save_shift,
+                       int32_t relu, rigl_bf16* dx, rigl_bf16* dresidual, float* dgamma, float* dbeta,
+                       const float* stats, int32_t stats_parts, float* coef_out, void* workspace,
+                       size_t workspace_bytes, rigl_stream_t stream) {
   using namespace rigl;
   using namespace rigl::kbn;
-  if (m <= 0 || c <= 0 || !x || !dy || !gamma || !save_mean || !save_invstd || !dx || !dgamma || !dbeta)
+  if (m <= 0 || c <= 0 || !x || !dy || !gamma || !save_mean || !save_invstd || (!dx && !coef_out) || !dgamma || !dbeta)
     return fail(RIGL_EINVAL, "rigl_bn_bwd: bad arguments");
   if (c % 8) return fail(RIGL_EUNSUPPORTED, "rigl_bn_bwd: channels %% 8 != 0");
   if (relu && !y && !relu_bits && (!save_scale || !save_shift))
@@ -762,7 +761,7 @@
   hipStream_t st = as_stream(stream);
   Geom g = make_geom(m, c);
   float* partial = static_cast<float*>(workspace);
-  float* coef = reinterpret_cast<float*>(static_cast<char*>(workspace) + align_up((size_t)g.parts * 2 * c * 4, 256));
+  float* coef = coef_out ? coef_out : reinterpret_cast<float*>(static_cast<char*>(workspace) + align_up((size_t)g.parts * 2 * c * 4, 256));
   dim3 rgrid((unsigned)g.parts, (unsigned)((g.cg + g.tpr - 1) / g.tpr));
   const int msk = relu_bits ? 2 : (y ? 1 : 0);
   const float* red = partial;
@@ -783,6 +782,10 @@
   else
     hipLaunchKernelGGL(k_bwd_finalize<16>, dim3((unsigned)((c + 15) / 16)), dim3(THREADS), 0, st, g, red, gamma,
                        save_invstd, dgamma, dbeta, coef);
+  if (coef_out) {
+    RIGL_CHECK_LAUNCH("rigl_bn_bwd_reduce");
+    return RIGL_OK;
+  }
   dim3 agrid(apply_grid(g));
   const size_t lds = g.fixed ? 0 : (size_t)7 * c * 4;
 #define RIGL_BWD_APPLY(R, K, D) hipLaunchKernelGGL((k_bwd_apply<R, K, D>), agrid, dim3(THREADS), lds, st, g, x, y, relu_bits, dy, save_mean, save_invstd, save_scale, save_shift, coef, dx, dresidual)
@@ -794,6 +797,25 @@
 #undef RIGL_BWD_APPLY
   RIGL_CHECK_LAUNCH("rigl_bn_bwd");
   return RIGL_OK;
+}
+
+int rigl_bn_bwd_stats(int64_t m, int32_t c, const rigl_bf16* x, const rigl_bf16* y, const uint8_t* relu_bits,
+                      const rigl_bf16* dy, const float* gamma,
+                      const float* save_mean, const float* save_invstd, const float* save_scale, const float* save_shift,
+                      int32_t relu, rigl_bf16* dx, rigl_bf16* dresidual, float* dgamma, float* dbeta,
+                      const float* stats, int32_t stats_parts, void* workspace,
+                      size_t workspace_bytes, rigl_stream_t stream) {
+  return bn_bwd_impl(m, c, x, y, relu_bits, dy, gamma, save_mean, save_invstd, save_scale, save_shift, relu, dx, dresidual, dgamma,
+                     dbeta, stats, stats_parts, nullptr, workspace, workspace_bytes, stream);
+}
+
+int rigl_bn_bwd_reduce(int64_t m, int32_t c, const rigl_bf16* x, const uint8_t* relu_bits, const rigl_bf16* dy, const float* gamma,
+                       const float* save_mean, const float* save_invstd, int32_t relu, float* dgamma, float* dbeta, float* coef,
+                       void* workspace, size_t workspace_bytes, rigl_stream_t stream) {
+  if (!coef) return rigl::fail(RIGL_EINVAL, "rigl_bn_bwd_reduce: coef is required");
+  if (relu && !relu_bits) return rigl::fail(RIGL_EINVAL, "rigl_bn_bwd_reduce: relu needs relu_bits");
+  return bn_bwd_impl(m, c, x, nullptr, relu ? relu_bits : nullptr, dy, gamma, save_mean, save_invstd, nullptr, nullptr, relu, nullptr,
+                     nullptr, dgamma, dbeta, nullptr, 0, coef, workspace, workspace_bytes, stream);
 }
 
 int rigl_bn_bwd(int64_t m, int32_t c, const rigl_bf16* x, const rigl_bf16* y, const uint8_t* relu_bits,
diff --git a/rigl_amd/csrc/bwd1x1.hpp b/rigl_amd/csrc/bwd1x1.hpp
--- a/rigl_amd/csrc/bwd1x1.hpp
+++ b/rigl_amd/csrc/bwd1x1.hpp
@@ -9,6 +9,11 @@
   float* SLAB;
   int M, splits, interleave;
   uint32_t x_bytes, dy_bytes;
+  const uint16_t* Y3;
+  const uint8_t* BITS;
+  const float* MEAN;
+  const float* INVSTD;
+  const float* COEF;
 };
 
 template <int ROWB>
@@ -19,17 +24,22 @@
 
 typedef __attribute__((ext_vector_type(4))) float f32x4;
 
-template <int CI, int CO, bool DO_W, int NST>
-struct Bwd1x1Smem { static constexpr int BYTES = NST * 32 * ((DO_W ? CI : 0) + CO) * 2 + (CI <= 64 ? 2 : 1) * 32 * (CI * 2 + 16); };
-template <int CI, int CO, bool DO_W, int NST>
+template <int CI, int CO, bool DO_W, int NST, bool BNA = false>
+struct Bwd1x1Smem {
+  static constexpr int BYTES = NST * (32 * ((DO_W ? CI : 0) + CO) * 2 + (BNA ? 32 * CO * 2 + 32 * (CO / 8) : 0)) + (CI <= 64 ? 2 : 1) * 32 * (CI * 2 + 16);
+};
+template <int CI, int CO, bool DO_W, int NST, bool BNA = false>
 __global__ __launch_bounds__(THREADS) void k_bwd1x1(Bwd1x1Args P) {
   constexpr int PX = 32;
   constexpr int YROWB = CO * 2, XROWB = CI * 2;
-  constexpr int Y_BYTES = PX * YROWB, X_BYTES = DO_W ? PX * XROWB : 0, STAGE = Y_BYTES + X_BYTES;
+  constexpr int Y_BYTES = PX * YROWB, X_BYTES = DO_W ? PX * XROWB : 0;
+  constexpr int B_BYTES = BNA ? PX * (CO / 8) : 0;
+  constexpr int Y3_OFF = Y_BYTES + X_BYTES, B_OFF = Y3_OFF + (BNA ? Y_BYTES : 0), STAGE = B_OFF + B_BYTES;
+  static_assert(!BNA || (YROWB == 512 && B_BYTES == 4 * 256), "BNA: 256 output channels (a lane's pieces share one channel chunk)");
   constexpr int YI = YROWB / 32, XI = XROWB / 32;
   constexpr int YPW = YI / 4 > 0 ? YI / 4 : 1, XPW = XI / 4 > 0 ? XI / 4 : 1;
   static_assert(YI % 4 == 0 && XI % 4 == 0, "tiles are whole rounds of four waves");
-  constexpr int L = YPW + (DO_W ? XPW : 0);
+  constexpr int L = YPW + (DO_W ? XPW : 0) + (BNA ? YPW + 1 : 0);
   constexpr int CF = CI / 16, CFW = CF / 2;
   constexpr int KSD = CO / 32;
   constexpr int NFI = CI / 32, NFO = CO / 32;
@@ -39,7 +49,7 @@
   constexpr bool DXDB = CI <= 64;
   constexpr int NDX = DXDB ? 2 : 1;
   constexpr int DXROWB = XROWB + 16, DX_BYTES = PX * DXROWB;
-  static_assert(NST * STAGE + NDX * DX_BYTES == Bwd1x1Smem<CI, CO, DO_W, NST>::BYTES, "host and device agree on the LDS size");
+  static_assert(NST * STAGE + NDX * DX_BYTES == Bwd1x1Smem<CI, CO, DO_W, NST, BNA>::BYTES, "host and device agree on the LDS size");
   extern __shared__ __attribute__((aligned(1024))) unsigned char smem[];
   unsigned char* const dxs = smem + NST * STAGE;
 
@@ -54,6 +64,9 @@
   const __amdgpu_buffer_rsrc_t rsrcY = make_rsrc(P.DY, P.dy_bytes), rsrcX = make_rsrc(P.X, P.x_bytes);
   const u32x4 rsrcY4 = make_rsrc4(P.DY, P.dy_bytes), rsrcX4 = make_rsrc4(P.X, P.x_bytes);
   (void)rsrcY4; (void)rsrcX4; (void)rsrcY; (void)rsrcX;
+  const u32x4 rsrcZ4 = make_rsrc4(BNA ? P.Y3 : P.DY, BNA ? P.dy_bytes : 0u);
+  const u32x4 rsrcB4 = make_rsrc4(BNA ? (const void*)P.BITS : (const void*)P.DY, BNA ? P.dy_bytes >> 4 : 0u);
+  (void)rsrcZ4; (void)rsrcB4;
 
   int y_row[YPW], y_col[YPW], x_row[XPW], x_col[XPW];
 #pragma unroll
@@ -65,6 +78,17 @@
   for (int q = 0; q < XPW; ++q) {
     const int i = q * 4 + wave, row = i * (1024 / XROWB) + lane / (XROWB / 16), slot = lane % (XROWB / 16);
     x_row[q] = row; x_col[q] = (slot ^ dual_swz<XROWB>(row)) * 8;
+  }
+  const int b_row = (((lane >> 4) * 4 + wave) << 1) | ((lane >> 3) & 1), b_col = (lane & 7) * 4;
+  float pm[8], pis[8], pa[8], pb[8], pc[8];
+  (void)pm; (void)pis; (void)pa; (void)pb; (void)pc; (void)b_row; (void)b_col;
+  if constexpr (BNA) {
+    const int c0 = y_col[0];
+#pragma unroll
+    for (int j = 0; j < 8; ++j) {
+      pm[j] = P.MEAN[c0 + j]; pis[j] = P.INVSTD[c0 + j];
+      pa[j] = P.COEF[c0 + j]; pb[j] = P.COEF[CO + c0 + j]; pc[j] = P.COEF[2 * CO + c0 + j];
+    }
   }
 #if !defined(RIGL_B1_NO_NT) && !defined(RIGL_DMA_BUILTIN)
 #define B1_DMA16(r_, lds_, off_) lds_dma16_nt(r_##4, lds_, off_)
@@ -78,6 +102,11 @@
       const int p_ = p0_ + y_row[q];                                                                     \
       const int off_ = p_ < P.M ? (int)((uint32_t)(p_ * CO + y_col[q]) * 2u) : (int)OOB;                 \
       B1_DMA16(rsrcY, smem + (stage_) * STAGE + (q * 4 + wave) * 1024, off_); \
+      if (BNA) lds_dma16_nt(rsrcZ4, smem + (stage_) * STAGE + Y3_OFF + (q * 4 + wave) * 1024, off_);       \
+    }                                                                                                    \
+    if (BNA) {                                                                                           \
+      const int p_ = p0_ + b_row;                                                                        \
+      lds_dma4(rsrcB4, smem + (stage_) * STAGE + B_OFF + wave * 256, p_ < P.M ? p_ * (CO / 8) + b_col : (int)OOB); \
     }                                                                                                    \
     if (DO_W) {                                                                                          \
       _Pragma("unroll") for (int q = 0; q < XPW; ++q) {                                                  \
@@ -150,6 +179,29 @@
     } else {
       wait_vmcnt<0>();
     }
+    if constexpr (BNA) {
+      unsigned char* const Yw = smem + (kt % NST) * STAGE;
+      const int p0 = (kt_begin + kt * kt_step) * PX;
+#pragma unroll
+      for (int q = 0; q < YPW; ++q) {
+        unsigned char* const pd = Yw + (q * 4 + wave) * 1024 + lane * 16;
+        const uint4 d4 = *reinterpret_cast<const uint4*>(pd), x4 = *reinterpret_cast<const uint4*>(pd + Y3_OFF);
+        const uint32_t mb = Yw[B_OFF + wave * 256 + (2 * q + (lane >> 5)) * 32 + (y_col[q] >> 3)];
+        const bool rowok = p0 + y_row[q] < P.M;
+        uint32_t o4[4];
+#pragma unroll
+        for (int dd = 0; dd < 4; ++dd) {
+          const uint32_t dw_ = dword_of(d4, dd), xw_ = dword_of(x4, dd);
+          const float dz0 = (mb >> (2 * dd)) & 1u ? __uint_as_float(dw_ << 16) : 0.f;
+          const float dz1 = (mb >> (2 * dd + 1)) & 1u ? __uint_as_float(dw_ & 0xFFFF0000u) : 0.f;
+          const f32x2 o = {bn_bwd_dx(dz0, __uint_as_float(xw_ << 16), pm[2 * dd], pis[2 * dd], pa[2 * dd], pb[2 * dd], pc[2 * dd]),
+                           bn_bwd_dx(dz1, __uint_as_float(xw_ & 0xFFFF0000u), pm[2 * dd + 1], pis[2 * dd + 1], pa[2 * dd + 1],
+                                     pb[2 * dd + 1], pc[2 * dd + 1])};
+          o4[dd] = rowok ? __builtin_bit_cast(uint32_t, __builtin_convertvector(o, bf16x2)) : 0u;
+        }
+        *reinterpret_cast<uint4*>(pd) = make_uint4(o4[0], o4[1], o4[2], o4[3]);
+      }
+    }
     asm volatile("s_waitcnt lgkmcnt(0)" ::: "memory");
     __builtin_amdgcn_s_barrier();
     asm volatile("" ::: "memory");
@@ -240,8 +292,8 @@
 static inline int bwd1x1_kind(const RiglConvDesc* d) {
   if (d->kh != 1 || d->kw != 1 || d->stride_h != 1 || d->stride_w != 1 || d->pad_top || d->pad_left) return 0;
   if (d->ho != d->h || d->wo != d->w) return 0;
-  if ((int64_t)d->n * d->h * d->w < 65536) return 0;
-  if (RIGL_TUNE("bwd1x1", 1) == 0) return 0;
+  const int knob = RIGL_TUNE("bwd1x1", 1);
+  if (knob == 0 || (int64_t)d->n * d->h * d->w < (knob == 2 ? 8192 : 65536)) return 0;
   if (d->cin == 64 && d->cout == 256) return 1;
   if (d->cin == 64 && d->cout == 64) return 3;
   return 0;
@@ -289,3 +341,25 @@
     default: return false;
   }
 }
+
+static bool bwd1x1_bna_ready(const RiglConvDesc* d) {
+  if (!RIGL_TUNE("bn_bwd_on_load", 1) || bwd1x1_kind(d) != 1 || !bwd1x1_ready(d)) return false;
+  constexpr int SMEM = Bwd1x1Smem<64, 256, true, 4, true>::BYTES;
+  static_assert(SMEM <= 160 * 1024, "the ring fits a CU's LDS");
+  static const bool ready = hipFuncSetAttribute(reinterpret_cast<const void*>(&k_bwd1x1<64, 256, true, 4, true>),
+                                                hipFuncAttributeMaxDynamicSharedMemorySize, SMEM) == hipSuccess;
+  return ready;
+}
+static bool launch_bwd1x1_bna(const RiglConvDesc* d, const rigl_bf16* x, const rigl_bf16* dout, const rigl_bf16* w_hwio,
+                              const rigl_bf16* addend, rigl_bf16* dx, float* slab, const rigl_bf16* y3, const uint8_t* bits,
+                              const float* mean, const float* invstd, const float* coef, hipStream_t st) {
+  if (!bwd1x1_bna_ready(d)) return false;
+  Bwd1x1Args a = {};
+  a.X = x; a.DY = dout; a.W = w_hwio; a.ADD = addend; a.DX = dx; a.SLAB = slab;
+  a.M = d->n * d->h * d->w; a.splits = bwd1x1_splits(); a.interleave = RIGL_TUNE("bwd1x1_il", 1);
+  a.x_bytes = (uint32_t)((size_t)a.M * d->cin * 2); a.dy_bytes = (uint32_t)((size_t)a.M * d->cout * 2);
+  a.Y3 = y3; a.BITS = bits; a.MEAN = mean; a.INVSTD = invstd; a.COEF = coef;
+  RIGL_K_LAUNCH((k_bwd1x1<64, 256, true, 4, true>), dim3((unsigned)a.splits), dim3(THREADS),
+                (Bwd1x1Smem<64, 256, true, 4, true>::BYTES), st, a);
+  return true;
+}
diff --git a/rigl_amd/csrc/common.hpp b/rigl_amd/csrc/common.hpp
--- a/rigl_amd/csrc/common.hpp
+++ b/rigl_amd/csrc/common.hpp
@@ -89,4 +89,9 @@
   return make_uint4(gate_bf16x2(v.x, x.x), gate_bf16x2(v.y, x.y), gate_bf16x2(v.z, x.z), gate_bf16x2(v.w, x.w));
 }
 
+__device__ __forceinline__ float bn_bwd_dx(float dz, float x, float mean, float invstd, float a, float b, float c) {
+  const float xh = (x - mean) * invstd;
+  return a * (dz - b - xh * c);
 }
+
+}
diff --git a/rigl_amd/csrc/conv.hip b/rigl_amd/csrc/conv.hip
--- a/rigl_amd/csrc/conv.hip
+++ b/rigl_amd/csrc/conv.hip
@@ -1771,7 +1771,7 @@
     const IgemmArgs ap = dgrad_args(d, dy, w_hwio, addend, dx);
     dgrad_pp = plan_pp<1>(ap).variant != 0;
   }
-  if (whole && !bn && bwd1x1_kind(d) && bwd1x1_ready(d)) {
+  if (whole && !bn && !addend_bits && bwd1x1_kind(d) && bwd1x1_ready(d)) {
     if (need && (!workspace || workspace_bytes < need))
       return fail(RIGL_EWORKSPACE, "rigl_masked_conv2d_bwd: workspace %zu < %zu", workspace_bytes, need);
     ProfFamily prof(PROF_CONV_BWD);
@@ -1797,7 +1797,8 @@
       return RIGL_OK;
     }
   }
-  if (addend_bits) return fail(RIGL_EUNSUPPORTED, "rigl_masked_conv2d_bwd_masked: this layer's kernels take no masked addend (ask rigl_conv2d_bwd_takes_masked_addend)");
+  if (addend_bits && !(whole && rs_masked_use(d)))
+    return fail(RIGL_EUNSUPPORTED, "rigl_masked_conv2d_bwd_masked: this layer's kernels take no masked addend (ask rigl_conv2d_bwd_takes_masked_addend)");
   {
     RsPlan rp;
     if (whole && !bn && rs_use<1>(d, &rp)) {
@@ -1805,7 +1806,7 @@
       rc = rigl_masked_conv2d_wgrad(d, x, dy, dw, workspace, workspace_bytes, stream);
       if (rc) return rc;
       prof_current_kind() = PROF_CONV_BWD;
-      launch_rs<1>(d, rp, dy, w_hwio, addend, dx, nullptr, st);
+      launch_rs<1>(d, rp, dy, w_hwio, addend, dx, nullptr, st, addend_bits);
       RIGL_CHECK_LAUNCH("rigl_masked_conv2d_bwd");
       return RIGL_OK;
     }
@@ -1933,8 +1934,43 @@
   using namespace rigl;
   using namespace rigl::k1;
   if (!d || check_desc(d, "rigl_conv2d_bwd_takes_masked_addend")) return 0;
-  return bs_use(d) ? 1 : 0;
-}
+  if (bs_use(d)) return 1;
+  if ((bwd1x1_kind(d) && bwd1x1_ready(d)) || !rs_masked_use(d)) return 0;
+  return RIGL_TUNE("rs_masked_addend", 1) == 2 || (int64_t)d->n * d->h * d->w >= 65536 ? 1 : 0;
+}
+int32_t rigl_conv2d_bwd_takes_bn_apply(const RiglConvDesc* d) {
+  using namespace rigl;
+  using namespace rigl::k1;
+  if (!d || check_desc(d, "rigl_conv2d_bwd_takes_bn_apply")) return 0;
+  return bwd1x1_bna_ready(d) ? 1 : 0;
+}
+int rigl_masked_conv2d_bwd_bnapply(const RiglConvDesc* d, const rigl_bf16* x, const rigl_bf16* dout, const rigl_bf16* w_hwio,
+                                   const rigl_bf16* addend, float* dw, rigl_bf16* dx, void* workspace, size_t workspace_bytes,
+                                   const rigl_bf16* y, const uint8_t* relu_bits, const float* mean, const float* invstd,
+                                   const float* coef, rigl_stream_t stream) {
+  using namespace rigl;
+  using namespace rigl::k1;
+  int rc = check_desc(d, "rigl_masked_conv2d_bwd_bnapply");
+  if (rc) return rc;
+  if (!x || !dout || !w_hwio || !dw || !dx || !y || !relu_bits || !mean || !invstd || !coef)
+    return fail(RIGL_EINVAL, "rigl_masked_conv2d_bwd_bnapply: NULL tensor");
+  if (!bwd1x1_bna_ready(d))
+    return fail(RIGL_EUNSUPPORTED, "rigl_masked_conv2d_bwd_bnapply: this layer's backward does not take the transform (rigl_conv2d_bwd_takes_bn_apply)");
+  const size_t need = rigl_conv2d_workspace_bytes(d, 2);
+  if (need && (!workspace || workspace_bytes < need))
+    return fail(RIGL_EWORKSPACE, "rigl_masked_conv2d_bwd_bnapply: workspace %zu < %zu", workspace_bytes, need);
+  hipStream_t st = as_stream(stream);
+  prof_set_tag(d);
+  ProfFamily prof(PROF_CONV_BWD);
+  if (!launch_bwd1x1_bna(d, x, dout, w_hwio, addend, dx, static_cast<float*>(workspace), y, relu_bits, mean, invstd, coef, st))
+    return fail(RIGL_EUNSUPPORTED, "rigl_masked_conv2d_bwd_bnapply: the kernel did not launch");
+  const int64_t n_out = (int64_t)d->cin * d->cout;
+  ReduceArgs ra = {static_cast<const float*>(workspace), dw, n_out, n_out, bwd1x1_splits()};
+  launch_wgrad_reduce(ra, st);
+  RIGL_CHECK_LAUNCH("rigl_masked_conv2d_bwd_bnapply");
+  return RIGL_OK;
+}
+
 int rigl_masked_conv2d_bwd_masked(const RiglConvDesc* d, const rigl_bf16* x, const rigl_bf16* dy, const rigl_bf16* w_hwio,
                                   const rigl_bf16* addend, const uint8_t* addend_bits, float* dw, rigl_bf16* dx,
                                   void* workspace, size_t workspace_bytes, rigl_stream_t stream) {
diff --git a/rigl_amd/csrc/rowstream.hpp b/rigl_amd/csrc/rowstream.hpp
--- a/rigl_amd/csrc/rowstream.hpp
+++ b/rigl_amd/csrc/rowstream.hpp
@@ -14,6 +14,7 @@
   const float* BNP;
   uint16_t* A2;
   const float* EPS;
+  const uint8_t* ABITS;
 };
 #ifdef RIGL_RS_TRACE
 #define RS_STAMP(i_) { if (tid == 0 && P.TRACE && (i_) < 64) P.TRACE[blockIdx.x * 64 + (i_)] = __builtin_amdgcn_s_memtime(); }
@@ -27,6 +28,10 @@
   const f32x2 s = {__uint_as_float(a << 16) + __uint_as_float(b << 16),
                    __uint_as_float(a & 0xFFFF0000u) + __uint_as_float(b & 0xFFFF0000u)};
   return __builtin_bit_cast(uint32_t, __builtin_convertvector(s, bf16x2));
+}
+
+__device__ __forceinline__ uint32_t rs_mask_bf16x2(uint32_t m) {
+  return ((0u - (m & 1u)) & 0x0000FFFFu) | ((0u - ((m >> 1) & 1u)) & 0xFFFF0000u);
 }
 
 typedef __attribute__((ext_vector_type(4))) float rs_f32x4;
@@ -60,7 +65,8 @@
   static_assert(!BNL || MODE == 0, "the on-load transform belongs to the forward");
   static_assert(EPI == 0 || (MODE == 0 && (EPI & RS_EPI_EVAL)), "the eval epilogue belongs to the forward");
   constexpr bool EVAL = EPI != 0, EBN = (EPI & RS_EPI_BN) != 0, ERES = EBN && (EPI & RS_EPI_RES), ERELU = EBN && (EPI & RS_EPI_RELU);
-  constexpr bool DGRAD = MODE != 0, ADDEND = MODE == 2 || ERES, STATS = !DGRAD && !EVAL, A2OUT = BNL && !EVAL;
+  constexpr bool MADD = MODE == 3;
+  constexpr bool DGRAD = MODE != 0, ADDEND = MODE == 2 || MADD || ERES, STATS = !DGRAD && !EVAL, A2OUT = BNL && !EVAL;
   using G = RsGeom<KC, TN>;
   constexpr int NS = G::NS, RB = G::RB, CPR = G::CPR, SROW = G::SROW;
   constexpr int CHR = 4 * TN, RPI = 64 / CHR, ITERS = 32 / RPI;
@@ -76,6 +82,7 @@
   const __amdgpu_buffer_rsrc_t rsrcA = make_rsrc(P.A, P.a_bytes), rsrcB = make_rsrc(P.B, P.b_bytes);
   const __amdgpu_buffer_rsrc_t rsrcD = make_rsrc(ADDEND ? P.ADD : P.A, ADDEND ? P.c_bytes : 0u);
   const __amdgpu_buffer_rsrc_t rsrcC = make_rsrc(P.C, P.c_bytes);
+  const __amdgpu_buffer_rsrc_t rsrcM = make_rsrc(MADD ? (const void*)P.ABITS : (const void*)P.A, MADD ? P.c_bytes >> 4 : 0u);
 
   float* const prm = reinterpret_cast<float*>(smem_rs + G::SMEM);
   const __amdgpu_buffer_rsrc_t rsrcA2 = make_rsrc(A2OUT ? P.A2 : P.C, A2OUT ? P.a_bytes : 0u);
@@ -148,6 +155,11 @@
       if (ADDEND) {
 #pragma unroll
         for (int it = 0; it < ITERS; ++it) addv[it] = buf_load16(rsrcD, coff[it]);
+      }
+      uint32_t mbit[MADD ? ITERS : 1];
+      if constexpr (MADD) {
+#pragma unroll
+        for (int it = 0; it < ITERS; ++it) mbit[it] = __builtin_amdgcn_raw_buffer_load_b8(rsrcM, (int)(coff[it] >> 4), 0, 0);
       }
       f32x16 acc[TN];
 #pragma unroll
@@ -242,7 +254,11 @@
         } else if (ADDEND) {
 #pragma unroll
           for (int i4 = 0; i4 < 4; ++i4) {
-            const uint4 q4 = addv[g0 + i4];
+            uint4 q4 = addv[g0 + i4];
+            if constexpr (MADD) {
+              const uint32_t mb = mbit[g0 + i4];
+              q4.x &= rs_mask_bf16x2(mb); q4.y &= rs_mask_bf16x2(mb >> 2); q4.z &= rs_mask_bf16x2(mb >> 4); q4.w &= rs_mask_bf16x2(mb >> 6);
+            }
             v[i4].x = rs_add_bf16x2(v[i4].x, q4.x); v[i4].y = rs_add_bf16x2(v[i4].y, q4.y);
             v[i4].z = rs_add_bf16x2(v[i4].z, q4.z); v[i4].w = rs_add_bf16x2(v[i4].w, q4.w);
           }
@@ -374,20 +390,30 @@
   if (ready && out) *out = p;
   return ready;
 }
+static bool rs_masked_use(const RiglConvDesc* d, RsPlan* out = nullptr) {
+  RsPlan p;
+  if (!RIGL_TUNE("rs_masked_addend", 1) || !rs_use<1>(d, &p)) return false;
+  if (p.kc != 1 || p.tn != 4) return false;
+  if (!rs_ready_i<1, 4, 3>()) return false;
+  if (out) *out = p;
+  return true;
+}
 template <int MODE>
 static void launch_rs(const RiglConvDesc* d, const RsPlan& p, const rigl_bf16* a_act, const rigl_bf16* b_w, const rigl_bf16* addend,
-                      rigl_bf16* c_out, float* stats, hipStream_t st) {
+                      rigl_bf16* c_out, float* stats, hipStream_t st, const uint8_t* addend_bits = nullptr) {
   RsArgs a = {};
 #ifdef RIGL_RS_TRACE
   { const char* e = getenv("RIGL_RS_TRACE_PTR"); a.TRACE = e ? reinterpret_cast<unsigned long long*>(strtoull(e, nullptr, 0)) : nullptr; }
 #endif
   const int k = MODE == 0 ? d->cin : d->cout, n = MODE == 0 ? d->cout : d->cin;
-  a.A = a_act; a.B = b_w; a.C = c_out; a.ADD = addend; a.STATS = stats;
+  a.A = a_act; a.B = b_w; a.C = c_out; a.ADD = addend; a.STATS = stats; a.ABITS = addend_bits;
   a.M = d->n * d->h * d->w; a.N = n; a.F = p.F; a.nfrag = p.nfrag; a.slices = p.slices; a.gprime = p.gprime;
   a.a_bytes = (uint32_t)((size_t)a.M * k * 2); a.b_bytes = (uint32_t)((size_t)n * k * 2); a.c_bytes = (uint32_t)((size_t)a.M * n * 2);
   const dim3 grid((unsigned)(p.slices * p.gprime)), blk(RS_THREADS);
 #define RS_LAUNCH(KC_, TN_, DG_) RIGL_K_LAUNCH((k_rowstream<KC_, TN_, DG_>), grid, blk, (unsigned)(RsGeom<KC_, TN_>::SMEM), st, a);
-  if (MODE == 0) { RS_DISPATCH(p, 0, RS_LAUNCH) } else if (addend) { RS_DISPATCH(p, 2, RS_LAUNCH) } else { RS_DISPATCH(p, 1, RS_LAUNCH) }
+  if (MODE == 0) { RS_DISPATCH(p, 0, RS_LAUNCH) }
+  else if (addend && addend_bits) { RS_LAUNCH(1, 4, 3) }
+  else if (addend) { RS_DISPATCH(p, 2, RS_LAUNCH) } else { RS_DISPATCH(p, 1, RS_LAUNCH) }
 #undef RS_LAUNCH
 }
 
diff --git a/rigl_amd/ops.py b/rigl_amd/ops.py
--- a/rigl_amd/ops.py
+++ b/rigl_amd/ops.py
@@ -538,13 +538,48 @@
   return bool(_plan_cached(d, 'masked_addend', lambda: int(_lib.load().rigl_conv2d_bwd_takes_masked_addend(C.byref(d)))))
 
 
+def conv_bwd_takes_bn_apply(d):
+  if not (mfma_supported(d) and mfma_dgrad_supported(d)):
+    return False
+  return bool(_plan_cached(d, 'bwd_bn_apply', lambda: int(_lib.load().rigl_conv2d_bwd_takes_bn_apply(C.byref(d)))))
+
+
+def conv_bwd_bnapply(d, x, dout, w_hwio, dw, y, relu_bits, saved, coef, addend=None, on_dw_ready=None, dx=None):
+  if not conv_bwd_takes_bn_apply(d):
+    raise ValueError('this layer\'s backward does not take the batch-norm apply (conv_bwd_takes_bn_apply)')
+  for t, nm in ((x, 'x'), (dout, 'dout'), (w_hwio, 'w_hwio'), (y, 'y')):
+    _req(t, torch.bfloat16, nm)
+  _req(addend, torch.bfloat16, 'addend', allow_none=True)
+  _req(dw, torch.float32, 'dw'); _req(saved, torch.float32, 'saved'); _req(coef, torch.float32, 'coef')
+  _req(relu_bits, torch.uint8, 'relu_bits')
+  n_out = d.n * d.ho * d.wo * d.cout
+  if dout.numel() != n_out or y.numel() != n_out or relu_bits.numel() * 8 != n_out:
+    raise ValueError('dout and y must have the shape of the conv output and relu_bits one bit per element of it')
+  if saved.numel() != 4 * d.cout or coef.numel() != 3 * d.cout:
+    raise ValueError('saved must be [4, Cout] and coef [3, Cout]')
+  if addend is not None and addend.numel() != d.n * d.h * d.w * d.cin:
+    raise ValueError('addend must have the shape of dx')
+  lib = _lib.load()
+  _count_macs('wgrad_macs', d)
+  _count_macs('dgrad_macs', d)
+  need = _plan_cached(d, 'ws_wgrad', lambda: lib.rigl_conv2d_workspace_bytes(C.byref(d), 2))
+  ws = workspace(need, x.device, 'wg') if need else None
+  dx = _out(dx, (d.n, d.h, d.w, d.cin), torch.bfloat16, dout.device, 'dx')
+  check(lib.rigl_masked_conv2d_bwd_bnapply(C.byref(d), _ptr(x), _ptr(dout), _ptr(w_hwio), _ptr(addend), _ptr(dw), _ptr(dx), _ptr(ws),
+                                           ws.numel() if ws is not None else 0, _ptr(y), _ptr(relu_bits), _ptr(saved[0]),
+                                           _ptr(saved[1]), _ptr(coef), _stream()))
+  if on_dw_ready is not None:
+    on_dw_ready()
+  return dx
+
+
 def conv_bwd(d, x, dy, w_hwio, dw, need_dx=True, addend=None, on_dw_ready=None, bn_fuse=None, addend_sub=None,
              addend_bits=None, dx=None):
   if addend_sub is not None and tuple(addend_sub) == (1, 1):
     addend_sub = None
   if addend_bits is not None:
-    if addend is None or not need_dx or bn_fuse is not None or addend_sub is not None or not conv_bwd_takes_masked_addend(d):
-      raise ValueError('addend_bits needs an addend, dX and a layer whose backward takes a masked addend')
+    if addend is None or not need_dx or bn_fuse is not None or addend_sub is not None:
+      raise ValueError('addend_bits needs an addend and dX, and combines with neither bn_fuse nor addend_sub')
     _req(x, torch.bfloat16, 'x'); _req(dy, torch.bfloat16, 'dy'); _req(dw, torch.float32, 'dw')
     _req(addend, torch.bfloat16, 'addend'); _req(addend_bits, torch.uint8, 'addend_bits'); _req(w_hwio, torch.bfloat16, 'w_hwio')
     if addend.numel() != d.n * d.h * d.w * d.cin or addend_bits.numel() * 8 != addend.numel():
@@ -836,6 +871,23 @@
   return dx, dres
 
 
+def bn_bwd_reduce(x, dy, gamma, saved, relu, relu_bits, dgamma, dbeta):
+  _req(x, torch.bfloat16, 'x')
+  _req(dy, torch.bfloat16, 'dy')
+  _req(relu_bits, torch.uint8, 'relu_bits', allow_none=not relu)
+  c = x.shape[-1]
+  m = x.numel() // c
+  if dy.numel() != x.numel() or (relu and relu_bits.numel() * 8 != x.numel()):
+    raise ValueError('dy must have the shape of x and relu_bits one bit per element of it')
+  lib = _lib.load()
+  coef = torch.empty((3, c), dtype=torch.float32, device=x.device)
+  ws = workspace(lib.rigl_bn_workspace_bytes(m, c), x.device)
+  check(lib.rigl_bn_bwd_reduce(m, c, _ptr(x), _ptr(relu_bits) if relu else None, _ptr(dy), _ptr(gamma), _ptr(saved[0]),
+                               _ptr(saved[1]), int(bool(relu)), _ptr(dgamma), _ptr(dbeta), _ptr(coef), _ptr(ws), ws.numel(),
+                               _stream()))
+  return coef
+
+
 def stateless_random(n, seed0, seed1, dist, scale=1.0, shift=0.0, device=None,
                      out=None):
   def i32(v):
diff --git a/rigl_amd/pruning_layers.py b/rigl_amd/pruning_layers.py
--- a/rigl_amd/pruning_layers.py
+++ b/rigl_amd/pruning_layers.py
@@ -41,6 +41,30 @@
 def _bn_fuse_publish(holder, req, dx):
   if req is not None and req.get('partials') is not None and dx is not None:
     holder.partials, holder.dx_ptr = req['partials'], dx.data_ptr()
+
+
+class BnApplyHolder:
+  __slots__ = ('armed', 'dout', 'y', 'bits', 'saved', 'coef')
+
+  def __init__(self):
+    self.armed = False
+    self.dout = self.y = self.bits = self.saved = self.coef = None
+
+  def fill(self, dout, y, bits, saved, coef):
+    self.dout, self.y, self.bits, self.saved, self.coef = dout, y, bits, saved, coef
+
+  def take(self, dy):
+    filled = self.dout is not None
+    if self.armed != filled:
+      raise RuntimeError('bn_bwd_on_load: the batch norm %s its apply pass but the forward had decided otherwise'
+                         % ('skipped' if filled else 'ran'))
+    if not filled:
+      return None
+    if dy is not self.dout and (dy.data_ptr() != self.dout.data_ptr() or dy.shape != self.dout.shape or not dy.is_contiguous()):
+      raise RuntimeError('bn_bwd_on_load: the gradient that reached the conv is not the one the batch norm handed over')
+    got = (self.dout, self.y, self.bits, self.saved, self.coef)
+    self.dout = self.y = self.bits = self.saved = self.coef = None
+    return got
 
 
 def _mask_bits(lv):
@@ -92,6 +116,12 @@
       dx = ops.conv_bwd_f32(d, x, dy, lv.weights.data.view(-1), _mask_bits(lv), lv.weights.grad.view(-1),
                             need_dx=ctx.need_dx, on_dw_ready=ready)
       return dx, None, None, None, None, None, None
+    apply_holder = getattr(ctx, 'apply_holder', None)
+    got = apply_holder.take(dy) if apply_holder is not None else None
+    if got is not None:
+      dout, y, bits, saved, coef = got
+      dx = ops.conv_bwd_bnapply(d, x, dout, lv.hwio, lv.weights.grad.view(-1), y, bits, saved, coef, on_dw_ready=ready)
+      return dx, None, None, None, None, None, None
     req = _bn_fuse_request(ctx.bn_holder, ctx.need_dx)
     dx = ops.conv_bwd(d, x, dy, lv.hwio, lv.weights.grad.view(-1), need_dx=ctx.need_dx, on_dw_ready=ready, bn_fuse=req)
     _bn_fuse_publish(ctx.bn_holder, req, dx)
@@ -302,11 +332,16 @@
       raise RuntimeError('a deferred batch-norm output must reach its consumer conv as it was returned')
     if not x.requires_grad:
       x = x.detach().requires_grad_(True)
+    apply_holder = BnApplyHolder() if (need_dx and x.dtype == torch.bfloat16 and x.is_cuda and ops.conv_bwd_takes_bn_apply(d)) else None
     if not bn_stats:
-      return _MaskedConvFn.apply(x.contiguous(), self.vars, d, need_dx, False, holder, pending)
-    y, part = _MaskedConvFn.apply(x.contiguous(), self.vars, d, need_dx, True, holder, pending)
-    if part.numel():
-      y.bn_partials = part
+      y = _MaskedConvFn.apply(x.contiguous(), self.vars, d, need_dx, False, holder, pending)
+    else:
+      y, part = _MaskedConvFn.apply(x.contiguous(), self.vars, d, need_dx, True, holder, pending)
+      if part.numel():
+        y.bn_partials = part
+    if apply_holder is not None and y.grad_fn is not None:
+      y.grad_fn.apply_holder = apply_holder
+      y.bn_apply = apply_holder
     return y
 
   def conv_relu(self, x, gate_input=True):
diff --git a/rigl_amd/workloads/nn.py b/rigl_amd/workloads/nn.py
--- a/rigl_amd/workloads/nn.py
+++ b/rigl_amd/workloads/nn.py
@@ -44,13 +44,19 @@
 class _FusedBNFn(torch.autograd.Function):
 
   @staticmethod
-  def forward(ctx, x, residual, bn, relu, partials=None, holder=None, lazy_res_grad=False, defer=False):
-    from rigl_amd import ops
+  def forward(ctx, x, residual, bn, relu, partials=None, holder=None, lazy_res_grad=False, defer=False, apply_holder=None):
+    from rigl_amd import ops
+    x_in = x
     x = x.contiguous()
     res = residual.contiguous() if residual is not None else None
     ctx.bn, ctx.relu, ctx.has_res = bn, relu, res is not None
     ctx.holder = holder
     ctx.lazy_res_grad = bool(lazy_res_grad) and relu and res is not None
+    ctx.apply_holder = None
+    if (apply_holder is not None and ctx.lazy_res_grad and not defer and x is x_in and ctx.needs_input_grad[0]
+        and ctx.needs_input_grad[1]):
+      ctx.apply_holder = apply_holder
+      apply_holder.armed = True
     if defer:
       saved = ops.bn_statistics(x, bn.gamma.data, bn.beta.data, bn.moving_mean, bn.moving_variance, 1.0 - bn.decay, bn.eps,
                                 partials=partials)
@@ -86,16 +92,21 @@
       if h.partials is not None and h.dx_ptr == dy.data_ptr():
         part = h.partials
       h.partials = h.x = h.saved = h.bits = None
+    if ctx.apply_holder is not None:
+      coef = ops.bn_bwd_reduce(x, dy, bn.gamma.data, saved, True, bits, bn.gamma.grad, bn.beta.grad)
+      ctx.apply_holder.fill(dy, x, bits, saved, coef)
+      ops.LAZY_ADDEND_BITS[dy.data_ptr()] = (bits, dy)
+      return dy, dy, None, None, None, None, None, None, None
     if ctx.lazy_res_grad and bits is not None and ctx.needs_input_grad[1]:
       dx, _ = ops.bn_bwd(x, None, dy, bn.gamma.data, saved, ctx.relu, bn.gamma.grad, bn.beta.grad, want_dres=False,
                          relu_bits=bits, partials=part)
       ops.LAZY_ADDEND_BITS[dy.data_ptr()] = (bits, dy)
-      return dx, dy, None, None, None, None, None, None
+      return dx, dy, None, None, None, None, None, None, None
     dx, dres = ops.bn_bwd(x, None, dy, bn.gamma.data, saved, ctx.relu,
                           bn.gamma.grad, bn.beta.grad,
                           want_dres=ctx.has_res and ctx.needs_input_grad[1],
                           relu_bits=bits, partials=part)
-    return dx, dres, None, None, None, None, None, None
+    return dx, dres, None, None, None, None, None, None, None
 
 
 class _BnAddBnFn(torch.autograd.Function):
@@ -163,7 +174,8 @@
         x = x.detach().requires_grad_(True)
       holder = _BnBwdHolder(relu)
       defer = bool(_BN_ON_LOAD and consumer is not None and relu and residual is None and consumer.takes_bn_input(x))
-      y = _FusedBNFn.apply(x, residual, self, relu, partials, holder, lazy_res_grad and _LAZY_RES_GRAD, defer)
+      apply_holder = getattr(x, 'bn_apply', None)
+      y = _FusedBNFn.apply(x, residual, self, relu, partials, holder, lazy_res_grad and _LAZY_RES_GRAD, defer, apply_holder)
       y.bn_ctx = holder
       if defer:
         y.bn_pending = holder
```

Measured after the change: 12670, median of 6. 1.01x the previous value.
